# ShanningLiu/xsDeepFwFM_deprecated

Measured on AMD Instinct MI355X. Metric: CTR samples/sec (forward, batch 4096, Criteo-39) at 1/2/4/8 MI355X; AUC match, higher is better.
Workload: dtype f32

## Files before the change

xsdeepfwfm_deprecated_amd/DeepFMs.py:

```python
from __future__ import annotations

import contextlib
import logging
import math
import os
import random
from time import time, time_ns

import numpy as np
import torch
import torch.nn as nn
import torch.nn.functional as F

from . import metrics
from .QREmbeddingBag import QREmbeddingBag
from .engine import CpuEngine, ForwardEngine
from ._lib import DfwfmError, FLAG_INDEX_OUT_OF_RANGE

_log = logging.getLogger("xsDeepFwFM")


class DeepFMs(nn.Module):
    def __init__(self, field_size, feature_sizes, embedding_size=10, is_shallow_dropout=True,
                 dropout_shallow=[0.0, 0.0], h_depth=3, deep_nodes=400, is_deep_dropout=True,
                 dropout_deep=[0.5, 0.5, 0.5, 0.5], eval_metric=metrics.roc_auc_score, n_epochs=64,
                 batch_size=2048, learning_rate=0.001, momentum=0.9, optimizer_type="adam",
                 is_batch_norm=False, verbose=False, random_seed=0, weight_decay=0.0, use_fm=True,
                 use_fwlw=False, use_lw=False, use_ffm=False, use_fwfm=False, use_deep=True,
                 loss_type="logloss", use_cuda=True, n_class=1, greater_is_better=True, sparse=0.9,
                 warm=10, num_deeps=1, numerical=13, use_logit=0, embedding_bag=False,
                 quantization_aware=False, dynamic_quantization=False, static_quantization=False,
                 static_calibrate=False, qr_flag=0, qr_operation="mult", qr_collisions=1,
                 qr_threshold=200, md_flag=0, md_threshold=200, logger=None):
        super().__init__()
        self.logger = logger if logger is not None else _log
        self.field_size = int(field_size)
        self.feature_sizes = [int(s) for s in feature_sizes]
        self.embedding_size = int(embedding_size)
        self.is_shallow_dropout = is_shallow_dropout
        self.dropout_shallow = dropout_shallow
        self.h_depth = int(h_depth)
        self.num_deeps = int(num_deeps)
        self.deep_layers = [int(deep_nodes)] * self.h_depth
        self.is_deep_dropout = is_deep_dropout
        self.dropout_deep = [0.5] * (self.h_depth + 1)
        self.n_epochs = n_epochs
        self.batch_size = batch_size
        self.learning_rate = learning_rate
        self.momentum = momentum
        self.optimizer_type = optimizer_type
        self.is_batch_norm = is_batch_norm
        self.verbose = verbose
        self.weight_decay = weight_decay
        self.random_seed = random_seed
        self.use_fm, self.use_ffm, self.use_fwfm = use_fm, use_ffm, use_fwfm
        self.use_fwlw, self.use_lw, self.use_logit, self.use_deep = use_fwlw, use_lw, use_logit, use_deep
        self.loss_type = loss_type
        self.eval_metric = eval_metric
        self.use_cuda = use_cuda
        self.n_class = n_class
        self.greater_is_better = greater_is_better
        self.target_sparse = sparse
        self.warm = warm
        self.num = int(numerical)
        self.embedding_bag = embedding_bag if not qr_flag else qr_flag
        self.quantization_aware = quantization_aware
        self.static_quantization = static_quantization
        self.static_calibrate = static_calibrate
        self.dynamic_quantization = dynamic_quantization
        self.qr_flag = qr_flag
        self.qr_operation = qr_operation
        self.qr_collisions = qr_collisions
        self.qr_threshold = qr_threshold
        self.md_flag = md_flag
        self.md_threshold = md_threshold
        self.strict_index_check = True
        self.eval_batch_sets = True
        self.sparse_mlp_max_density = 0.0
        self.fwfm_pair_max = 0
        self.pack_tables = True
        self.small_batch_rows = 0
        self.mlp_dtype = "f32"
        self.deterministic = True
        self._defer_index_check = 0
        self._engine = None

        np.random.seed(self.random_seed)
        random.seed(self.random_seed)
        torch.manual_seed(self.random_seed)

        if quantization_aware or dynamic_quantization or static_quantization:
            raise NotImplementedError("quantization is not part of the MI355X engine (SURVEY.md section 2 #10)")
        if use_ffm:
            raise NotImplementedError("FFM is not part of the MI355X engine (SURVEY.md section 2 #12)")
        if self.num_deeps != 1:
            raise NotImplementedError("num_deeps > 1 is not supported")
        if is_batch_norm:
            raise NotImplementedError("batch norm in the deep tower is not supported")
        if self.use_cuda and not torch.cuda.is_available():
            self.use_cuda = False
            self.logger.info("Cuda is not available, automatically changed into cpu model")

        n_shallow = int(bool(use_fm)) + int(bool(use_ffm)) + int(bool(use_fwfm)) + int(bool(use_logit))
        if n_shallow > 1:
            self.logger.info("only support one type only, please make sure to choose only LR, FM, FFM or FwFM part")
            raise SystemExit(1)
        if n_shallow == 0 and not use_deep:
            self.logger.info("You have to choose more than one of (fm, ffm, fwfm, deep) models to use")
            raise SystemExit(1)
        self.logger.info(self._describe())

        D, Fs = self.embedding_size, self.field_size
        if use_logit or use_fm or use_fwfm:
            self.bias = nn.Parameter(torch.tensor([0.01]))
            if not use_fwlw:
                self.fm_1st_embeddings = self._tables(1)
            if self.dropout_shallow:
                self.fm_first_order_dropout = nn.Dropout(self.dropout_shallow[0])
            if use_fm or use_fwfm:
                self.fm_2nd_embeddings = self._tables(D)
                if self.dropout_shallow:
                    self.fm_second_order_dropout = nn.Dropout(self.dropout_shallow[1])
                if use_lw:
                    self.fm_1st = nn.Linear(Fs, 1, bias=False)
                if use_fwlw:
                    self.fwfm_linear = nn.Linear(D, Fs, bias=False)
                if use_fwfm:
                    self.field_cov = nn.Linear(Fs, Fs, bias=False)
        if use_deep:
            if not use_fm and not use_fwfm:
                self.fm_2nd_embeddings = self._tables(D)
            widths = [Fs * D] + self.deep_layers
            if self.is_deep_dropout:
                self.net_1_linear_0_dropout = nn.Dropout(self.dropout_deep[0])
            for i in range(1, self.h_depth + 1):
                setattr(self, f"net_1_linear_{i}", nn.Linear(widths[i - 1], widths[i]))
                setattr(self, f"net_1_linear_{i}_relu", nn.ReLU())
                if self.is_deep_dropout:
                    setattr(self, f"net_1_linear_{i}_dropout", nn.Dropout(self.dropout_deep[i]))
            self.net_1_fc = nn.Linear(self.deep_layers[-1], 1, bias=False)

    def _describe(self):
        if self.use_logit:
            return "The model is logistic regression."
        kind = "fm" if self.use_fm else ("fwfm" if self.use_fwfm else None)
        if kind and self.use_deep:
            return f"The model is deep{kind}({kind}+deep layers)"
        if kind:
            return f"The model is {kind} only"
        return "The model is deep layers only"

    def _tables(self, dim):
        if not self.embedding_bag:
            return nn.ModuleList([nn.Embedding(n, dim) for n in self.feature_sizes])
        tables = nn.ModuleList()
        for n in self.feature_sizes:
            if self.qr_flag and n > self.qr_threshold:
                tables.append(QREmbeddingBag(n, dim, self.qr_collisions, operation=self.qr_operation,
                                             mode="sum", sparse=False))
            else:
                bag = nn.EmbeddingBag(n, dim, mode="sum", sparse=False)
                w = np.random.uniform(low=-np.sqrt(1 / n), high=np.sqrt(1 / n), size=(n, dim)).astype(np.float32)
                bag.weight.data = torch.tensor(w)
                tables.append(bag)
        return tables

    def engine_config(self):
        return dict(field_size=self.field_size, numerical=self.num, embedding_size=self.embedding_size,
                    use_fwfm=int(bool(self.use_fwfm)), use_fm=int(bool(self.use_fm)),
                    use_logit=int(bool(self.use_logit)), use_deep=int(bool(self.use_deep)),
                    use_lw=int(bool(self.use_lw)), use_fwlw=int(bool(self.use_fwlw)),
                    h_depth=self.h_depth, deep_nodes=self.deep_layers[0])

    @staticmethod
    def _field_desc(mod_2nd, mod_1st):
        def parts(mod):
            if mod is None:
                return None, None
            if isinstance(mod, QREmbeddingBag):
                if mod.operation not in ("mult", "add"):
                    raise NotImplementedError("QR 'concat' changes the field width; unsupported")
                return mod.weight_q.detach(), mod.weight_r.detach()
            return mod.weight.detach(), None
        ref = mod_2nd if mod_2nd is not None else mod_1st
        if isinstance(ref, QREmbeddingBag):
            n, c, op = ref.num_categories, ref.num_collisions, 0 if ref.operation == "mult" else 1
        else:
            n, c, op = ref.weight.shape[0], 0, 0
        e2, e2r = parts(mod_2nd)
        e1, e1r = parts(mod_1st)
        return dict(emb2=e2, emb2_r=e2r, emb1=e1, emb1_r=e1r, n=n, c=c, op=op)

    def _sync_engine(self, device):
        if device.type == "cpu":
            return self._sync_cpu_engine()
        if device.type != "cuda":
            raise DfwfmError(f"DeepFMs forward runs on a HIP device or the CPU, not on {device}")
        if self._engine is None or self._engine.device != device:
            if self._engine is not None:
                self._engine.close()
            self._engine = ForwardEngine(self.engine_config(), device)
        eng = self._engine
        first = getattr(self, "fm_1st_embeddings", None)
        second = getattr(self, "fm_2nd_embeddings", None)
        fields = [self._field_desc(None if second is None else second[f], None if first is None else first[f])
                  for f in range(self.field_size)]
        eng.sync_tables(fields)

        def w(name, attr="weight"):
            m = getattr(self, name, None)
            return None if m is None else getattr(m, attr).detach()

        lin_w = [w(f"net_1_linear_{i}") for i in range(1, self.h_depth + 1)] if self.use_deep else []
        lin_b = [w(f"net_1_linear_{i}", "bias") for i in range(1, self.h_depth + 1)] if self.use_deep else []
        eng.sync_dense(w("field_cov"), w("fwfm_linear"), w("fm_1st") if self.use_lw else None,
                       self.bias.detach(), lin_w, lin_b, w("net_1_fc") if self.use_deep else None)
        return eng

    def _sync_inference(self, device):
        eng = self._sync_engine(device)
        if device.type == "cuda":
            first = getattr(self, "fm_1st_embeddings", None)
            second = getattr(self, "fm_2nd_embeddings", None)
            tabs = []
            for f in range(self.num, self.field_size):
                d = self._field_desc(None if second is None else second[f], None if first is None else first[f])
                tabs.append((d["emb2"], d["emb1"]))
            eng.sync_packed(tabs, self.pack_tables)
            eng.small_rows = max(int(getattr(self, "small_batch_rows", 0)), 0) if self.use_deep else 0
            eng.bf16 = eng.sync_bf16(self._mlp_bf16()) if self.use_deep else False
        return eng

    def _mlp_bf16(self) -> bool:
        dt = getattr(self, "mlp_dtype", "f32")
        if dt not in ("f32", "bf16"):
            raise ValueError(f"mlp_dtype must be 'f32' or 'bf16', got {dt!r}")
        if not self.use_deep or dt == "f32":
            return False
        if self.sparse_mlp_max_density > 0:
            raise ValueError("mlp_dtype='bf16' and sparse_mlp_max_density > 0 are two deep towers: choose one")
        return True

    def _sync_cpu_engine(self):
        if not isinstance(self._engine, CpuEngine):
            if self._engine is not None:
                self._engine.close()
            self._engine = CpuEngine(self.engine_config())
        first = getattr(self, "fm_1st_embeddings", None)
        second = getattr(self, "fm_2nd_embeddings", None)
        fields = [self._field_desc(None if second is None else second[f], None if first is None else first[f])
                  for f in range(self.field_size)]

        def w(name, attr="weight"):
            m = getattr(self, name, None)
            return None if m is None else getattr(m, attr).detach()
        lin_w = [w(f"net_1_linear_{i}") for i in range(1, self.h_depth + 1)] if self.use_deep else []
        lin_b = [w(f"net_1_linear_{i}", "bias") for i in range(1, self.h_depth + 1)] if self.use_deep else []
        self._engine.sync(fields, w("field_cov"), w("fwfm_linear"), w("fm_1st") if self.use_lw else None,
                          self.bias.detach(), lin_w, lin_b, w("net_1_fc") if self.use_deep else None)
        return self._engine

    def _param_layout(self):
        def parts(mod):
            if mod is None:
                return None, None
            if isinstance(mod, QREmbeddingBag):
                return mod.weight_q, mod.weight_r
            return mod.weight, None
        first = getattr(self, "fm_1st_embeddings", None)
        second = getattr(self, "fm_2nd_embeddings", None)
        fields = []
        for f in range(self.field_size):
            e2, e2r = parts(None if second is None else second[f])
            e1, e1r = parts(None if first is None else first[f])
            fields.append((e2, e2r, e1, e1r))

        def w(name, attr="weight"):
            m = getattr(self, name, None)
            return None if m is None else getattr(m, attr)
        H = self.h_depth if self.use_deep else 0
        dense = dict(field_cov=w("field_cov"), fwfm_lin=w("fwfm_linear"),
                     fm_1st=w("fm_1st") if self.use_lw else None, bias=getattr(self, "bias", None),
                     lin_w=[w(f"net_1_linear_{i}") for i in range(1, H + 1)],
                     lin_b=[w(f"net_1_linear_{i}", "bias") for i in range(1, H + 1)],
                     fc_w=w("net_1_fc") if self.use_deep else None)
        return fields, dense

    def _prep_inputs(self, Xi, Xv, device):
        ncat = self.field_size - self.num
        Xi = torch.as_tensor(Xi)
        Xv = torch.as_tensor(Xv)
        if Xi.dim() == 3:
            Xi = Xi.reshape(Xi.shape[0], Xi.shape[1])
        if Xi.dim() != 2 or Xi.shape[1] != ncat:
            raise RuntimeError(f"Xi must be [B, {ncat}, 1] or [B, {ncat}], got {tuple(Xi.shape)}")
        if Xv.dim() != 2 or Xv.shape[0] != Xi.shape[0] or Xv.shape[1] < self.num:
            raise RuntimeError(f"Xv must be [B, >= {self.num}], got {tuple(Xv.shape)}")
        Xi = Xi.to(device=device, dtype=torch.int64)
        Xv = Xv.to(device=device, dtype=torch.float32)
        if Xi.stride(1) != 1:
            Xi = Xi.contiguous()
        if Xv.stride(1) != 1:
            Xv = Xv.contiguous()
        return Xi, Xv

    def forward(self, Xi, Xv):
        device = self._device()
        eng = self._sync_engine(device)
        xi, xv = self._prep_inputs(Xi, Xv, device)
        needs_grad = torch.is_grad_enabled() and any(p.requires_grad for p in self.parameters())
        if needs_grad:
# ... 306 lines not shown
```

xsdeepfwfm_deprecated_amd/_lib.py:

```python
from __future__ import annotations

import ctypes
import os
import subprocess
import threading

import torch

PKG_DIR = os.path.dirname(os.path.abspath(__file__))
REPO_DIR = os.path.dirname(PKG_DIR)
CSRC = os.path.join(PKG_DIR, "csrc")
LIB_PATH = os.path.join(PKG_DIR, "libdfwfm.so")
LOAD_PATH = os.path.join(PKG_DIR, os.environ["DFWFM_LIB"]) if os.environ.get("DFWFM_LIB") else LIB_PATH
SOURCES = ["dfwfm_kernels.hip", "dfwfm_fwd32.hip", "dfwfm_ftrain.hip", "dfwfm_train.hip", "dfwfm_prune.hip", "dfwfm_metrics.hip", "dfwfm_sparse.hip",
           "dfwfm_spmlp.hip", "dfwfm_serve.hip", "dfwfm_bf16.hip", "dfwfm_capi.hip"]
EMB_SIZES = (4, 8, 10, 16, 32)
PER_D_SOURCES = ["dfwfm_kernels.hip", "dfwfm_train.hip"]


def _units():
    u = [(s, os.path.splitext(s)[0] + ".o", []) for s in SOURCES]
    for s in PER_D_SOURCES:
        u += [(s, f"{os.path.splitext(s)[0]}_d{d}.o", [f"-DDFWFM_KD={d}"]) for d in EMB_SIZES]
    return u
HEADERS = ["dfwfm_internal.h", "dfwfm_device.h", os.path.join("..", "..", "include", "dfwfm.h"),
           os.path.join("..", "..", "include", "dfwfm_serve.h"), os.path.join("..", "..", "include", "dfwfm_bf16.h")]
ARCH = os.environ.get("DFWFM_OFFLOAD_ARCH", "gfx950")
CPU_PATH = os.path.join(PKG_DIR, "libdfwfm_cpu.so")
CPU_SOURCES = ["dfwfm_cpu.cpp"]
CPU_HEADERS = [os.path.join("..", "..", "include", "dfwfm_cpu.h"), os.path.join("..", "..", "include", "dfwfm.h")]
INGEST_PATH = os.path.join(PKG_DIR, "libdfwfm_ingest.so")
INGEST_SOURCES = ["dfwfm_ingest.cpp"]
INGEST_HEADERS = [os.path.join("..", "..", "include", "dfwfm_ingest.h")]

DFWFM_OK = 0
STATUS = {0: "ok", -1: "invalid argument", -2: "unsupported", -3: "HIP error", -4: "bad state"}
FLAG_INDEX_OUT_OF_RANGE = 1
BWD_TABLES, BWD_MLP_WEIGHTS, BWD_TILES, BWD_SPREAD, BWD_REDUCE, BWD_SCATTER = 1, 2, 4, 8, 16, 32
FAMILY_SECOND, FAMILY_FIRST = 0, 1
ADAM_STATE_BYTES = 48


class DfwfmError(RuntimeError):
    pass


class dfwfm_config(ctypes.Structure):
    _fields_ = [(n, ctypes.c_int32) for n in (
        "field_size", "numerical", "embedding_size", "use_fwfm", "use_fm", "use_logit",
        "use_deep", "use_lw", "use_fwlw", "h_depth", "deep_nodes")]


class dfwfm_field_tables(ctypes.Structure):
    _fields_ = [
        ("emb2", ctypes.c_void_p), ("emb2_r", ctypes.c_void_p),
        ("emb1", ctypes.c_void_p), ("emb1_r", ctypes.c_void_p),
        ("num_categories", ctypes.c_int64), ("qr_collisions", ctypes.c_int64),
        ("qr_operation", ctypes.c_int32), ("reserved", ctypes.c_int32),
    ]


class dfwfm_field_grads(ctypes.Structure):
    _fields_ = [(n, ctypes.c_void_p) for n in ("emb2", "emb2_r", "emb1", "emb1_r")]


class dfwfm_grads(ctypes.Structure):
    _fields_ = [
        ("fields", ctypes.POINTER(dfwfm_field_grads)),
        ("field_cov", ctypes.c_void_p), ("fwfm_lin", ctypes.c_void_p), ("fm_1st", ctypes.c_void_p),
        ("bias", ctypes.c_void_p), ("lin_w", ctypes.POINTER(ctypes.c_void_p)),
        ("lin_b", ctypes.POINTER(ctypes.c_void_p)), ("fc_w", ctypes.c_void_p),
    ]


class dfwfm_adam_tensor(ctypes.Structure):
    _fields_ = [("param", ctypes.c_void_p), ("grad", ctypes.c_void_p), ("exp_avg", ctypes.c_void_p),
                ("exp_avg_sq", ctypes.c_void_p), ("numel", ctypes.c_int64)]


class dfwfm_sparse_dest(ctypes.Structure):
    _fields_ = [("q", ctypes.c_int64), ("r", ctypes.c_int64)]


class dfwfm_prune_source(ctypes.Structure):
    _fields_ = [("values", ctypes.c_void_p), ("numel", ctypes.c_int64), ("sym_f", ctypes.c_int32),
                ("reserved", ctypes.c_int32)]


_P = ctypes.c_void_p
SIGNATURES = {
    "dfwfm_model_create": (ctypes.c_int, [ctypes.POINTER(dfwfm_config), ctypes.POINTER(_P)]),
    "dfwfm_model_destroy": (None, [_P]),
    "dfwfm_model_set_tables": (ctypes.c_int, [_P, ctypes.POINTER(dfwfm_field_tables), ctypes.c_int32, _P]),
    "dfwfm_model_set_dense": (ctypes.c_int, [_P, _P, _P, _P, _P, ctypes.POINTER(_P), ctypes.POINTER(_P), _P, _P]),
    "dfwfm_model_set_dense_zero": (ctypes.c_int, [_P, _P, _P, _P, _P, ctypes.POINTER(_P), ctypes.POINTER(_P), _P, _P,
                                                  ctypes.c_int64, _P]),
    "dfwfm_forward": (ctypes.c_int, [_P, _P, ctypes.c_int64, _P, ctypes.c_int64, ctypes.c_int64, _P, _P]),
    "dfwfm_forward_batches": (ctypes.c_int, [_P, ctypes.c_int32, _P, ctypes.c_int64, _P, ctypes.c_int64,
                                             ctypes.c_int64, _P, _P]),
    "dfwfm_forward_workspace_bytes": (ctypes.c_int, [_P, ctypes.c_int64, ctypes.POINTER(ctypes.c_size_t)]),
    "dfwfm_forward_ws": (ctypes.c_int, [_P, _P, ctypes.c_int64, _P, ctypes.c_int64, ctypes.c_int64, _P, _P,
                                        ctypes.c_size_t, _P]),
    "dfwfm_model_build_sparse_mlp": (ctypes.c_int, [_P, ctypes.c_double, ctypes.POINTER(ctypes.c_int32), _P]),
    "dfwfm_model_build_fwfm_pairs": (ctypes.c_int, [_P, ctypes.c_int32, ctypes.POINTER(ctypes.c_int32), _P]),
    "dfwfm_model_pack_tables": (ctypes.c_int, [_P, ctypes.c_int32, ctypes.POINTER(ctypes.c_int32), _P]),
    "dfwfm_forward_gather": (ctypes.c_int, [_P, _P, ctypes.c_int64, _P, ctypes.c_int64, ctypes.c_int64, _P,
                                            ctypes.c_int64, _P, _P]),
    "dfwfm_train_forward": (ctypes.c_int, [_P, _P, ctypes.c_int64, _P, ctypes.c_int64, ctypes.c_int64, _P,
                                           ctypes.c_float, ctypes.c_uint32, _P]),
    "dfwfm_backward": (ctypes.c_int, [_P, _P, ctypes.POINTER(dfwfm_grads), _P]),
    "dfwfm_backward_phases": (ctypes.c_int, [_P, _P, ctypes.POINTER(dfwfm_grads), ctypes.c_int32, _P]),
    "dfwfm_adam_step": (ctypes.c_int, [ctypes.POINTER(dfwfm_adam_tensor), ctypes.c_int32, ctypes.c_double,
                                       ctypes.c_double, ctypes.c_double, ctypes.c_double, ctypes.c_double,
                                       ctypes.c_int64, _P]),
    "dfwfm_set_step_source": (ctypes.c_int, [_P, _P]),
    "dfwfm_workspace_generation": (ctypes.c_int, [_P, ctypes.POINTER(ctypes.c_int64)]),
    "dfwfm_adam_step_dev": (ctypes.c_int, [ctypes.POINTER(dfwfm_adam_tensor), ctypes.c_int32, ctypes.c_double,
                                           ctypes.c_double, ctypes.c_double, ctypes.c_double, ctypes.c_double,
                                           _P, _P]),
    "dfwfm_bce_grad": (ctypes.c_int, [_P, _P, ctypes.c_int64, ctypes.c_double, _P, _P, _P]),
    "dfwfm_backward_phases_bce": (ctypes.c_int, [_P, _P, _P, ctypes.c_double, _P, _P, ctypes.POINTER(dfwfm_grads),
                                                 ctypes.c_int32, _P]),
    "dfwfm_sparse_grads_size": (ctypes.c_int, [_P, ctypes.c_int32, ctypes.c_int64, ctypes.POINTER(ctypes.c_int64),
                                               ctypes.POINTER(ctypes.c_int32), ctypes.POINTER(ctypes.c_int64)]),
    "dfwfm_sparse_grads_apply": (ctypes.c_int, [_P, ctypes.c_int32, _P, _P, _P, ctypes.c_int64, _P]),
    "dfwfm_sparse_grads_local": (ctypes.c_int, [_P, ctypes.c_int32, ctypes.POINTER(dfwfm_sparse_dest), ctypes.c_int64,
                                                _P, _P, ctypes.c_int64, _P, _P, _P, _P]),
    "dfwfm_prune_workspace_bytes": (ctypes.c_int64, [ctypes.c_int64]),
    "dfwfm_prune_threshold": (ctypes.c_int, [ctypes.POINTER(dfwfm_prune_source), ctypes.c_int32, ctypes.c_double,
                                             _P, _P, ctypes.c_int64, _P]),
    "dfwfm_prune_apply": (ctypes.c_int, [_P, ctypes.c_int64, ctypes.c_int32, _P, _P]),
    "dfwfm_metrics_workspace_bytes": (ctypes.c_int64, [ctypes.c_int64]),
    "dfwfm_eval_metrics": (ctypes.c_int, [_P, _P, ctypes.c_int64, _P, _P, ctypes.c_int64, _P]),
    "dfwfm_read_error_flag": (ctypes.c_int, [_P, ctypes.POINTER(ctypes.c_int32), _P]),
    "dfwfm_last_error": (ctypes.c_char_p, []),
    "dfwfm_diag_stamps": (ctypes.c_int, [_P, ctypes.POINTER(ctypes.c_uint64), ctypes.c_int64, _P]),
    "dfwfm_abi_version": (ctypes.c_int, []),
    "dfwfm_set_deterministic": (ctypes.c_int, [_P, ctypes.c_int32]),
}

SERVE_SIGNATURES = {
    "dfwfm_serve_abi_version": (ctypes.c_int, []),
    "dfwfm_serve_workspace_bytes": (ctypes.c_int, [_P, ctypes.c_int64, ctypes.POINTER(ctypes.c_size_t)]),
    "dfwfm_serve_forward": (ctypes.c_int, [_P, _P, ctypes.c_int64, _P, ctypes.c_int64, ctypes.c_int64, _P, _P,
                                           ctypes.c_size_t, _P]),
}

BF16_SIGNATURES = {
    "dfwfm_bf16_abi_version": (ctypes.c_int, []),
    "dfwfm_model_pack_bf16": (ctypes.c_int, [_P, ctypes.c_int, _P]),
    "dfwfm_bf16_workspace_bytes": (ctypes.c_int, [_P, ctypes.c_int64, ctypes.POINTER(ctypes.c_size_t)]),
    "dfwfm_bf16_forward": (ctypes.c_int, [_P, _P, ctypes.c_int64, _P, ctypes.c_int64, ctypes.c_int64, _P, _P,
                                          ctypes.c_size_t, _P]),
}

_lib = None
_lock = threading.Lock()


def _stale() -> bool:
    if not os.path.exists(LIB_PATH):
        return True
    t = os.path.getmtime(LIB_PATH)
    deps = [os.path.join(CSRC, s) for s in SOURCES + HEADERS]
    return any(os.path.getmtime(d) > t for d in deps if os.path.exists(d))


def _stale_ingest() -> bool:
    if not os.path.exists(INGEST_PATH):
        return True
    t = os.path.getmtime(INGEST_PATH)
    deps = [os.path.join(CSRC, s) for s in INGEST_SOURCES + INGEST_HEADERS]
    return any(os.path.getmtime(d) > t for d in deps if os.path.exists(d))


def build_ingest(force: bool = False, verbose: bool = False) -> str:
    if not force and not _stale_ingest():
        return INGEST_PATH
    cxx = os.environ.get("CXX", "g++")
    tmp = INGEST_PATH + ".tmp"
    cmd = [cxx, "-O3", "-std=c++17", "-fPIC", "-shared", "-pthread", "-o", tmp] + \
        [os.path.join(CSRC, s) for s in INGEST_SOURCES]
    if verbose:
        print(" ".join(cmd))
    subprocess.run(cmd, check=True, cwd=CSRC)
    os.replace(tmp, INGEST_PATH)
    return INGEST_PATH


def _stale_cpu() -> bool:
    if not os.path.exists(CPU_PATH):
        return True
    t = os.path.getmtime(CPU_PATH)
    deps = [os.path.join(CSRC, s) for s in CPU_SOURCES + CPU_HEADERS]
    return any(os.path.getmtime(d) > t for d in deps if os.path.exists(d))


def build_cpu(force: bool = False, verbose: bool = False) -> str:
    if not force and not _stale_cpu():
        return CPU_PATH
    cxx = os.environ.get("CXX", "g++")
    tmp = CPU_PATH + ".tmp"
    cmd = [cxx, "-O3", "-std=c++17", "-fPIC", "-shared", "-pthread", "-mavx2", "-mfma", "-o", tmp] + \
        [os.path.join(CSRC, s) for s in CPU_SOURCES]
    if verbose:
        print(" ".join(cmd))
    subprocess.run(cmd, check=True, cwd=CSRC)
    os.replace(tmp, CPU_PATH)
    return CPU_PATH


def build(force: bool = False, verbose: bool = False) -> str:
    build_ingest(force, verbose)
    build_cpu(force, verbose)
    hipcc = os.environ.get("HIPCC", "/opt/rocm/bin/hipcc")
    flags = [f"--offload-arch={ARCH}", "-O3", "-std=c++17", "-fPIC"] + os.environ.get("DFWFM_HIPCC_FLAGS", "").split()
    stamp = os.path.join(CSRC, ".build_flags")
    if not os.path.exists(stamp) or open(stamp).read() != " ".join(flags):
        force = True
    if not force and not _stale():
        return LIB_PATH
    from concurrent.futures import ThreadPoolExecutor
    units = _units()
    objs = [os.path.join(CSRC, o) for _, o, _ in units]
    hdr_m = max(os.path.getmtime(os.path.join(CSRC, h)) for h in HEADERS)

    def compile_one(i):
        src, _, extra = units[i]
        src = os.path.join(CSRC, src)
        if not force and os.path.exists(objs[i]) and \
                os.path.getmtime(objs[i]) >= max(os.path.getmtime(src), hdr_m):
            return
        cmd = [hipcc] + flags + extra + ["-c", "-o", objs[i], src]
        if verbose:
            print(" ".join(cmd))
        subprocess.run(cmd, check=True, cwd=CSRC)

    jobs = int(os.environ.get("MAX_JOBS", "0")) or min(len(units), max(1, len(os.sched_getaffinity(0))))
# ... 31 lines not shown
    "dfwfm_cpu_saved_floats": (ctypes.c_int64, [ctypes.POINTER(dfwfm_config)]),
    "dfwfm_cpu_forward": (ctypes.c_int, [ctypes.POINTER(dfwfm_cpu_model), _P, ctypes.c_int64, _P, ctypes.c_int64,
                                         ctypes.c_int64, _P, _P, ctypes.c_float, ctypes.c_uint32,
                                         ctypes.POINTER(ctypes.c_int32), ctypes.c_int32]),
    "dfwfm_cpu_backward": (ctypes.c_int, [ctypes.POINTER(dfwfm_cpu_model), _P, ctypes.c_int64, _P, ctypes.c_int64,
                                          ctypes.c_int64, _P, _P, ctypes.c_float, ctypes.c_uint32,
                                          ctypes.POINTER(dfwfm_grads), ctypes.c_int32]),
    "dfwfm_cpu_last_error": (ctypes.c_char_p, []),
    "dfwfm_cpu_abi_version": (ctypes.c_int, []),
}


def cpu_lib():
    global _cpu
    if _cpu is not None:
        return _cpu
    with _lock:
        if _cpu is None:
            if not os.path.exists(CPU_PATH):
                raise DfwfmError(f"{CPU_PATH} is missing: run xsdeepfwfm_deprecated_amd.build()")
            L = ctypes.CDLL(CPU_PATH)
            for name, (res, args) in CPU_SIGNATURES.items():
                fn = getattr(L, name)
                fn.restype = res
                fn.argtypes = args
            if L.dfwfm_cpu_abi_version() != 1:
                raise DfwfmError("libdfwfm_cpu ABI mismatch")
            _cpu = L
    return _cpu


def check_cpu(rc: int, what: str) -> None:
    if rc != DFWFM_OK:
        msg = cpu_lib().dfwfm_cpu_last_error().decode(errors="replace")
        raise DfwfmError(f"{what} failed ({STATUS.get(rc, rc)}): {msg}")


def ingest_lib():
    global _ingest
    if _ingest is not None:
        return _ingest
    with _lock:
        if _ingest is None:
            if not os.path.exists(INGEST_PATH):
                raise DfwfmError(f"{INGEST_PATH} is missing: run xsdeepfwfm_deprecated_amd.build()")
            L = ctypes.CDLL(INGEST_PATH)
            for name, (res, args) in INGEST_SIGNATURES.items():
                fn = getattr(L, name)
                fn.restype = res
                fn.argtypes = args
            _ingest = L
    return _ingest


def lib():
    global _lib
    if _lib is not None:
        return _lib
    with _lock:
        if _lib is not None:
            return _lib
        if not os.path.exists(LOAD_PATH):
            raise DfwfmError(f"{LOAD_PATH} is missing: run xsdeepfwfm_deprecated_amd.build() "
                             "(hipcc --offload-arch=gfx950); there is no CPU fallback")
        L = ctypes.CDLL(LOAD_PATH)
        for name, (res, args) in SIGNATURES.items():
            fn = getattr(L, name)
            fn.restype = res
            fn.argtypes = args
        if L.dfwfm_abi_version() != 4:
            raise DfwfmError("libdfwfm ABI mismatch")
        for name, (res, args) in SERVE_SIGNATURES.items():
            fn = getattr(L, name)
            fn.restype = res
            fn.argtypes = args
        if L.dfwfm_serve_abi_version() != 1:
            raise DfwfmError("libdfwfm serve ABI mismatch")
        for name, (res, args) in BF16_SIGNATURES.items():
            fn = getattr(L, name)
            fn.restype = res
            fn.argtypes = args
        if L.dfwfm_bf16_abi_version() != 1:
            raise DfwfmError("libdfwfm bf16 ABI mismatch")
        _lib = L
    return _lib


def check(rc: int, what: str) -> None:
    if rc != DFWFM_OK:
        msg = lib().dfwfm_last_error().decode(errors="replace")
        raise DfwfmError(f"{what} failed ({STATUS.get(rc, rc)}): {msg}")
```

xsdeepfwfm_deprecated_amd/csrc/dfwfm_capi.hip:

```cpp
#include <hip/hip_runtime.h>
#include <mutex>
#include <stdint.h>
#include <stdarg.h>
#include <stdio.h>
#include <stdlib.h>
#include <string.h>

#include <cmath>
#include <string>
#include <vector>

#include "dfwfm_internal.h"
#include "../../include/dfwfm_serve.h"
#include "../../include/dfwfm_bf16.h"

using namespace dfwfm;

struct dfwfm_model {
  dfwfm_config cfg;
  int device;
  int F, D, num, H, N;
  int NT, NC0, SX, SY, TPW, MT, S, W0, KS;
  int TPWF, tail;
  int flags;
  size_t lds_bytes;
  size_t lds_gather;
  int NG, TPWI, tailI;
  int r32;
  size_t lds_r32;
  size_t lds_ftrain;
  void* cu_stream[8];
  int cu_count[8], cu_n, cu_next;
  int dev_cus;
  size_t lds_inf;
  int sp;
  const float* lin_w[kMaxH];
  int2* d_ell;
  int32_t* d_cnt;
  int32_t* d_spstat;
  int spW[kMaxH];
  int64_t spoff[kMaxH];
  double sp_density;
  uint8_t fw_list4[kMaxPieces], fw_off4[5];
  uint8_t fw_list8[kMaxPieces], fw_off8[9];
  FieldDev* d_fields;
  float* d_upack;
  int2* d_pairs;
  float* d_pkrows;
  size_t pkrows_floats;
  const float** d_pk;
  int pkw;
  int32_t npairs;
  int32_t* d_err;
  float4* d_wpack;
  size_t wpack_elems;
  float* d_mlp_b;
  float* d_fc;
  float* d_fwlw;
  float* d_lw;
  float* d_bias;
  uint16_t* d_wbf16;
  bool bf16_on;
  uint64_t* d_stamps;
  size_t stamps_cap;
  size_t stamps_ring;
  size_t stamps_next;
  float4* d_wtpack;
  size_t wtpack_elems;
  int wt_off[kMaxH + 1];
  float* d_rsk;
  float* d_ws;
  int64_t ws_batch;
  int64_t ws_gen;
  float* sv_e;
  float* sv_fo;
  float* sv_x[kMaxH + 1];
  float* sv_g[kMaxH + 1];
  float* sv_de;
  int32_t* sv_keys;
  int64_t keys_stride;
  bool t_keys;
  float* sv_x0;
  float* red_part;
  float* dw_part;
  float* dw_bpart;
  int64_t dw_slices;
  FieldDev h_fields[64];
  const int64_t* t_xi;
  int64_t t_xs;
  const float* t_xv;
  int64_t t_vs;
  int64_t t_batch;
  float t_drop;
  uint32_t t_seed;
  const int64_t* step_src;
  bool trained;
  bool bwd_tables;
  bool bwd_fused_red;
  float* bwd_loss_sum;
  bool deterministic;
  bool tables_set;
  bool dense_set;
};

namespace {

thread_local std::string g_last_error;

int fail(int code, const char* fmt, ...) __attribute__((format(printf, 2, 3)));
int fail(int code, const char* fmt, ...) {
  char buf[512];
  va_list ap;
  va_start(ap, fmt);
  vsnprintf(buf, sizeof buf, fmt, ap);
  va_end(ap);
  g_last_error = buf;
  return code;
}

int hip_fail(hipError_t e, const char* what) {
  return fail(DFWFM_ERR_HIP, "%s: %s", what, hipGetErrorString(e));
}

#define HIP_TRY(expr)                                  \
  do {                                                 \
    hipError_t e_ = (expr);                            \
    if (e_ != hipSuccess) return hip_fail(e_, #expr);  \
  } while (0)

template <typename T>
int dev_alloc(T** p, size_t count) {
  *p = nullptr;
  if (count == 0) count = 1;
  HIP_TRY(hipMalloc(reinterpret_cast<void**>(p), count * sizeof(T)));
  return DFWFM_OK;
}

void free_model(dfwfm_model* m) {
  if (!m) return;
  void* ptrs[] = {m->d_fields, m->d_upack, m->d_err,     m->d_wpack, m->d_mlp_b,   m->d_fc,  m->d_fwlw,
                  m->d_lw,     m->d_bias,  m->d_stamps,  m->d_wtpack, m->d_rsk,   m->d_ws,
                  m->d_ell,    m->d_cnt,   m->d_spstat, m->d_pairs, m->d_pkrows, m->d_pk,
                  m->d_wbf16};
  for (void* p : ptrs)
    if (p) (void)hipFree(p);
// ... 51 lines not shown
    return fail(DFWFM_ERR_INVALID_ARG, "use_logit with use_fwlw has no first-order tables");
  const int F = c.field_size, D = c.embedding_size;
  int H = 0, N = 0, NT = 0, TPW = 0;
  if (c.use_deep) {
    H = c.h_depth;
    N = c.deep_nodes;
    if (H < 1 || H > 16) return fail(DFWFM_ERR_UNSUPPORTED, "h_depth %d outside [1, 16]", H);
    NT = (N + 15) / 16;
    TPW = (NT + 3) / 4;
    if (N < 1 || TPW > kMaxTPW)
      return fail(DFWFM_ERR_UNSUPPORTED, "deep_nodes %d outside [1, %d]", N, 64 * kMaxTPW);
  }

  dfwfm_model* m = new dfwfm_model();
  memset(m, 0, sizeof *m);
  m->cfg = c;
  m->deterministic = true;
  hipError_t e = hipGetDevice(&m->device);
  if (e != hipSuccess) {
    delete m;
    return hip_fail(e, "hipGetDevice");
  }
  m->F = F;
  m->D = D;
  m->num = c.numerical;
  m->H = H;
  m->N = N;
  m->NT = NT;
  m->TPW = TPW;
  m->NC0 = (F * D + 15) / 16;
  m->MT = (F + 15) / 16;
  m->S = (F + 3) / 4;
  fw_schedule(m->MT, D, m->S, 4, m->fw_list4, m->fw_off4);
  fw_schedule(m->MT, D, m->S, 8, m->fw_list8, m->fw_off8);
  m->W0 = m->NC0 * 16 > 4 * m->S * D ? m->NC0 * 16 : 4 * m->S * D;
  const int kx = m->W0 > NT * 16 ? m->W0 : NT * 16;
  m->SX = r4(kx) + 4;
  m->SY = c.use_deep ? NT * 16 + 4 : 0;
  m->KS = 1;
  m->TPWF = TPW;
  m->tail = 0;
  if (c.use_deep && m->KS == 1 && NT % 4 == 1 && NT >= 5 && m->NC0 >= 4 && m->NC0 <= 4 * kTailC &&
      NT <= 4 * kTailC) {
    m->TPWF = NT / 4;
    m->tail = 1;
  }
  const bool second = c.use_fwfm || c.use_fm;
  m->flags = (second ? kHasSecond : 0) | (c.use_deep ? kHasDeep : 0) |
             (c.use_fwlw ? kFoFwlw : kFoTables) | ((second && c.use_lw) ? kFoLw : 0) |
             ((second || c.use_deep) ? kNeedE : 0);
  const LdsLayout L = lds_layout(F, D, m->MT, m->S, m->SX, m->SY, m->TPWF > 0 ? m->TPWF : 1, m->KS,
                                 c.use_deep != 0, m->tail != 0);
  m->lds_bytes = sizeof(float) * (size_t)L.total;
  m->lds_gather = sizeof(float) * (size_t)lds_layout(F, D, m->MT, m->S, m->SX, m->SY, m->TPWF > 0 ? m->TPWF : 1,
                                                     1, false, false).total;
  m->NG = 4;
  m->TPWI = m->TPWF;
  m->tailI = m->tail;
  m->lds_inf = m->lds_bytes;
  if (!c.use_deep)
    m->lds_inf = sizeof(float) * (size_t)lds_layout(F, D, m->MT, m->S, m->SX, m->SY, 1, 1, false, false, 8).total;
  if (c.use_deep && m->KS == 1 && NT <= 32 && m->NC0 <= 32) {
    if (diag_opt("ng", 8) == 8) {
      m->NG = 8;
      m->tailI = (NT % 8 == 1 && NT >= 9 && m->NC0 >= 8) ? 1 : 0;
      m->TPWI = m->tailI ? NT / 8 : (NT + 7) / 8;
      m->lds_inf = sizeof(float) * (size_t)lds_layout(F, D, m->MT, m->S, m->SX, m->SY, m->TPWI, 1, true,
                                                      m->tailI != 0, 8).total;
    }
  }
  {
    const int r32 = diag_opt("r32", -1);
    const int mode = r32 < 0 ? 1 : (r32 != 0 ? 2 : 0);
    m->r32 = (c.use_deep && fwd32_supported(F, D, H, NT, m->NC0, m->tailI, m->NG)) ? mode : 0;
    m->lds_r32 = m->r32 ? fwd32_lds_bytes(F, D, m->MT, m->S, m->SX) : 0;
    m->lds_ftrain = (c.use_deep && ftrain_supported(F, D, H, NT, m->NC0, m->tailI, m->NG))
                        ? ftrain_lds_bytes(F, D, m->MT, m->S, m->SX, m->SY) : 0;
    if (m->lds_ftrain > 160 * 1024) m->lds_ftrain = 0;
  }
  if (m->lds_bytes > 160 * 1024 || m->lds_inf > 160 * 1024) {
    free_model(m);
    return fail(DFWFM_ERR_UNSUPPORTED, "LDS tile of %zu bytes exceeds 160 KiB", m->lds_bytes);
  }

  int rc = DFWFM_OK;
  if ((rc = dev_alloc(&m->d_fields, F)) || (rc = dev_alloc(&m->d_upack, (size_t)m->MT * m->S * 64)) ||
      (rc = dev_alloc(&m->d_err, 1)) ||
      (rc = dev_alloc(&m->d_fwlw, (size_t)F * D)) || (rc = dev_alloc(&m->d_lw, F)) ||
      (rc = dev_alloc(&m->d_bias, 1))) {
    free_model(m);
    return rc;
  }
  if ((rc = dev_alloc(&m->d_rsk, (size_t)m->MT * m->S * 64))) {
    free_model(m);
    return rc;
  }
  if (c.use_deep) {
    m->wpack_elems = (size_t)NT * m->NC0 * 64 + (size_t)(H - 1) * NT * NT * 64;
    if (m->wpack_elems * sizeof(float4) >= (size_t)1 << 31) {
      free_model(m);
      return fail(DFWFM_ERR_UNSUPPORTED, "packed MLP weights exceed the 2 GiB buffer-descriptor range");
    }
    m->wtpack_elems = m->wpack_elems;
    m->wt_off[1] = 0;
    for (int l = 2; l <= H; ++l) m->wt_off[l] = m->wt_off[l - 1] + (l == 2 ? m->NC0 : NT) * NT * 64;
    if ((rc = dev_alloc(&m->d_wtpack, m->wtpack_elems)) || (rc = dev_alloc(&m->d_wpack, m->wpack_elems)) ||
        (rc = dev_alloc(&m->d_mlp_b, (size_t)H * NT * 16)) || (rc = dev_alloc(&m->d_fc, (size_t)NT * 16))) {
      free_model(m);
      return rc;
    }
  }
  e = hipMemset(m->d_err, 0, sizeof(int32_t));
  if (e == hipSuccess) e = hipMemset(m->d_upack, 0, sizeof(float) * (size_t)m->MT * m->S * 64);
  if (e != hipSuccess) {
    free_model(m);
    return hip_fail(e, "hipMemset");
  }
  *out = m;
  return DFWFM_OK;
}

void dfwfm_model_destroy(dfwfm_model* m) { free_model(m); }

int dfwfm_model_set_tables(dfwfm_model* m, const dfwfm_field_tables* t, int32_t n, void* stream) {
  if (!m || !t) return fail(DFWFM_ERR_INVALID_ARG, "null argument");
  if (n != m->F) return fail(DFWFM_ERR_INVALID_ARG, "%d tables for %d fields", n, m->F);
  const bool need_fo = (m->flags & kFoTables) != 0;
  const bool need_e = (m->flags & kNeedE) != 0;
  for (int f = 0; f < n; ++f) {
    const dfwfm_field_tables& x = t[f];
    if (need_e && !x.emb2) return fail(DFWFM_ERR_INVALID_ARG, "field %d: emb2 is null", f);
    if (need_fo && !x.emb1) return fail(DFWFM_ERR_INVALID_ARG, "field %d: emb1 is null", f);
    if (x.num_categories < 1) return fail(DFWFM_ERR_INVALID_ARG, "field %d: num_categories < 1", f);
    if (x.qr_collisions < 0) return fail(DFWFM_ERR_INVALID_ARG, "field %d: qr_collisions < 0", f);
    if (x.qr_collisions > 0) {
      if (f < m->num) return fail(DFWFM_ERR_INVALID_ARG, "field %d: numerical field cannot be QR", f);
      if ((need_e && !x.emb2_r) || (need_fo && !x.emb1_r))
        return fail(DFWFM_ERR_INVALID_ARG, "field %d: QR remainder table is null", f);
      if (x.qr_operation != 0 && x.qr_operation != 1)
        return fail(DFWFM_ERR_UNSUPPORTED, "field %d: QR operation %d (only mult=0, add=1)", f,
                    x.qr_operation);
    }
    const uintptr_t align = (m->D % 4 == 0) ? 16 : (m->D % 2 == 0 ? 8 : 4);
    if (((uintptr_t)x.emb2 % align) || (x.emb2_r && ((uintptr_t)x.emb2_r % align)))
      return fail(DFWFM_ERR_UNSUPPORTED, "field %d: table base not %zu-byte aligned", f, (size_t)align);
  }
  FieldDev host[64];
  memcpy(host, t, sizeof(dfwfm_field_tables) * n);
  for (int f = 0; f < n; ++f)
    if (host[f].c > 0) host[f].n = (host[f].n + host[f].c - 1) / host[f].c * host[f].c;
  memcpy(m->h_fields, host, sizeof(FieldDev) * n);
  m->pkw = 0;
  m->flags &= ~kHasQR;
  for (int f = 0; f < n; ++f)
    if (host[f].c > 0) m->flags |= kHasQR;
  HIP_TRY(hipMemcpyAsync(m->d_fields, host, sizeof(FieldDev) * n, hipMemcpyHostToDevice, (hipStream_t)stream));
  HIP_TRY(hipStreamSynchronize((hipStream_t)stream));
  m->tables_set = true;
  return DFWFM_OK;
}

static int set_dense_impl(dfwfm_model* m, const float* field_cov, const float* fwfm_lin, const float* fm_1st,
                          const float* bias, const float* const* lin_w, const float* const* lin_b,
                          const float* fc_w, float* zero, int64_t nzero, void* stream) {
  if (!m) return fail(DFWFM_ERR_INVALID_ARG, "null model");
  if (nzero < 0 || (nzero > 0 && (!zero || (nzero & 3) || (reinterpret_cast<uintptr_t>(zero) & 15))))
    return fail(DFWFM_ERR_INVALID_ARG, "zero range: 16-byte aligned, a multiple of 4 floats");
  hipStream_t s = (hipStream_t)stream;
  const dfwfm_config& c = m->cfg;
  if (c.use_fwfm && !field_cov) return fail(DFWFM_ERR_INVALID_ARG, "use_fwfm needs field_cov");
  if ((m->flags & kFoFwlw) && !fwfm_lin) return fail(DFWFM_ERR_INVALID_ARG, "use_fwlw needs fwfm_linear");
  if ((m->flags & kFoLw) && !fm_1st) return fail(DFWFM_ERR_INVALID_ARG, "use_lw needs fm_1st");
  if (!bias) return fail(DFWFM_ERR_INVALID_ARG, "bias is required");
  PackList L;
  memset(&L, 0, sizeof L);
  int blocks = 0;
  auto job = [&](int type, const float* src, void* dst, int64_t total, int a, int b, int d) {
    PackJob& j = L.j[L.n++];
    j.src = src;
    j.dst = reinterpret_cast<float*>(dst);
    j.total = total;
    j.type = type;
    j.a = a;
    j.b = b;
    j.d = d;
    j.block0 = blocks;
    blocks += (int)((total + 255) / 256);
  };
  if (nzero > 0) {
    const int64_t n4 = nzero / 4;
    if ((n4 + 256 * kPackZeroPT - 1) / (256 * kPackZeroPT) > 0x3fffffff) return fail(DFWFM_ERR_UNSUPPORTED, "zero range");
    PackJob& j = L.j[L.n++];
    j.src = nullptr;
    j.dst = zero;
    j.total = n4;
    j.type = kPackZero;
    j.a = j.b = j.d = 0;
    j.block0 = blocks;
    blocks += (int)((n4 + 256 * kPackZeroPT - 1) / (256 * kPackZeroPT));
  }
  if (c.use_fwfm || c.use_fm) {
    const int64_t tot = (int64_t)m->MT * m->S * 64;
    job(kPackFwfm, field_cov, m->d_upack, tot, m->F, c.use_fm ? 1 : 0, m->S);
    job(kPackFwfmSym, field_cov, m->d_rsk, tot, m->F, c.use_fm ? 1 : 0, m->S);
  }
  if (m->flags & kFoFwlw) job(kPackPad, fwfm_lin, m->d_fwlw, m->F * m->D, m->F * m->D, 0, 0);
  if (m->flags & kFoLw) job(kPackPad, fm_1st, m->d_lw, m->F, m->F, 0, 0);
  job(kPackPad, bias, m->d_bias, 1, 1, 0, 0);
  if (c.use_deep) {
    if (!lin_w || !lin_b || !fc_w) return fail(DFWFM_ERR_INVALID_ARG, "use_deep needs MLP weights");
    size_t off = 0;
    for (int h = 0; h < m->H; ++h) {
      if (!lin_w[h] || !lin_b[h]) return fail(DFWFM_ERR_INVALID_ARG, "layer %d weight/bias is null", h);
      const int K = h == 0 ? m->F * m->D : m->N;
      const int NC = h == 0 ? m->NC0 : m->NT;
      const int64_t tot = (int64_t)m->NT * NC * 64;
      job(kPackLinear, lin_w[h], m->d_wpack + off, tot, m->N, K, NC);
      job(kPackLinearT, lin_w[h], m->d_wtpack + m->wt_off[h + 1], tot, m->N, K, m->NT);
      job(kPackPad, lin_b[h], m->d_mlp_b + (size_t)h * m->NT * 16, m->NT * 16, m->N, 0, 0);
      off += (size_t)tot;
    }
    job(kPackPad, fc_w, m->d_fc, m->NT * 16, m->N, 0, 0);
  }
  hipError_t e = launch_pack_list(L, blocks, s);
  if (e != hipSuccess) return hip_fail(e, "pack launch");
  m->dense_set = true;
  m->sp = 0;
  m->bf16_on = false;
  m->flags &= ~kPairs;
  for (int h = 0; h < m->H; ++h) m->lin_w[h] = lin_w ? lin_w[h] : nullptr;
  return DFWFM_OK;
}

int dfwfm_model_set_dense(dfwfm_model* m, const float* field_cov, const float* fwfm_lin, const float* fm_1st,
                          const float* bias, const float* const* lin_w, const float* const* lin_b,
                          const float* fc_w, void* stream) {
  return set_dense_impl(m, field_cov, fwfm_lin, fm_1st, bias, lin_w, lin_b, fc_w, nullptr, 0, stream);
}

int dfwfm_model_set_dense_zero(dfwfm_model* m, const float* field_cov, const float* fwfm_lin, const float* fm_1st,
                               const float* bias, const float* const* lin_w, const float* const* lin_b,
                               const float* fc_w, float* zero, int64_t nzero, void* stream) {
  return set_dense_impl(m, field_cov, fwfm_lin, fm_1st, bias, lin_w, lin_b, fc_w, zero, nzero, stream);
}

}

namespace {

int check_inputs(dfwfm_model* m, const int64_t* xi, int64_t xi_stride, const float* xv, int64_t xv_stride,
                 int64_t batch, const void* out) {
  if (batch < 0) return fail(DFWFM_ERR_INVALID_ARG, "negative batch");
  if (!m->tables_set || !m->dense_set)
    return fail(DFWFM_ERR_STATE, "set_tables and set_dense must precede forward");
  if (batch == 0) return DFWFM_OK;
  const int ncat = m->F - m->num;
  if (!out || (ncat > 0 && !xi) || (m->num > 0 && !xv))
    return fail(DFWFM_ERR_INVALID_ARG, "null input/output pointer");
  if (ncat > 0 && xi_stride < ncat) return fail(DFWFM_ERR_INVALID_ARG, "xi_stride < F - numerical");
  if (m->num > 0 && xv_stride < m->num) return fail(DFWFM_ERR_INVALID_ARG, "xv_stride < numerical");
  if ((batch + kBM - 1) / kBM > 0x7fffffff) return fail(DFWFM_ERR_UNSUPPORTED, "batch too large");
  return DFWFM_OK;
}

void fill_forward_args(const dfwfm_model* m, FwdArgs& a, const int64_t* xi, int64_t xi_stride, const float* xv,
                       int64_t xv_stride, int64_t batch, float* out) {
  memset(&a, 0, sizeof a);
  a.fields = m->d_fields;
  a.xi = xi;
  a.xi_stride = xi_stride;
  a.xv = xv;
  a.xv_stride = xv_stride;
  a.batch = batch;
  a.out = out;
  a.err = m->d_err;
  a.upack = m->d_upack;
  a.pk = m->pkw ? m->d_pk : nullptr;
  a.pkw = m->pkw;
  a.pairs = m->d_pairs;
  a.npairs = m->npairs;
  a.fwlw = m->d_fwlw;
  a.lw = m->d_lw;
  a.bias = m->d_bias;
  a.wpack = m->d_wpack;
  a.wpack_bytes = (int32_t)(m->wpack_elems * sizeof(float4));
  a.mlp_b = m->d_mlp_b;
  a.fc = m->d_fc;
  a.F = m->F;
  a.num = m->num;
  a.H = m->H;
  a.N = m->N;
  a.NT = m->NT;
  a.NC0 = m->NC0;
  a.MT = m->MT;
  a.S = m->S;
  a.W0 = m->W0;
  a.tail = m->tail;
  a.SX = m->SX;
  a.SY = m->SY;
  a.flags = m->flags;
  if (!m->cfg.use_deep && m->MT <= 3) a.flags |= kP3Pieces;
  a.ns = (m->NC0 == 25 && m->NT == 25) ? 25 : 0;
  memcpy(a.fw_list4, m->fw_list4, sizeof a.fw_list4);
  memcpy(a.fw_list8, m->fw_list8, sizeof a.fw_list8);
  memcpy(a.fw_off4, m->fw_off4, sizeof a.fw_off4);
  memcpy(a.fw_off8, m->fw_off8, sizeof a.fw_off8);
}

int dw_plan(const dfwfm_model* m, int64_t batch, int* per_split, int64_t* splits, int64_t* rows,
            int64_t* cap = nullptr) {
  const int edge = kDwEdge, quantum = kDwRows;
  const int nnb = (m->N + edge - 1) / edge;
  int ps = 0;
  for (int l = 1; l <= m->H; ++l) ps += nnb * (((l == 1 ? m->F * m->D : m->N) + edge - 1) / edge);
  *per_split = ps;
  *splits = *rows = 0;
  if (cap) *cap = 0;
  if (ps == 0 || batch <= 0) return DFWFM_OK;
  int64_t sp = 256 / ps;
  const int64_t max_splits = (batch + 127) / 128;
  if (sp > max_splits) sp = max_splits;
  if (sp < 1) sp = 1;
  const int64_t wmax = r4(m->F * m->D) > m->N ? r4(m->F * m->D) : m->N;
  const int64_t rows_cap = ((0x7fffffffLL / (wmax * 4)) * 4 - 4 * quantum) / quantum * quantum;
  if (rows_cap < quantum) return fail(DFWFM_ERR_UNSUPPORTED, "MLP rows of %lld floats", (long long)wmax);
  if ((batch + sp - 1) / sp > rows_cap) sp = (batch + rows_cap - 1) / rows_cap;
  if (cap) *cap = sp;
  int64_t r = (batch + sp - 1) / sp;
  r = (r + quantum - 1) / quantum * quantum;
  *splits = (batch + r - 1) / r;
  *rows = r;
  return DFWFM_OK;
}

int ensure_workspace(dfwfm_model* m, int64_t batch) {
  if (batch <= m->ws_batch) return DFWFM_OK;
  const int64_t FD = (int64_t)m->F * m->D;
  const int64_t SE = r4((int)FD);
  const int64_t per_row = SE + FD + m->F + (m->H > 0 ? SE + 2 * (int64_t)m->H * m->N : 0);
  const int64_t keys_stride = (batch + 3) & ~(int64_t)3;
  const int64_t keys_words = (int64_t)(m->F - m->num) * keys_stride;
  const int64_t red_blocks = (batch + kBM - 1) / kBM;
  const int64_t red_floats = red_blocks * red_outputs(m->F, m->D, m->N, m->num);
  int per_split = 0;
  int64_t splits = 0, rows = 0, cap = 0;
  int rc = dw_plan(m, batch, &per_split, &splits, &rows, &cap);
  if (rc != DFWFM_OK) return rc;
  const int64_t slices = cap > 1 ? (int64_t)per_split * cap : 0;
  const int64_t dw_floats = slices * (kDwEdge * kDwEdge + kDwEdge);
  if (m->d_ws) (void)hipFree(m->d_ws);
  m->d_ws = nullptr;
  m->ws_batch = 0;
  const size_t total = (size_t)(per_row * batch + red_floats + dw_floats + keys_words + 64);
  HIP_TRY(hipMalloc(reinterpret_cast<void**>(&m->d_ws), sizeof(float) * total));
  auto al = [](int64_t x) { return (x + 3) & ~(int64_t)3; };
  float* p = m->d_ws;
  m->dw_part = p;   p += slices * kDwEdge * kDwEdge;
  m->dw_bpart = p;  p += al(slices * kDwEdge);
  m->dw_slices = slices;
  m->sv_e = p;   p += al(SE * batch);
  m->sv_de = p;  p += al(FD * batch);
  m->red_part = p;  p += al(red_floats);
  m->sv_fo = p;  p += al((int64_t)m->F * batch);
  m->sv_keys = reinterpret_cast<int32_t*>(p);  p += keys_words;
  m->keys_stride = keys_stride;
  for (int h = 0; h <= kMaxH; ++h) m->sv_x[h] = m->sv_g[h] = nullptr;
  if (m->H > 0) {
    m->sv_x0 = p;  p += SE * batch;
    for (int h = 1; h <= m->H; ++h) {
      m->sv_x[h] = p;  p += (int64_t)m->N * batch;
      m->sv_g[h] = p;  p += (int64_t)m->N * batch;
    }
  }
  m->ws_batch = batch;
  m->ws_gen++;
  return DFWFM_OK;
}

size_t split_e_floats(const dfwfm_model* m, int64_t batch) { return (size_t)batch * m->NC0 * 16; }
size_t split_ws_bytes(const dfwfm_model* m, int64_t batch) {
  return sizeof(float) * (split_e_floats(m, batch) + (size_t)batch);
}

int diag_stamps_buffer(dfwfm_model* m, int64_t batch, int which, uint64_t** out) {
  *out = nullptr;
  if (diag_opt("stamps", 0) != which) return DFWFM_OK;
  const size_t grid = (size_t)((batch + kBM - 1) / kBM);
  const size_t ring = diag_opt("ring", 1) > 1 ? (size_t)diag_opt("ring", 1) : 1;
  if (grid > m->stamps_cap || ring != m->stamps_ring) {
    if (m->d_stamps) (void)hipFree(m->d_stamps);
    m->d_stamps = nullptr;
    m->stamps_cap = 0;
    HIP_TRY(hipMalloc(reinterpret_cast<void**>(&m->d_stamps), ring * grid * kStampSlots * sizeof(uint64_t)));
    m->stamps_cap = grid;
    m->stamps_ring = ring;
    m->stamps_next = 0;
  }
  *out = m->d_stamps + (m->stamps_next % ring) * m->stamps_cap * kStampSlots;
  m->stamps_next++;
  return DFWFM_OK;
}

std::mutex g_cu_mu;

int stream_cu_count(dfwfm_model* m, void* stream) {
  std::lock_guard<std::mutex> lock(g_cu_mu);
  if (m->dev_cus == 0) {
    hipDeviceProp_t prop;
    m->dev_cus = hipGetDeviceProperties(&prop, m->device) == hipSuccess ? prop.multiProcessorCount : 256;
  }
  const int cached = m->cu_n < 8 ? m->cu_n : 8;
  for (int i = 0; i < cached; ++i)
    if (m->cu_stream[i] == stream) return m->cu_count[i];
  int n = 0;
  uint32_t mask[64] = {0};
  if (hipExtStreamGetCUMask((hipStream_t)stream, 64, mask) == hipSuccess) {
    for (int i = 0; i < 64; ++i) n += __builtin_popcount(mask[i]);
  } else {
    (void)hipGetLastError();
    hipDeviceProp_t prop;
    n = hipGetDeviceProperties(&prop, m->device) == hipSuccess ? prop.multiProcessorCount : 256;
  }
  const int slot = m->cu_n < 8 ? m->cu_n++ : (m->cu_next++ & 7);
  m->cu_stream[slot] = stream;
  m->cu_count[slot] = n > 0 ? n : 256;
  return m->cu_count[slot];
}

bool use_fwd32(dfwfm_model* m, int64_t batch, void* stream) {
  if (m->r32 == 0) return false;
  if (m->r32 == 2) return true;
  const int cus = stream_cu_count(m, stream);
  const bool masked = cus < m->dev_cus;
  return (batch + 31) / 32 >= (masked ? 1 : 2) * (int64_t)cus;
}

}

extern "C" {

int dfwfm_forward(dfwfm_model* m, const int64_t* xi, int64_t xi_stride, const float* xv, int64_t xv_stride,
                  int64_t batch, float* out, void* stream) {
  if (!m) return fail(DFWFM_ERR_INVALID_ARG, "null model");
  int rc = check_inputs(m, xi, xi_stride, xv, xv_stride, batch, out);
  if (rc != DFWFM_OK || batch == 0) return rc;
  FwdArgs a;
  fill_forward_args(m, a, xi, xi_stride, xv, xv_stride, batch, out);
  a.flags &= ~diag_opt("drop_flags", 0);
  a.flags |= kPrio | kPrioEpi | kDeferTail;
  if ((rc = diag_stamps_buffer(m, batch, 1, &a.stamps)) != DFWFM_OK) return rc;
  a.tail = m->tailI;
  const bool r32 = (a.flags & kHasDeep) && use_fwd32(m, batch, stream);
  hipError_t e = r32 ? launch_fwd32(a, m->D, m->lds_r32, (hipStream_t)stream)
                     : launch_forward(a, m->D, m->TPWI > 0 ? m->TPWI : 1, m->KS, m->NG, m->lds_inf, (hipStream_t)stream);
  if (e != hipSuccess) return hip_fail(e, "forward launch");
  return DFWFM_OK;
}

int dfwfm_forward_batches(dfwfm_model* m, int32_t nb, const int64_t* const* xi, int64_t xi_stride,
                          const float* const* xv, int64_t xv_stride, int64_t batch, float* const* out, void* stream) {
  if (!m) return fail(DFWFM_ERR_INVALID_ARG, "null model");
  if (nb < 0) return fail(DFWFM_ERR_INVALID_ARG, "negative batch count");
  if (nb == 0) return DFWFM_OK;
  if (!xi || !xv || !out) return fail(DFWFM_ERR_INVALID_ARG, "null pointer array");
  for (int32_t i = 0; i < nb; ++i) {
    const int rc = check_inputs(m, xi[i], xi_stride, xv[i], xv_stride, batch, out[i]);
    if (rc != DFWFM_OK) return rc;
  }
  if (batch == 0) return DFWFM_OK;
  if (nb == 1) {
    for (int32_t i = 0; i < nb; ++i) {
      const int rc = dfwfm_forward(m, xi[i], xi_stride, xv[i], xv_stride, batch, out[i], stream);
      if (rc != DFWFM_OK) return rc;
    }
    return DFWFM_OK;
  }
  if ((int64_t)nb * ((batch + kBM - 1) / kBM) > 0x7fffffff) return fail(DFWFM_ERR_UNSUPPORTED, "batch set too large");
  const int64_t set_rows = (int64_t)(nb < kMaxSet ? nb : kMaxSet) * batch;
  const bool r32 = m->cfg.use_deep && use_fwd32(m, set_rows, stream);
  const int rows = r32 ? 32 : kBM;
  for (int32_t i0 = 0; i0 < nb; i0 += kMaxSet) {
    const int32_t n = nb - i0 < kMaxSet ? nb - i0 : kMaxSet;
    FwdArgs a;
    fill_forward_args(m, a, xi[i0], xi_stride, xv[i0], xv_stride, batch, out[i0]);
    a.flags |= kPrio | kPrioEpi | kDeferTail;
    a.tail = m->tailI;
    if (n > 1) {
      a.nb = n;
      a.tiles = (int32_t)((batch + rows - 1) / rows);
      for (int32_t j = 0; j < n; ++j) {
        a.set_xi[j] = xi[i0 + j];
        a.set_xv[j] = xv[i0 + j];
        a.set_out[j] = out[i0 + j];
      }
    }
    int rc = diag_stamps_buffer(m, (int64_t)n * a.tiles * rows, 1, &a.stamps);
    if (rc != DFWFM_OK) return rc;
    const hipError_t e = r32 ? launch_fwd32(a, m->D, m->lds_r32, (hipStream_t)stream)
                             : launch_forward(a, m->D, m->TPWI > 0 ? m->TPWI : 1, m->KS, m->NG, m->lds_inf,
                                              (hipStream_t)stream);
    if (e != hipSuccess) return hip_fail(e, "batch-set forward launch");
  }
  return DFWFM_OK;
}

int dfwfm_forward_workspace_bytes(dfwfm_model* m, int64_t batch, size_t* bytes) {
  if (!m || !bytes || batch < 0) return fail(DFWFM_ERR_INVALID_ARG, "null argument");
  *bytes = m->sp ? split_ws_bytes(m, batch) : 0;
  return DFWFM_OK;
}

int dfwfm_forward_ws(dfwfm_model* m, const int64_t* xi, int64_t xi_stride, const float* xv, int64_t xv_stride,
                     int64_t batch, float* out, void* workspace, size_t ws_bytes, void* stream) {
  if (!m) return fail(DFWFM_ERR_INVALID_ARG, "null model");
  if (!m->sp || !workspace) return dfwfm_forward(m, xi, xi_stride, xv, xv_stride, batch, out, stream);
  int rc = check_inputs(m, xi, xi_stride, xv, xv_stride, batch, out);
  if (rc != DFWFM_OK || batch == 0) return rc;
  if (ws_bytes < split_ws_bytes(m, batch))
    return fail(DFWFM_ERR_INVALID_ARG, "workspace of %zu bytes < %zu (dfwfm_forward_workspace_bytes)", ws_bytes,
                split_ws_bytes(m, batch));
  if (reinterpret_cast<uintptr_t>(workspace) % 16) return fail(DFWFM_ERR_INVALID_ARG, "workspace not 16-byte aligned");
  FwdArgs a;
  fill_forward_args(m, a, xi, xi_stride, xv, xv_stride, batch, out);
  a.part_stride = m->NC0 * 16;
  a.part_e = static_cast<float*>(workspace);
  a.part_fs = a.part_e + split_e_floats(m, batch);
  if ((rc = diag_stamps_buffer(m, batch, 1, &a.stamps)) != DFWFM_OK) return rc;
  a.tail = m->tailI;
  {
    hipError_t e = launch_forward_gather(a, m->D, m->lds_gather, (hipStream_t)stream);
    if (e != hipSuccess) return hip_fail(e, "gather launch");
    SpMlpArgs sa;
    memset(&sa, 0, sizeof sa);
    sa.part_e = a.part_e;
    sa.part_fs = a.part_fs;
    sa.part_stride = a.part_stride;
    sa.K0p = a.part_stride;
    sa.ell = m->d_ell;
    sa.gcnt = m->d_cnt + m->H * m->N;
    for (int h = 0; h < m->H; ++h) {
      sa.W[h] = m->spW[h];
      sa.off[h] = m->spoff[h];
    }
    sa.mlp_b = m->d_mlp_b;
    sa.fc = m->d_fc;
    sa.bias = m->d_bias;
    sa.out = out;
    sa.batch = batch;
    sa.H = m->H;
    sa.N = m->N;
    sa.NT = m->NT;
    e = launch_sparse_mlp(sa, (hipStream_t)stream);
    if (e != hipSuccess) return hip_fail(e, "sparse MLP launch");
    return DFWFM_OK;
  }
}

int dfwfm_forward_gather(dfwfm_model* m, const int64_t* xi, int64_t xi_stride, const float* xv, int64_t xv_stride,
                         int64_t batch, float* deep_emb, int64_t deep_emb_stride, float* first_second, void* stream) {
  if (!m) return fail(DFWFM_ERR_INVALID_ARG, "null model");
  if (!m->cfg.use_deep) return fail(DFWFM_ERR_UNSUPPORTED, "forward_gather: the model has no deep tower");
  int rc = check_inputs(m, xi, xi_stride, xv, xv_stride, batch, first_second);
  if (rc != DFWFM_OK || batch == 0) return rc;
  if (!deep_emb || deep_emb_stride != (int64_t)m->NC0 * 16)
    return fail(DFWFM_ERR_INVALID_ARG, "deep_emb stride %lld, need %d", (long long)deep_emb_stride, m->NC0 * 16);
  if (reinterpret_cast<uintptr_t>(deep_emb) % 16) return fail(DFWFM_ERR_INVALID_ARG, "deep_emb not 16-byte aligned");
  FwdArgs a;
  fill_forward_args(m, a, xi, xi_stride, xv, xv_stride, batch, nullptr);
  a.flags &= ~kHasDeep;
  if (m->MT <= 3) a.flags |= kP3Pieces;
  a.part_stride = m->NC0 * 16;
  a.part_e = deep_emb;
  a.part_fs = first_second;
  hipError_t e = launch_forward(a, m->D, 1, 1, 8, m->lds_inf, (hipStream_t)stream);
  if (e != hipSuccess) return hip_fail(e, "gather launch");
  return DFWFM_OK;
}

int dfwfm_serve_abi_version(void) { return DFWFM_SERVE_ABI_VERSION; }

int dfwfm_serve_workspace_bytes(dfwfm_model* m, int64_t batch, size_t* bytes) {
  if (!m || !bytes) return fail(DFWFM_ERR_INVALID_ARG, "null argument");
  if (batch < 0) return fail(DFWFM_ERR_INVALID_ARG, "negative batch");
// ... 52 lines not shown
  sa.NC0 = m->NC0;
  e = launch_serve_mlp(sa, (hipStream_t)stream);
  if (e != hipSuccess) return hip_fail(e, "serve MLP launch");
  return DFWFM_OK;
}

int dfwfm_bf16_abi_version(void) { return DFWFM_BF16_ABI_VERSION; }

int dfwfm_model_pack_bf16(dfwfm_model* m, int enable, void* stream) {
  if (!m) return fail(DFWFM_ERR_INVALID_ARG, "null model");
  m->bf16_on = false;
  if (!enable) return DFWFM_OK;
  if (!m->cfg.use_deep) return fail(DFWFM_ERR_UNSUPPORTED, "bf16 pack: the model has no deep tower");
  if (!m->dense_set) return fail(DFWFM_ERR_STATE, "set_dense must precede pack_bf16");
  if (!m->d_wbf16) {
    int rc = dev_alloc(&m->d_wbf16, bf16_pack_elems(m->H, m->NT, m->NC0));
    if (rc != DFWFM_OK) return rc;
  }
  hipError_t e = launch_bf16_pack(m->lin_w, m->d_wbf16, m->H, m->N, m->F * m->D, m->NT, m->NC0, (hipStream_t)stream);
  if (e != hipSuccess) return hip_fail(e, "bf16 pack launch");
  m->bf16_on = true;
  return DFWFM_OK;
}

int dfwfm_bf16_workspace_bytes(dfwfm_model* m, int64_t batch, size_t* bytes) {
  if (!m || !bytes) return fail(DFWFM_ERR_INVALID_ARG, "null argument");
  if (batch < 0) return fail(DFWFM_ERR_INVALID_ARG, "negative batch");
  if (!m->cfg.use_deep) return fail(DFWFM_ERR_UNSUPPORTED, "bf16 forward: the model has no deep tower");
  *bytes = bf16_workspace_bytes(m->NT, m->NC0, batch);
  return DFWFM_OK;
}

int dfwfm_bf16_forward(dfwfm_model* m, const int64_t* xi, int64_t xi_stride, const float* xv, int64_t xv_stride,
                       int64_t batch, float* out, void* workspace, size_t ws_bytes, void* stream) {
  if (!m) return fail(DFWFM_ERR_INVALID_ARG, "null model");
  if (!m->cfg.use_deep) return fail(DFWFM_ERR_UNSUPPORTED, "bf16 forward: the model has no deep tower");
  int rc = check_inputs(m, xi, xi_stride, xv, xv_stride, batch, out);
  if (rc != DFWFM_OK) return rc;
  if (!m->bf16_on)
    return fail(DFWFM_ERR_STATE, "bf16 forward: the bf16 weight copy is absent or stale (dfwfm_model_pack_bf16)");
  if (batch == 0) return DFWFM_OK;
  if (!workspace) return fail(DFWFM_ERR_INVALID_ARG, "null workspace");
  const size_t need = bf16_workspace_bytes(m->NT, m->NC0, batch);
  if (ws_bytes < need)
    return fail(DFWFM_ERR_INVALID_ARG, "workspace of %zu bytes < %zu (dfwfm_bf16_workspace_bytes)", ws_bytes, need);
  if (reinterpret_cast<uintptr_t>(workspace) % 16) return fail(DFWFM_ERR_INVALID_ARG, "workspace not 16-byte aligned");
  const int64_t tiles = (batch + kBM - 1) / kBM;
  if (tiles * m->NT > 0x7fffffff) return fail(DFWFM_ERR_UNSUPPORTED, "batch too large for the bf16 forward");
  const size_t rows16 = (size_t)tiles * kBM;
  Bf16Args ba;
  memset(&ba, 0, sizeof ba);
  float* w = static_cast<float*>(workspace);
  float* deep_emb = w;
  w += rows16 * m->NC0 * 16;
  float* fs = w;
  w += rows16;
  ba.partial = w;
  w += rows16 * m->NT;
  ba.act[0] = reinterpret_cast<uint16_t*>(w);
  ba.act[1] = ba.act[0] + rows16 * m->NT * 16;
  FwdArgs a;
  fill_forward_args(m, a, xi, xi_stride, xv, xv_stride, batch, nullptr);
  a.flags &= ~kHasDeep;
  if (m->MT <= 3) a.flags |= kP3Pieces;
  a.part_stride = m->NC0 * 16;
  a.part_e = deep_emb;
  a.part_fs = fs;
  hipError_t e = launch_forward(a, m->D, 1, 1, 8, m->lds_inf, (hipStream_t)stream);
  if (e != hipSuccess) return hip_fail(e, "bf16 gather launch");
  ba.deep_emb = deep_emb;
  ba.fs = fs;
  ba.wb = m->d_wbf16;
  ba.mlp_b = m->d_mlp_b;
  ba.fc = m->d_fc;
  ba.bias = m->d_bias;
  ba.out = out;
  ba.batch = batch;
  ba.H = m->H;
  ba.N = m->N;
  ba.NT = m->NT;
  ba.NC0 = m->NC0;
  e = launch_bf16_mlp(ba, (hipStream_t)stream);
  if (e != hipSuccess) return hip_fail(e, "bf16 MLP launch");
  return DFWFM_OK;
}

int dfwfm_model_pack_tables(dfwfm_model* m, int32_t enable, int32_t* enabled, void* stream) {
  if (!m || !enabled) return fail(DFWFM_ERR_INVALID_ARG, "null argument");
  *enabled = 0;
  m->pkw = 0;
  if (!enable) return DFWFM_OK;
  if (!m->tables_set) return fail(DFWFM_ERR_STATE, "set_tables must precede pack_tables");
  const int need = kHasSecond | kNeedE | kFoTables;
  if ((m->flags & need) != need || (m->flags & kHasQR) || m->F - m->num < 1) return DFWFM_OK;
  const int D = m->D;
  const int pkw = D + 1 <= 16 ? 16 : (D + 4) & ~3;
  PackTabList L;
  memset(&L, 0, sizeof L);
  L.D = D;
  L.pkw = pkw;
  size_t rows = 0;
  for (int f = m->num; f < m->F; ++f) rows += (size_t)m->h_fields[f].n;
  if (rows * pkw > m->pkrows_floats) {
    if (m->d_pkrows) (void)hipFree(m->d_pkrows);
    m->d_pkrows = nullptr;
    m->pkrows_floats = 0;
    HIP_TRY(hipMalloc(reinterpret_cast<void**>(&m->d_pkrows), rows * pkw * sizeof(float)));
    m->pkrows_floats = rows * pkw;
  }
  if (!m->d_pk) HIP_TRY(hipMalloc(reinterpret_cast<void**>(&m->d_pk), 64 * sizeof(float*)));
  const float* bases[64] = {};
  size_t off = 0;
  for (int f = m->num; f < m->F; ++f) {
    const int j = f - m->num;
    const int64_t n = m->h_fields[f].n;
    bases[f] = m->d_pkrows + off;
    L.emb2[j] = m->h_fields[f].emb2;
    L.emb1[j] = m->h_fields[f].emb1;
    L.dst[j] = m->d_pkrows + off;
    L.n[j] = n;
    const int64_t nb = (n + 255) / 256;
    if ((int64_t)L.blk0[j] + nb > 0x7fffffff) return fail(DFWFM_ERR_UNSUPPORTED, "tables too large to pack");
    L.blk0[j + 1] = L.blk0[j] + (int32_t)nb;
    off += (size_t)n * pkw;
  }
  L.nf = m->F - m->num;
  hipStream_t s = (hipStream_t)stream;
  HIP_TRY(hipMemcpyAsync(m->d_pk, bases, sizeof bases, hipMemcpyHostToDevice, s));
  HIP_TRY(hipStreamSynchronize(s));
  hipError_t e = launch_pack_tables(L, s);
  if (e != hipSuccess) return hip_fail(e, "pack tables launch");
  m->pkw = pkw;
  *enabled = 1;
  return DFWFM_OK;
}

int dfwfm_model_build_fwfm_pairs(dfwfm_model* m, int32_t max_pairs, int32_t* enabled, void* stream) {
  if (!m || !enabled) return fail(DFWFM_ERR_INVALID_ARG, "null argument");
  *enabled = 0;
  m->flags &= ~kPairs;
  if (!m->dense_set) return fail(DFWFM_ERR_STATE, "set_dense must precede build_fwfm_pairs");
  if (!(m->flags & kHasSecond) || max_pairs <= 0) return DFWFM_OK;
  hipStream_t s = (hipStream_t)stream;
  std::vector<float> pk((size_t)m->MT * m->S * 64);
  hipError_t e = hipMemcpyAsync(pk.data(), m->d_upack, pk.size() * sizeof(float), hipMemcpyDeviceToHost, s);
  if (e == hipSuccess) e = hipStreamSynchronize(s);
  if (e != hipSuccess) return hip_fail(e, "read FwFM pack");
  std::vector<int2> list;
  for (int k = 0; k < m->F; ++k)
    for (int l = k + 1; l < m->F; ++l) {
      const float w = pk[((size_t)(k >> 4) * m->S + (l >> 2)) * 64 + (k & 15) + 16 * (l & 3)];
      if (w != 0.f) {
        if ((int)list.size() >= max_pairs) return DFWFM_OK;
        int2 q;
        q.x = k | (l << 16);
        memcpy(&q.y, &w, sizeof w);
        list.push_back(q);
      }
    }
  if (!m->d_pairs) {
    const size_t cap = (size_t)m->F * (m->F - 1) / 2 + 1;
    e = hipMalloc(&m->d_pairs, cap * sizeof(int2));
    if (e != hipSuccess) return hip_fail(e, "pair list alloc");
  }
  if (!list.empty()) {
    e = hipMemcpyAsync(m->d_pairs, list.data(), list.size() * sizeof(int2), hipMemcpyHostToDevice, s);
// ... 747 lines not shown
```

xsdeepfwfm_deprecated_amd/csrc/dfwfm_fwd32.hip:

```cpp
#include <hip/hip_runtime.h>
#include <stdint.h>

#include "dfwfm_device.h"
#include "dfwfm_internal.h"

namespace dfwfm {

namespace {

constexpr int kRT = 2;
constexpr int kRows = 16 * kRT;
constexpr int kNG = 8;
constexpr int kTPW = 3;
constexpr int kNS = 25;
constexpr int kNTH = 64 * kNG;

struct Lds32 {
  int buf, fs, dsum, desc, lw, fwlw, upk, fo, part2, tailr, taild, total;
};

__host__ __device__ inline Lds32 lds32_layout(int F, int D, int MT, int S, int SX) {
  Lds32 L;
  int o = 0;
  L.buf = o;   o += kRows * SX;
  L.fs = o;    o += kRows;
  L.dsum = o;  o += kNG * kRows;
  int s = o;
  L.desc = s;  s += r4(14 * F);
  L.lw = s;    s += r4(F);
  L.fwlw = s;  s += r4(F * D);
  L.upk = s;   s += MT * S * 64;
  L.fo = s;    s += kRows * r4(F);
  L.part2 = s; s += kRT * MT * D * 16;
  int t = o;
  L.tailr = t; t += kNG * kRT * 64 * 4;
  L.taild = t; t += 4 * kRows;
  L.total = r4(s > t ? s : t);
  return L;
}

template <int TPW, int RT>
__device__ __forceinline__ void mfma_chunk_rt(f32x4 (&acc)[RT][TPW], const float4 (&a)[RT], const f32x4 (&w)[TPW]) {
#pragma unroll
  for (int s = 0; s < 4; ++s)
#pragma unroll
    for (int rt = 0; rt < RT; ++rt)
#pragma unroll
      for (int j = 0; j < TPW; ++j) {
        const float av = s == 0 ? a[rt].x : (s == 1 ? a[rt].y : (s == 2 ? a[rt].z : a[rt].w));
        acc[rt][j] = __builtin_amdgcn_mfma_f32_16x16x4f32(w[j][s], av, acc[rt][j], 0, 0, 0);
      }
}

template <int TPW, int RT, int NG, int NS>
__device__ __forceinline__ void k_loop_rt(f32x4 (&acc)[RT][TPW], const float* __restrict__ act, int SA,
                                          const LayerStream<TPW, 1, NG>& ls, f32x4 (&b0)[TPW], f32x4 (&b1)[TPW],
                                          f32x4 (&b2)[TPW], int lane, const TailStream<NG>& ts, f32x4 (&tp)[RT],
                                          bool mid_barrier) {
  const int voff = lane * 16;
  const float* arow = act + (lane & 15) * SA + 4 * (lane >> 4);
  float4 a0[RT], a1[RT], a2[RT];
#pragma unroll
  for (int rt = 0; rt < RT; ++rt) {
    a0[rt] = *reinterpret_cast<const float4*>(arow + rt * 16 * SA);
    a1[rt] = *reinterpret_cast<const float4*>(arow + rt * 16 * SA + 16);
  }
#pragma unroll
  for (int i = 0; i < NS; ++i) {
    f32x4 (&X)[TPW] = (i % 3 == 0) ? b0 : ((i % 3 == 1) ? b1 : b2);
    f32x4 (&Z)[TPW] = (i % 3 == 0) ? b2 : ((i % 3 == 1) ? b0 : b1);
    float4 (&AX)[RT] = (i % 3 == 0) ? a0 : ((i % 3 == 1) ? a1 : a2);
    float4 (&AZ)[RT] = (i % 3 == 0) ? a2 : ((i % 3 == 1) ? a0 : a1);
    if (i + 3 == NS && mid_barrier) __syncthreads();
    if (i + 2 < NS) {
#pragma unroll
      for (int rt = 0; rt < RT; ++rt) AZ[rt] = *reinterpret_cast<const float4*>(arow + rt * 16 * SA + 16 * (i + 2));
      ls.load(Z, ls.c0 + i + 2, voff);
    } else {
      ts.template load_set<TPW>(ls.rsrc, Z, i + 2 == NS ? 0 : TPW, voff);
    }
    mfma_chunk_rt<TPW, RT>(acc, AX, X);
    __builtin_amdgcn_sched_group_barrier(0x100, RT, 0);
    for (int q = 0; q < TPW; ++q) {
      __builtin_amdgcn_sched_group_barrier(0x008, 2 * RT, 0);
      __builtin_amdgcn_sched_group_barrier(0x020, 1, 0);
    }
    __builtin_amdgcn_sched_group_barrier(0x008, 2 * RT * TPW, 0);
    __builtin_amdgcn_sched_barrier(0);
  }
  f32x4 c0[RT], c1[RT];
#pragma unroll
  for (int rt = 0; rt < RT; ++rt) c0[rt] = c1[rt] = f32x4{0.f, 0.f, 0.f, 0.f};
#pragma unroll
  for (int half = 0; half < 2; ++half) {
    const f32x4 (&B)[TPW] = ((NS + half) % 3 == 0) ? b0 : (((NS + half) % 3 == 1) ? b1 : b2);
#pragma unroll
    for (int j = 0; j < TPW; ++j) {
      const int u = half * TPW + j;
      if (u < ts.cnt) {
#pragma unroll
        for (int rt = 0; rt < RT; ++rt) {
          const float4 a = *reinterpret_cast<const float4*>(arow + rt * 16 * SA + 16 * (ts.c_lo + u));
          f32x4& c = (u & 1) ? c1[rt] : c0[rt];
          c = __builtin_amdgcn_mfma_f32_16x16x4f32(B[j].x, a.x, c, 0, 0, 0);
          c = __builtin_amdgcn_mfma_f32_16x16x4f32(B[j].y, a.y, c, 0, 0, 0);
          c = __builtin_amdgcn_mfma_f32_16x16x4f32(B[j].z, a.z, c, 0, 0, 0);
          c = __builtin_amdgcn_mfma_f32_16x16x4f32(B[j].w, a.w, c, 0, 0, 0);
        }
      }
    }
  }
#pragma unroll
  for (int rt = 0; rt < RT; ++rt) tp[rt] = c0[rt] + c1[rt];
}

}

template <int D, bool QR>
__global__ void __launch_bounds__(kNTH) __attribute__((amdgpu_waves_per_eu(4)))
fwd32_kernel(FwdArgs p) {
  constexpr int RPT = (kRows * 48 + kNTH - 1) / kNTH;
  extern __shared__ __attribute__((aligned(16))) float smem[];
  const int tid = threadIdx.x;
  const int lane = tid & 63;
  const int wave = __builtin_amdgcn_readfirstlane(tid >> 6);
  const int F = p.F;
  const int num = p.num;
  const int SX = p.SX;
  const int flags = p.flags;
  const int Fp = r4(F);
  const Lds32 L = lds32_layout(F, D, p.MT, p.S, SX);
  float* buf = smem + L.buf;
  float* fs = smem + L.fs;
  float* dsum = smem + L.dsum;
  FieldDev* desc = reinterpret_cast<FieldDev*>(smem + L.desc);
  float* lw_s = smem + L.lw;
  float* fwlw_s = smem + L.fwlw;
  float* upk = smem + L.upk;
  float* fo = smem + L.fo;
  float* part2 = smem + L.part2;
  float* tailr = smem + L.tailr;
  float* taild = smem + L.taild;
  const TileRef tr = tile_ref<kRows>(p);
  const int64_t b0 = tr.b0;
  stamp(p.stamps, 0, tid);
  stamp_start_rt(p.stamps, tid);
  if (flags & kPrio) __builtin_amdgcn_s_setprio(1);
  const int g = wave;

  LayerStream<kTPW, 1, kNG> ls;
  f32x4 wb0[kTPW], wb1[kTPW], wb2[kTPW];
  const __amdgpu_buffer_rsrc_t wrsrc = __builtin_amdgcn_make_buffer_rsrc(
      const_cast<float4*>(p.wpack), (short)0, p.wpack_bytes, 0x00020000);
  const __amdgpu_buffer_rsrc_t brsrc = __builtin_amdgcn_make_buffer_rsrc(
      const_cast<float*>(p.mlp_b), (short)0, p.H * p.NT * 16 * 4, 0x00020000);
  const __amdgpu_buffer_rsrc_t frsrc = __builtin_amdgcn_make_buffer_rsrc(
      const_cast<float*>(p.fc), (short)0, p.NT * 16 * 4, 0x00020000);
  TailStream<kNG> ts;
  constexpr int TT = kNG * kTPW;

  typedef uint32_t u32x2 __attribute__((ext_vector_type(2)));
  constexpr int kDescPT = (7 * 64 + kNTH - 1) / kNTH;
  constexpr int kUpkPT = (kMaxMT * 16 * 16 + kNTH - 1) / kNTH;
  constexpr int kFwlwPT = (64 * 32 + kNTH - 1) / kNTH;
  u32x2 dw[QR ? kDescPT : 1];
  const float* rd_emb2[QR ? 1 : RPT];
  const float* rd_emb1[QR ? 1 : RPT];
  int64_t rd_n[QR ? 1 : RPT];
  bool pkrow[QR ? 1 : RPT];
  if constexpr (!QR) {
#pragma unroll
    for (int k = 0; k < RPT; ++k) {
      const int f = (tid + k * kNTH) >> 5;
      rd_emb2[k] = rd_emb1[k] = nullptr;
      rd_n[k] = 0;
      pkrow[k] = p.pkw != 0 && f >= num && f < F;
      if (f < F) {
        rd_emb2[k] = pkrow[k] ? p.pk[f] : p.fields[f].emb2;
        rd_emb1[k] = p.fields[f].emb1;
        rd_n[k] = p.fields[f].n;
      }
    }
  } else {
#pragma unroll
    for (int k = 0; k < kDescPT; ++k) {
      const int i = tid + k * kNTH;
      if (i < 7 * F) dw[k] = reinterpret_cast<const u32x2*>(p.fields)[i];
    }
  }
  int64_t key[RPT];
#pragma unroll
  for (int k = 0; k < RPT; ++k) {
    const int r = tid + k * kNTH;
    const int f = r >> 5;
    const int64_t gb = b0 + (r & 31);
    key[k] = 0;
    if (f < F && gb < p.batch) {
      if (f < num)
        key[k] = __float_as_int(tr.xv[gb * p.xv_stride + f]);
      else
        key[k] = tr.xi[gb * p.xi_stride + (f - num)];
    }
  }
  f32x4 uw[kUpkPT];
  const int n_upk = (flags & kHasSecond) ? p.MT * p.S * 16 : 0;
#pragma unroll
  for (int k = 0; k < kUpkPT; ++k) {
    const int i = tid + k * kNTH;
    if (i < n_upk) uw[k] = reinterpret_cast<const f32x4*>(p.upack)[i];
  }
  float fw[kFwlwPT];
  const int n_fwlw = (flags & kFoFwlw) ? F * D : 0;
#pragma unroll
  for (int k = 0; k < kFwlwPT; ++k) {
    const int i = tid + k * kNTH;
// ... 24 lines not shown
#pragma unroll
    for (int k = 0; k < RPT; ++k) {
      const int r = tid + k * kNTH;
      const int f = r >> 5;
      live[k] = f < F && (b0 + (r & 31)) < p.batch;
      pa[k] = qa[k] = nullptr;
      if constexpr (QR) pb[k] = qb[k] = nullptr;
      scale[k] = 1.f;
      mode[k] = 0;
      if (!live[k]) continue;
      if constexpr (!QR) {
        if (f < num) {
          scale[k] = __int_as_float((int)key[k]);
          pa[k] = rd_emb2[k];
          qa[k] = rd_emb1[k];
        } else {
          int64_t idx = key[k];
          if (idx < 0 || idx >= rd_n[k]) {
            atomicOr(p.err, DFWFM_FLAG_INDEX_OUT_OF_RANGE);
            idx = 0;
          }
          if (pkrow[k]) {
            pa[k] = rd_emb2[k] + idx * p.pkw;
          } else {
            pa[k] = rd_emb2[k] + idx * D;
            if (fo_tab) qa[k] = rd_emb1[k] + idx;
          }
        }
      } else {
        const FieldDev fd = desc[f];
        if (f < num) {
          scale[k] = __int_as_float((int)key[k]);
          pa[k] = fd.emb2;
          qa[k] = fd.emb1;
        } else {
          int64_t idx = key[k];
          if (idx < 0 || idx >= fd.n) {
            atomicOr(p.err, DFWFM_FLAG_INDEX_OUT_OF_RANGE);
            idx = 0;
          }
          if (fd.c == 0) {
            pa[k] = fd.emb2 + idx * D;
            if (fo_tab) qa[k] = fd.emb1 + idx;
          } else {
            const int64_t q = idx / fd.c;
            const int64_t rr = idx - q * fd.c;
            mode[k] = fd.op == 0 ? 1 : 2;
            pa[k] = fd.emb2 + q * D;
            pb[k] = fd.emb2_r + rr * D;
            if (fo_tab) {
              qa[k] = fd.emb1 + q;
              qb[k] = fd.emb1_r + rr;
            }
          }
        }
      }
    }
    float va[RPT][D], vb[RQ][D], fa[RPT], fb[RQ];
#pragma unroll
    for (int k = 0; k < RPT; ++k) {
      fa[k] = 0.f;
#pragma unroll
      for (int d = 0; d < D; ++d) va[k][d] = 0.f;
      if constexpr (QR) {
        fb[k] = 0.f;
#pragma unroll
        for (int d = 0; d < D; ++d) vb[k][d] = 0.f;
      }
      if (!QR && live[k] && pkrow[QR ? 0 : k]) {
        load_row_fo<D>(va[k], fa[k], pa[k]);
      } else {
        if (live[k] && needE) {
          load_row<D>(va[k], pa[k]);
          if constexpr (QR)
            if (mode[k] != 0) load_row<D>(vb[k], pb[k]);
        }
        if (live[k] && fo_tab) {
          fa[k] = *qa[k];
          if constexpr (QR)
            if (mode[k] != 0) fb[k] = *qb[k];
        }
      }
    }
    ls.init(wrsrc, 0, p.NC0, p.NT, g, 0);
    ls.preload(wb0, wb1, lane * 16);
#pragma unroll
    for (int k = 0; k < kUpkPT; ++k) {
      const int i = tid + k * kNTH;
      if (i < n_upk) reinterpret_cast<f32x4*>(upk)[i] = uw[k];
    }
#pragma unroll
    for (int k = 0; k < kFwlwPT; ++k) {
      const int i = tid + k * kNTH;
      if (i < n_fwlw) fwlw_s[i] = fw[k];
    }
    if ((flags & kFoLw) && tid < F) lw_s[tid] = lwv;
    const int w = p.W0 - F * D;
    for (int i = tid; i < kRows * w; i += kNTH) {
      const int b = i / w;
      buf[b * SX + F * D + (i - b * w)] = 0.f;
    }
#pragma unroll
    for (int k = 0; k < RPT; ++k) {
      const int r = tid + k * kNTH;
      const int f = r >> 5;
      const int b = r & 31;
      if (f < F) {
        if (needE) {
          float e[D];
#pragma unroll
          for (int d = 0; d < D; ++d) e[d] = live[k] ? combine(mode[k], va[k][d], QR ? vb[k][d] : 0.f, scale[k]) : 0.f;
          store_row<D>(buf + b * SX + f * D, e);
        }
        fo[b * Fp + f] = live[k] ? combine(mode[k], fa[k], QR ? fb[k] : 0.f, scale[k]) : 0.f;
      }
    }
  }
  __syncthreads();
  stamp(p.stamps, 2, tid);

  if (flags & kFoFwlw) {
    for (int r = tid; r < kRows * F; r += kNTH) {
      const int f = r >> 5;
      const int b = r & 31;
      const float* e = buf + b * SX + f * D;
      const float* w = fwlw_s + f * D;
      float s = 0.f;
#pragma unroll
      for (int d = 0; d < D; ++d) s += e[d] * w[d];
      fo[b * Fp + f] = s;
    }
  }
  stamp(p.stamps, 9, tid);
  if (flags & kHasSecond) {
    const int S = p.S;
    const int MTD = p.MT * D;
    const int p_lo = p.fw_off8[wave], p_hi = p.fw_off8[wave + 1];
    for (int pi = p_lo; pi < p_hi; ++pi) {
      const int pc = p.fw_list8[pi];
      const int m = pc / D;
      const int nt = pc - m * D;
      const int n = nt * 16 + (lane & 15);
      const int b = n / D;
      const float* ecol0 = buf + b * SX + (n - b * D);
      const float* ecol1 = ecol0 + 16 * SX;
      const float* ua = upk + m * S * 64 + lane;
      f32x4 acc0 = f32x4{0.f, 0.f, 0.f, 0.f}, acc1 = acc0;
      auto group = [&](int s0, auto U_) {
        constexpr int U = decltype(U_)::value;
        float av[U], bv0[U], bv1[U];
#pragma unroll
        for (int u = 0; u < U; ++u) {
          const int l = (4 * (s0 + u) + (lane >> 4)) * D;
          av[u] = ua[(s0 + u) * 64];
          bv0[u] = ecol0[l];
          bv1[u] = ecol1[l];
        }
        __builtin_amdgcn_sched_barrier(0);
#pragma unroll
        for (int u = 0; u < U; ++u) {
          acc0 = __builtin_amdgcn_mfma_f32_16x16x4f32(av[u], bv0[u], acc0, 0, 0, 0);
          acc1 = __builtin_amdgcn_mfma_f32_16x16x4f32(av[u], bv1[u], acc1, 0, 0, 0);
        }
      };
      int s0 = 4 * m;
      for (; s0 + 4 <= S; s0 += 4) group(s0, std::integral_constant<int, 4>{});
      const int rem = S - s0;
      if (rem == 3) group(s0, std::integral_constant<int, 3>{});
      else if (rem == 2) group(s0, std::integral_constant<int, 2>{});
      else if (rem == 1) group(s0, std::integral_constant<int, 1>{});
      float v0 = 0.f, v1 = 0.f;
#pragma unroll
      for (int r = 0; r < 4; ++r) {
        const int k = 16 * m + 4 * (lane >> 4) + r;
        const int kk = (k < F ? k : 0) * D;
        v0 = fmaf(k < F ? ecol0[kk] : 0.f, acc0[r], v0);
        v1 = fmaf(k < F ? ecol1[kk] : 0.f, acc1[r], v1);
      }
      v0 += __shfl_xor(v0, 16);
      v1 += __shfl_xor(v1, 16);
      v0 += __shfl_xor(v0, 32);
      v1 += __shfl_xor(v1, 32);
      if (lane < 16) {
        part2[pc * 16 + lane] = v0;
        part2[(MTD + pc) * 16 + lane] = v1;
      }
    }
  }
  stamp(p.stamps, 10, tid);
  __syncthreads();
  stamp(p.stamps, 11, tid);
  {
    const int b = wave * 4 + (lane >> 4);
    const int h = b >> 4;
    const int bl = b & 15;
    const int q = lane & 15;
    float first = 0.f, second = 0.f;
    for (int f0 = 0; f0 < F; f0 += 64) {
      float x[4], l[4];
#pragma unroll
      for (int k = 0; k < 4; ++k) {
        const int f = min(f0 + 16 * k + q, F - 1);
        x[k] = fo[b * Fp + f];
        l[k] = (flags & kFoLw) ? lw_s[f] : 1.f;
      }
#pragma unroll
      for (int k = 0; k < 4; ++k) first = f0 + 16 * k + q < F ? fmaf(x[k], l[k], first) : first;
    }
    if (flags & kHasSecond) {
      const int MT = p.MT;
      for (int d = q; d < D; d += 16) {
        const int n = bl * D + d;
        const float* pp = part2 + (h * MT * D + (n >> 4)) * 16 + (n & 15);
        float v[4];
#pragma unroll
        for (int m = 0; m < 4; ++m) v[m] = pp[min(m, MT - 1) * D * 16];
#pragma unroll
        for (int m = 0; m < 4; ++m) second += m < MT ? v[m] : 0.f;
        for (int m = 4; m < MT; ++m) second += pp[m * D * 16];
      }
    }
    first = sum16(first);
    second = sum16(second);
    if (q == 0) fs[b] = first + second;
  }
  stamp(p.stamps, 3, tid);
  if (flags & kPrio) __builtin_amdgcn_s_setprio(0);

  auto load_bias = [&](f32x4 (&bq)[kTPW], int h, int nq) {
#pragma unroll
    for (int j = 0; j < kTPW; ++j) {
      int t = g + kNG * j;
      t = t < p.NT ? t : p.NT - 1;
      bq[j] = __builtin_bit_cast(f32x4, __builtin_amdgcn_raw_buffer_load_b128(
                                            brsrc, nq * 4, __builtin_amdgcn_readfirstlane((h * p.NT + t) * 64), 0));
    }
  };
  f32x4 bq[kTPW];
  load_bias(bq, 0, 4 * (lane >> 4));
  int layer_off = 0;
  for (int h = 0; h < p.H; ++h) {
    int lv = lane;
    asm volatile("" : "+v"(lv));
    const int rowl = lv & 15;
    const int nq = 4 * (lv >> 4);
    const int NC = h == 0 ? p.NC0 : p.NT;
    const bool last = h == p.H - 1;
    const int boff = __builtin_amdgcn_readfirstlane((h * p.NT + TT) * 64 + (g & 3) * 4);
    const int ntail = TT * 16 + nq + (g & 3);
    const float bn_t = __builtin_bit_cast(float, __builtin_amdgcn_raw_buffer_load_b32(brsrc, nq * 4, boff, 0));

    f32x4 acc[kRT][kTPW];
#pragma unroll
    for (int rt = 0; rt < kRT; ++rt)
#pragma unroll
      for (int j = 0; j < kTPW; ++j) acc[rt][j] = bq[j];
    ts.init(layer_off, NC, TT, g);
    f32x4 tp[kRT];
    k_loop_rt<kTPW, kRT, kNG, kNS>(acc, buf, SX, ls, wb0, wb1, wb2, lane, ts, tp, h > 0 && (flags & kDeferTail));
    if (flags & kPrioEpi) __builtin_amdgcn_s_setprio(1);
    if (h == 0) stamp(p.stamps, 12, tid);
    __syncthreads();
#pragma unroll
    for (int rt = 0; rt < kRT; ++rt) reinterpret_cast<f32x4*>(tailr)[(g * kRT + rt) * 64 + lane] = tp[rt];
    float dpart[kRT] = {0.f, 0.f};
#pragma unroll
    for (int rt = 0; rt < kRT; ++rt) {
      float* orow = buf + (rt * 16 + rowl) * SX + nq;
#pragma unroll
      for (int j = 0; j < kTPW; ++j) {
        const int t = g + kNG * j;
        float v[4];
#pragma unroll
        for (int r = 0; r < 4; ++r) v[r] = relu_keep_nan(acc[rt][j][r]);
        if (!last) {
          *reinterpret_cast<f32x4*>(orow + t * 16) = f32x4{v[0], v[1], v[2], v[3]};
        } else {
          const f32x4 wf = __builtin_bit_cast(f32x4, __builtin_amdgcn_raw_buffer_load_b128(frsrc, nq * 4, t * 64, 0));
          dpart[rt] = fmaf(v[0], wf[0], dpart[rt]);
          dpart[rt] = fmaf(v[1], wf[1], dpart[rt]);
          dpart[rt] = fmaf(v[2], wf[2], dpart[rt]);
          dpart[rt] = fmaf(v[3], wf[3], dpart[rt]);
        }
      }
    }
    if (last) {
#pragma unroll
      for (int rt = 0; rt < kRT; ++rt) {
        float d = dpart[rt];
        d += __shfl_xor(d, 16);
        d += __shfl_xor(d, 32);
        if (lane < 16) dsum[g * kRows + rt * 16 + rowl] = d;
      }
    }
    layer_off += p.NT * NC * 64;
    if (!last) {
      ls.init(wrsrc, layer_off, p.NT, p.NT, g, 0);
      ls.preload(wb0, wb1, lane * 16);
      load_bias(bq, h + 1, nq);
    }
    if (h == 0) stamp(p.stamps, 13, tid);
    __syncthreads();
    if (g < 4) {
      const bool valid = ntail < p.N;
      float wf_t = 0.f;
      if (last)
        wf_t = __builtin_bit_cast(float, __builtin_amdgcn_raw_buffer_load_b32(
                                             frsrc, nq * 4, __builtin_amdgcn_readfirstlane(TT * 64 + g * 4), 0));
#pragma unroll
      for (int rt = 0; rt < kRT; ++rt) {
        const float* tpp = tailr + (rt * 64 + lane) * 4 + g;
        float sum = tpp[0];
#pragma unroll
        for (int w = 1; w < kNG; ++w) sum += tpp[w * kRT * 256];
        const float v = valid ? relu_keep_nan(sum + bn_t) : 0.f;
        if (!last) {
          buf[(rt * 16 + rowl) * SX + TT * 16 + nq + g] = v;
        } else {
          float c = v * wf_t;
          c += __shfl_xor(c, 16);
          c += __shfl_xor(c, 32);
          if (lane < 16) taild[g * kRows + rt * 16 + rowl] = c;
        }
      }
    }
    if (last || !(flags & kDeferTail)) __syncthreads();
    if (flags & kPrioEpi) __builtin_amdgcn_s_setprio(0);
    stamp(p.stamps, 4 + (h < 3 ? h : 3), tid);
  }

  if (tid < kRows && b0 + tid < p.batch) {
    float deepv = dsum[tid];
#pragma unroll
    for (int w = 1; w < kNG; ++w) deepv += dsum[w * kRows + tid];
    deepv += ((taild[tid] + taild[kRows + tid]) + taild[2 * kRows + tid]) + taild[3 * kRows + tid];
    tr.out[b0 + tid] = (fs[tid] + deepv) + p.bias[0];
  }
  stamp(p.stamps, 8, tid);
  stamp_end_rt(p.stamps, tid);
}

size_t fwd32_lds_bytes(int F, int D, int MT, int S, int SX) {
  return sizeof(float) * (size_t)lds32_layout(F, D, MT, S, SX).total;
}

bool fwd32_supported(int F, int D, int H, int NT, int NC0, int tailI, int NG) {
  return D == 10 && F <= 48 && H >= 1 && NT == kNS && NC0 == kNS && tailI == 1 && NG == kNG;
}

hipError_t launch_fwd32(const FwdArgs& a, int D, size_t lds, hipStream_t s) {
  if (D != 10) return hipErrorInvalidValue;
  auto k = (a.flags & kHasQR) ? fwd32_kernel<10, true> : fwd32_kernel<10, false>;
  hipError_t e = ensure_lds_limit(reinterpret_cast<const void*>(k), lds);
  if (e != hipSuccess) return e;
  const unsigned grid = fwd_grid(a, kRows);
  hipLaunchKernelGGL(k, dim3(grid), dim3(kNTH), lds, s, a);
  return hipGetLastError();
}

}
```

xsdeepfwfm_deprecated_amd/csrc/dfwfm_internal.h:

```cpp
#pragma once
#include <hip/hip_runtime.h>
#include <stdint.h>
#include <stdlib.h>
#include <string.h>

#include <mutex>
#include <unordered_map>

#include "../../include/dfwfm.h"

namespace dfwfm {

constexpr int kBM = 16;
constexpr int kMaxTPW = 8;
constexpr int kMaxMT = 4;
constexpr int kStampSlots = 16;
constexpr int kTailC = 8;
constexpr int kMaxPieces = kMaxMT * 32;

constexpr int kHasSecond = 1;
constexpr int kHasDeep = 2;
constexpr int kFoTables = 4;
constexpr int kFoFwlw = 8;
constexpr int kFoLw = 16;
constexpr int kNeedE = 32;
constexpr int kTrain = 64;
constexpr int kDrop = 128;
constexpr int kPrio = 256;
constexpr int kHasQR = 512;
constexpr int kPrioEpi = 2048;
constexpr int kDeferTail = 4096;
constexpr int kPairs = 1024;
constexpr int kP3Pieces = 8192;
constexpr int kBwdNoGStore = 1 << 20, kBwdNoMask = 1 << 21, kBwdGeneric = 1 << 22;
constexpr int kFtDiagHwId = 1 << 23, kFtDiagNoMlp = 1 << 24;
constexpr int kMaxH = 16;
constexpr int kMaxSet = 32;

struct FieldDev {
  const float* emb2;
  const float* emb2_r;
  const float* emb1;
  const float* emb1_r;
  int64_t n;
  int64_t c;
  int32_t op;
  int32_t reserved;
};
static_assert(sizeof(FieldDev) == sizeof(dfwfm_field_tables), "descriptor layout");
static_assert(sizeof(FieldDev) == 56, "descriptor is 7 x 8 bytes in LDS");

struct FwdArgs {
  const FieldDev* fields;
  const int64_t* xi;
  int64_t xi_stride;
  const float* xv;
  int64_t xv_stride;
  int64_t batch;
  float* out;
  int32_t* err;
  const float* const* pk;
  int32_t pkw;
  const float* upack;
  const int2* pairs;
  int32_t npairs;
  const float* fwlw;
  const float* lw;
  const float* bias;
  const float4* wpack;
  int32_t wpack_bytes;
  const float* mlp_b;
  const float* fc;
  int32_t F, num, H, N;
  int32_t NT, NC0;
  int32_t MT, S;
  int32_t SX, SY;
  int32_t W0;
  int32_t tail;
  int32_t ns;
  int32_t flags;
  uint64_t* stamps;
  float* sv_e;
  float* sv_fo;
  float* sv_x[kMaxH + 1];
  float drop_p;
  float drop_scale;
  uint32_t seed;
  const int64_t* seed_src;
  int32_t* sv_keys;
  int64_t keys_stride;
  float* part_e;
  float* part_fs;
  int32_t part_stride;
  uint8_t fw_list4[kMaxPieces];
  uint8_t fw_list8[kMaxPieces];
  uint8_t fw_off4[5];
  uint8_t fw_off8[9];
  int32_t nb;
  int32_t tiles;
  const int64_t* set_xi[kMaxSet];
  const float* set_xv[kMaxSet];
  float* set_out[kMaxSet];
};

inline unsigned fwd_grid(const FwdArgs& a, int rows) {
  const unsigned tiles = (unsigned)((a.batch + rows - 1) / rows);
  return a.nb > 1 ? (unsigned)a.nb * tiles : tiles;
}

inline int diag_opt(const char* key, int dflt) {
  const char* s = getenv("DFWFM_DIAG");
  const size_t kl = strlen(key);
  while (s && *s) {
    if (!strncmp(s, key, kl) && s[kl] == '=') return atoi(s + kl + 1);
    s = strchr(s, ',');
    if (s) ++s;
  }
  return dflt;
}

struct LdsLayout {
  int desc, lw, fwlw, upk, bufX, bufY, red, tailr, fo, part2, dsum, fs, total;
};

__host__ __device__ inline int r4(int x) { return (x + 3) & ~3; }

__host__ __device__ inline LdsLayout lds_layout(int F, int D, int MT, int S, int SX, int SY, int TPW, int KS,
                                                bool deep, bool tail, int NG = 4, bool p3 = false, bool fwlw = true) {
  LdsLayout L;
  int o = 0;
  L.desc = o;  o += r4(14 * F);
  L.lw = o;    o += r4(F);
  L.fwlw = o;  o += (p3 && !fwlw) ? 0 : r4(F * D);
  L.upk = o;   o += p3 ? 0 : MT * S * 64;
  L.bufX = o;  o += kBM * SX;
  L.bufY = o;  o += deep ? kBM * SY : 0;
  L.red = o;   o += (deep && KS == 2) ? 4 * TPW * 64 * 4 : 0;
  L.tailr = o; o += (deep && tail) ? NG * 64 * 4 + 4 * kBM : 0;
  L.fo = o;    o += kBM * r4(F);
  L.part2 = o; o += p3 ? kBM * D : MT * D * 16;
  L.dsum = o;  o += p3 ? 0 : NG * kBM;
  L.fs = o;    o += kBM;
  L.total = r4(o);
  return L;
}

struct BwdArgs {
  int64_t batch;
  const float* dlogit;
  const float* bce_z;
  const float* bce_y;
  float* bce_dl;
  float* loss_sum;
  float bce_denom;
  const float* sv_e;
  const float* sv_x[kMaxH + 1];
  float* sv_g[kMaxH + 1];
  float* sv_de;
  const float* rsk;
  const float* fwlw;
  const float* lw;
  const float* fc;
  const float4* wtpack;
// ... 219 lines not shown
};

struct AdamTensor {
  float* p;
  const float* g;
  float* m;
  float* v;
  int64_t n;
};
constexpr int kAdamBlock = 4096;
constexpr int kAdamList = 91;
struct AdamList {
  AdamTensor t[kAdamList];
  int32_t block0[kAdamList];
  int32_t n;
};
static_assert(sizeof(AdamList) + 64 <= 4096, "Adam launch arguments over 4 KiB");

inline hipError_t ensure_lds_limit(const void* fn, size_t lds) {
  if (lds <= 65536) return hipSuccess;
  static std::mutex mu;
  static std::unordered_map<const void*, size_t> granted;
  std::lock_guard<std::mutex> g(mu);
  size_t& cur = granted[fn];
  if (lds <= cur) return hipSuccess;
  hipError_t e = hipFuncSetAttribute(fn, hipFuncAttributeMaxDynamicSharedMemorySize, (int)lds);
  if (e == hipSuccess) cur = lds;
  return e;
}

enum PackType : int32_t { kPackPad = 0, kPackLinear = 1, kPackLinearT = 2, kPackFwfm = 3, kPackFwfmSym = 4, kPackZero = 5 };
constexpr int kPackZeroPT = 16;
struct PackJob {
  const float* src;
  float* dst;
  int64_t total;
  int32_t type;
  int32_t a, b, d;
  int32_t block0;
  int32_t pad_;
};
constexpr int kPackList = 56;
struct PackList {
  PackJob j[kPackList];
  int32_t n;
};

struct PruneSrc {
  const float* p;
  int64_t numel;
  int64_t offset;
  int32_t sym_f;
  int32_t pad_;
};
constexpr int kMaxPruneSrc = 96;
struct PruneList {
  PruneSrc s[kMaxPruneSrc];
  int32_t n;
};
size_t prune_workspace_bytes(int64_t n);
hipError_t launch_prune_threshold(const PruneList& L, double target, double* d_thr, void* ws, size_t ws_bytes,
                                  hipStream_t s);
hipError_t launch_prune_apply(float* p, int64_t numel, int sym_f, const double* d_thr, hipStream_t s);

size_t metrics_workspace_bytes(int64_t n);
hipError_t launch_metrics(const float* z, const float* y, int64_t n, double* out, void* ws, size_t ws_bytes,
                          hipStream_t s);

bool supported_embedding_size(int D);
hipError_t launch_forward(const FwdArgs& a, int D, int tpw, int ks, int ng, size_t lds, hipStream_t s);

constexpr int kPackTabList = 64;
struct PackTabList {
  const float* emb2[kPackTabList];
  const float* emb1[kPackTabList];
  float* dst[kPackTabList];
  int64_t n[kPackTabList];
  int32_t blk0[kPackTabList + 1];
  int32_t nf, D, pkw;
};
hipError_t launch_pack_tables(const PackTabList& L, hipStream_t s);
hipError_t launch_forward_gather(const FwdArgs& a, int D, size_t lds1, hipStream_t s);
hipError_t launch_pack_list(const PackList& L, int total_blocks, hipStream_t s);
bool fwd32_supported(int F, int D, int H, int NT, int NC0, int tailI, int NG);
size_t fwd32_lds_bytes(int F, int D, int MT, int S, int SX);
hipError_t launch_fwd32(const FwdArgs& a, int D, size_t lds, hipStream_t s);
bool ftrain_supported(int F, int D, int H, int NT, int NC0, int tailI, int NG);
size_t ftrain_lds_bytes(int F, int D, int MT, int S, int SX, int SY);
hipError_t launch_ftrain(const FwdArgs& a, int D, size_t lds, hipStream_t s);
#define DFWFM_PER_D_CAT2(a, b) a##b
#define DFWFM_PER_D_CAT(a, b) DFWFM_PER_D_CAT2(a, b)
#define DFWFM_PER_D(name) DFWFM_PER_D_CAT(name, DFWFM_KD)
#define DFWFM_DECL_PER_D(D)                                                                                   \
  hipError_t launch_forward_d##D(const FwdArgs& a, int tpw, int ks, int ng, size_t lds, hipStream_t s);        \
  hipError_t launch_forward_gather_d##D(const FwdArgs& a, size_t lds1, hipStream_t s);                      \
  hipError_t launch_backward_d##D(const BwdArgs& a, int tpw, int ng, size_t lds, hipStream_t s);
DFWFM_DECL_PER_D(4)
DFWFM_DECL_PER_D(8)
DFWFM_DECL_PER_D(10)
DFWFM_DECL_PER_D(16)
DFWFM_DECL_PER_D(32)
hipError_t launch_backward(const BwdArgs& a, int D, int tpw, int ng, size_t lds, hipStream_t s);
size_t backward_lds_bytes(int F, int D, int MT, int S, int SX, int SY);
hipError_t launch_dw(const DwArgs& a, int total_blocks, hipStream_t s);
hipError_t launch_dw_reduce(const DwArgs& a, int total_blocks, const RedArgs& r, hipStream_t s);
constexpr int kDwEdge = 80;
constexpr int kDwRows = 64;
hipError_t launch_reduce(const RedArgs& a, hipStream_t s);
hipError_t launch_reduce_final(const RedArgs& a, hipStream_t s);
hipError_t launch_scatter(const ScatterArgs& a, int total_blocks, hipStream_t s);
hipError_t launch_sort_scatter(const SortScatterArgs& a, int total_blocks, hipStream_t s);
hipError_t launch_adam(const AdamList& list, int total_blocks, float step_size, float omb1, float b2, float omb2,
                       float eps, float wd, float bc2_sqrt, hipStream_t s);
struct AdamDevState {
  int64_t step;
  float step_size, omb1, b2, omb2, eps, wd, bc2_sqrt;
  int32_t ticket;
  int32_t pad[2];
};
constexpr int kAdamGrid = 2048;
struct AdamHyper {
  double lr, b1, b2, eps, wd;
};
hipError_t launch_adam_dev(const AdamList& list, int total_blocks, AdamDevState* st, const AdamHyper& h, bool bump,
                           hipStream_t s);
hipError_t launch_bce_grad(const float* z, const float* y, int64_t n, float denom, float* dz, float* loss_sum,
                           hipStream_t s);

}
```

xsdeepfwfm_deprecated_amd/csrc/dfwfm_kernels.hip:

```cpp
#include <hip/hip_runtime.h>
#include <stdint.h>
#include <stdlib.h>

#include <type_traits>

#include "dfwfm_device.h"
#include "dfwfm_internal.h"

namespace dfwfm {

#ifndef DFWFM_FWD_WPE
#define DFWFM_FWD_WPE 2
#endif
#ifndef DFWFM_P3_WPE
#define DFWFM_P3_WPE 6
#endif
#ifndef DFWFM_P3_DIRECT_DESC
#define DFWFM_P3_DIRECT_DESC 1
#endif
#ifndef DFWFM_DIRECT_DESC_DEEP
#define DFWFM_DIRECT_DESC_DEEP 1
#endif
#ifndef DFWFM_P3_WPE4
#define DFWFM_P3_WPE4 5
#endif
template <int D, int TPW, int KS, bool TRAIN, int PART, int NG, int NS, bool QR = true>
__global__ void __launch_bounds__(64 * NG * KS)
__attribute__((amdgpu_waves_per_eu(PART == 1 ? 3 : (PART == 3 ? (NG == 4 ? DFWFM_P3_WPE4 : DFWFM_P3_WPE)
                                                               : (NG == 8 ? (TRAIN ? 2 : 4) : DFWFM_FWD_WPE)))))
fwd_kernel(FwdArgs p) {
  static_assert(NG == 4 || (NG == 8 && KS == 1), "8 tile groups: no K split");
  constexpr int NTH = 64 * NG * KS;
  constexpr int NW = NG * KS;
  constexpr int RPT = (kBM * 64 + NTH - 1) / NTH;
  extern __shared__ __attribute__((aligned(16))) float smem[];
  const int tid = threadIdx.x;
  const int lane = tid & 63;
  const int wave = __builtin_amdgcn_readfirstlane(tid >> 6);
  const int F = p.F;
  const int num = p.num;
  const int SX = p.SX;
  const int SY = p.SY;
  const int flags = p.flags;
  const bool deep = PART != 1 && PART != 3 && (flags & kHasDeep) != 0;
  const int Fp = r4(F);
  const bool tail = KS == 1 && p.tail != 0;
  const LdsLayout L = lds_layout(F, D, p.MT, p.S, SX, SY, TPW, KS, deep, tail, NG, PART == 3,
                                 (flags & kFoFwlw) != 0);
  FieldDev* desc = reinterpret_cast<FieldDev*>(smem + L.desc);
  float* lw_s = smem + L.lw;
  float* fwlw_s = smem + L.fwlw;
  float* upk = smem + L.upk;
  float* bufX = smem + L.bufX;
  float* bufY = smem + L.bufY;
  f32x4* red = reinterpret_cast<f32x4*>(smem + L.red);
  float* tailr = smem + L.tailr;
  float* fo = smem + L.fo;
  float* part2 = smem + L.part2;
  float* dsum = smem + L.dsum;
  float* fs = smem + L.fs;

  const TileRef tr = tile_ref<kBM>(p);
  const int64_t b0 = tr.b0;
  stamp(p.stamps, 0, tid);
  stamp_start_rt(p.stamps, tid);
  if (flags & kPrio) __builtin_amdgcn_s_setprio(1);
  const int g = wave & (NG - 1);
  const int kh = wave / NG;

  LayerStream<TPW, KS, NG> ls;
  f32x4 wb0[TPW], wb1[TPW], wb2[TPW];
#define DFWFM_PRELOAD(LS) (LS).preload(wb0, wb1, lane * 16)
#define DFWFM_KLOOP(ACC, IN, SA, LS) mlp_k_loop<TPW, KS, NG>(ACC, IN, SA, LS, wb0, wb1, wb2, lane)
  const __amdgpu_buffer_rsrc_t wrsrc = __builtin_amdgcn_make_buffer_rsrc(
      const_cast<float4*>(p.wpack), (short)0, p.wpack_bytes, 0x00020000);
  const __amdgpu_buffer_rsrc_t brsrc = __builtin_amdgcn_make_buffer_rsrc(
      const_cast<float*>(p.mlp_b), (short)0, p.H * p.NT * 16 * 4, 0x00020000);
  const __amdgpu_buffer_rsrc_t frsrc = __builtin_amdgcn_make_buffer_rsrc(
      const_cast<float*>(p.fc), (short)0, p.NT * 16 * 4, 0x00020000);
  TailStream<NG> ts;
  constexpr int NSK = PART == 3 ? 0 : NS;
  f32x4 tw[NSK ? 1 : TailStream<NG>::C];
  constexpr int TT = NG * TPW;

  constexpr bool train = TRAIN;
  const int FD = F * D;
  const int SE = r4(FD);
  const int nrows = (int)((p.batch - b0) < kBM ? (p.batch - b0) : kBM);
  const bool drop0 = train && deep && (flags & kDrop) != 0;
  {
  constexpr int kDescPT = (7 * 64 + NTH - 1) / NTH;
  constexpr int kUpkPT = (kMaxMT * 16 * 16 + NTH - 1) / NTH;
  constexpr int kFwlwPT = (64 * 32 + NTH - 1) / NTH;
  typedef uint32_t u32x2 __attribute__((ext_vector_type(2)));
  constexpr bool kDirectDesc = !QR && ((DFWFM_P3_DIRECT_DESC && PART == 3) || (DFWFM_DIRECT_DESC_DEEP && PART == 0));
  u32x2 dw[kDirectDesc ? 1 : kDescPT];
  const float* rd_emb2[kDirectDesc ? RPT : 1];
  const float* rd_emb1[kDirectDesc ? RPT : 1];
  int64_t rd_n[kDirectDesc ? RPT : 1];
  constexpr bool kPackable = (PART == 3 || (PART == 0 && !TRAIN)) && !QR && kDirectDesc;
  bool pkrow[kPackable ? RPT : 1];
  if constexpr (kDirectDesc) {
#pragma unroll
    for (int k = 0; k < RPT; ++k) {
      const int f = (tid + k * NTH) >> 4;
      rd_emb2[k] = rd_emb1[k] = nullptr;
      rd_n[k] = 0;
      if constexpr (kPackable) pkrow[k] = p.pkw != 0 && f >= num && f < F;
      if (f < F) {
        rd_emb2[k] = (kPackable && pkrow[kPackable ? k : 0]) ? p.pk[f] : p.fields[f].emb2;
        rd_emb1[k] = p.fields[f].emb1;
        rd_n[k] = p.fields[f].n;
      }
    }
  } else {
#pragma unroll
    for (int k = 0; k < kDescPT; ++k) {
      const int i = tid + k * NTH;
      if (i < 7 * F) dw[k] = reinterpret_cast<const u32x2*>(p.fields)[i];
    }
  }
  int64_t key[RPT];
#pragma unroll
  for (int k = 0; k < RPT; ++k) {
    const int r = tid + k * NTH;
    const int f = r >> 4;
    const int64_t gb = b0 + (r & 15);
    key[k] = 0;
    if (f < F && gb < p.batch) {
      if (f < num)
        key[k] = __float_as_int(tr.xv[gb * p.xv_stride + f]);
      else
        key[k] = tr.xi[gb * p.xi_stride + (f - num)];
    }
  }
  f32x4 uw[kUpkPT];
  const int n_upk = (PART != 3 && (flags & kHasSecond)) ? p.MT * p.S * 16 : 0;
#pragma unroll
  for (int k = 0; k < kUpkPT; ++k) {
    const int i = tid + k * NTH;
    if (i < n_upk) uw[k] = reinterpret_cast<const f32x4*>(p.upack)[i];
  }
  float fw[kFwlwPT];
// ... 51 lines not shown
#pragma unroll
    for (int k = 0; k < RPT; ++k) {
      const int r = tid + k * NTH;
      const int f = r >> 4;
      live[k] = f < F && (b0 + (r & 15)) < p.batch;
      pa[k] = qa[k] = nullptr;
      if constexpr (QR) pb[k] = qb[k] = nullptr;
      scale[k] = 1.f;
      mode[k] = 0;
      if (kDirectDesc && live[k]) {
        if (f < num) {
          scale[k] = __int_as_float((int)key[k]);
          pa[k] = rd_emb2[kDirectDesc ? k : 0];
          qa[k] = rd_emb1[kDirectDesc ? k : 0];
        } else {
          int64_t idx = key[k];
          if (idx < 0 || idx >= rd_n[kDirectDesc ? k : 0]) {
            atomicOr(p.err, DFWFM_FLAG_INDEX_OUT_OF_RANGE);
            idx = 0;
          }
          if (kPackable && pkrow[kPackable ? k : 0]) {
            pa[k] = rd_emb2[kDirectDesc ? k : 0] + idx * p.pkw;
          } else {
            pa[k] = rd_emb2[kDirectDesc ? k : 0] + idx * D;
            if (fo_tab) qa[k] = rd_emb1[kDirectDesc ? k : 0] + idx;
          }
        }
      } else if (live[k]) {
        const FieldDev fd = desc[f];
        if (f < num) {
          scale[k] = __int_as_float((int)key[k]);
          pa[k] = fd.emb2;
          qa[k] = fd.emb1;
        } else {
          int64_t idx = key[k];
          if (idx < 0 || idx >= fd.n) {
            atomicOr(p.err, DFWFM_FLAG_INDEX_OUT_OF_RANGE);
            idx = 0;
          }
          if (!QR || fd.c == 0) {
            pa[k] = fd.emb2 + idx * D;
            if (fo_tab) qa[k] = fd.emb1 + idx;
          } else if constexpr (QR) {
            const int64_t q = idx / fd.c;
            const int64_t rr = idx - q * fd.c;
            mode[k] = fd.op == 0 ? 1 : 2;
            pa[k] = fd.emb2 + q * D;
            pb[k] = fd.emb2_r + rr * D;
            if (fo_tab) {
              qa[k] = fd.emb1 + q;
              qb[k] = fd.emb1_r + rr;
            }
          }
        }
      }
    }
    float va[RPT][D], vb[RQ][D], fa[RPT], fb[RQ];
#pragma unroll
    for (int k = 0; k < RPT; ++k) {
      fa[k] = 0.f;
#pragma unroll
      for (int d = 0; d < D; ++d) va[k][d] = 0.f;
      if constexpr (QR) {
        fb[k] = 0.f;
#pragma unroll
        for (int d = 0; d < D; ++d) vb[k][d] = 0.f;
      }
      if (kPackable && live[k] && pkrow[kPackable ? k : 0]) {
        load_row_fo<D>(va[k], fa[k], pa[k]);
      } else {
        if (live[k] && needE) {
          load_row<D>(va[k], pa[k]);
          if constexpr (QR)
            if (mode[k] != 0) load_row<D>(vb[k], pb[k]);
        }
        if (live[k] && fo_tab) {
          fa[k] = *qa[k];
          if constexpr (QR)
            if (mode[k] != 0) fb[k] = *qb[k];
        }
      }
    }
    if (deep) {
      ls.init(wrsrc, 0, p.NC0, p.NT, g, kh);
      DFWFM_PRELOAD(ls);
    }
    if constexpr (!QR)
      if (!(flags & kPairs) && !(kPieces && (flags & kP3Pieces))) load_uu();
#pragma unroll
    for (int k = 0; k < kUpkPT; ++k) {
      const int i = tid + k * NTH;
      if (i < n_upk) reinterpret_cast<f32x4*>(upk)[i] = uw[k];
    }
#pragma unroll
    for (int k = 0; k < kFwlwPT; ++k) {
      const int i = tid + k * NTH;
      if (i < n_fwlw) fwlw_s[i] = fw[k];
    }
    if ((flags & kFoLw) && tid < F) lw_s[tid] = lwv;
    const int w = p.W0 - F * D;
    for (int i = tid; i < kBM * w; i += NTH) {
      const int b = i / w;
      bufX[b * SX + F * D + (i - b * w)] = 0.f;
    }
#pragma unroll
    for (int k = 0; k < RPT; ++k) {
      const int r = tid + k * NTH;
      const int f = r >> 4;
      const int b = r & 15;
      if (f < F) {
        if (needE) {
          float e[D];
#pragma unroll
          for (int d = 0; d < D; ++d) e[d] = live[k] ? combine(mode[k], va[k][d], QR ? vb[k][d] : 0.f, scale[k]) : 0.f;
          store_row<D>(bufX + b * SX + f * D, e);
        }
        fo[b * Fp + f] = live[k] ? combine(mode[k], fa[k], QR ? fb[k] : 0.f, scale[k]) : 0.f;
      }
    }
  }
  __syncthreads();
  stamp(p.stamps, 2, tid);
  if constexpr (PART == 1 || PART == 3) {
    if (PART == 1 || p.part_e)
      store_tile(p.part_e + b0 * p.part_stride, p.part_stride, bufX, SX, nrows, p.part_stride >> 2, tid, NTH);
  }
  if constexpr (train) {
    if (drop0 || !deep) store_tile(p.sv_e + b0 * SE, SE, bufX, SX, nrows, SE / 4, tid, NTH);
  }

  if (flags & kFoFwlw) {
    for (int r = tid; r < kBM * F; r += NTH) {
      const int f = r >> 4;
      const int b = r & 15;
      const float* e = bufX + b * SX + f * D;
      const float* w = fwlw_s + f * D;
      float s = 0.f;
#pragma unroll
      for (int d = 0; d < D; ++d) s += e[d] * w[d];
      fo[b * Fp + f] = s;
    }
  }
  stamp(p.stamps, 9, tid);
  if constexpr (PART == 3) {
    if ((flags & kHasSecond) && (flags & kPairs)) {
      constexpr int LPS = NTH / kBM;
      const int b = tid / LPS, j = tid % LPS;
      const float* eb = bufX + b * SX;
      float part = 0.f;
      for (int q = j; q < p.npairs; q += LPS) {
        const int2 pr = p.pairs[q];
        const float* ek = eb + (pr.x & 0xffff) * D;
        const float* el = eb + (pr.x >> 16) * D;
        float dot = 0.f;
#pragma unroll
        for (int d = 0; d < D; ++d) dot = fmaf(ek[d], el[d], dot);
        part = fmaf(__int_as_float(pr.y), dot, part);
      }
#pragma unroll
      for (int o = LPS / 2; o >= 1; o >>= 1) part += __shfl_xor(part, o);
      if (j == 0) part2[b] = part;
    } else if ((flags & kHasSecond) && kPieces && (flags & kP3Pieces)) {
      constexpr int MTC = P3_MTC;
      constexpr int SMAX = 4 * MTC;
      const int MT = p.MT, S = p.S;
      float uf[MTC][SMAX];
      {
        const float* up = p.upack;
#pragma unroll
        for (int m = 0; m < MTC; ++m)
#pragma unroll
          for (int s = 0; s < SMAX; ++s)
            uf[m][s] = (m < MT && s >= 4 * m && s < S) ? up[(m * S + s) * 64 + lane] : 0.f;
      }
      for (int nt = wave; nt < D; nt += NW) {
        const int n = nt * 16 + (lane & 15);
        const int b = n / D;
        const int d = n - b * D;
        const float* ecol = bufX + b * SX + d;
        f32x4 acc[MTC];
#pragma unroll
        for (int m = 0; m < MTC; ++m) acc[m] = f32x4{0.f, 0.f, 0.f, 0.f};
#pragma unroll
        for (int s0 = 0; s0 < SMAX; s0 += 4) {
          float bv[4];
#pragma unroll
          for (int u = 0; u < 4; ++u) {
            const int s = s0 + u;
            bv[u] = s < S ? ecol[(4 * s + (lane >> 4)) * D] : 0.f;
          }
#pragma unroll
          for (int u = 0; u < 4; ++u)
#pragma unroll
            for (int m = 0; m < MTC; ++m)
              if (4 * m <= s0 + u && s0 + u < S && m < MT)
                acc[m] = __builtin_amdgcn_mfma_f32_16x16x4f32(uf[m][s0 + u], bv[u], acc[m], 0, 0, 0);
        }
        float colv = 0.f;
#pragma unroll
        for (int m = 0; m < MTC; ++m) {
#pragma unroll
          for (int r = 0; r < 4; ++r) {
            const int k = 16 * m + 4 * (lane >> 4) + r;
            colv = fmaf(k < F ? ecol[(k < F ? k : 0) * D] : 0.f, acc[m][r], colv);
          }
        }
        colv += __shfl_xor(colv, 16);
        colv += __shfl_xor(colv, 32);
        if (lane < 16) part2[n] = colv;
      }
    } else if (flags & kHasSecond) {
      constexpr int SD = (D + 3) / 4;
      constexpr int MTC = P3_MTC;
      constexpr int NTL = P3_NTL;
      const int MT = p.MT;
      if constexpr (QR) load_uu();
      for (int b = wave; b < kBM; b += NW) {
        float ev[MTC][SD];
#pragma unroll
        for (int m = 0; m < MTC; ++m)
#pragma unroll
          for (int s = 0; s < SD; ++s) {
            const int k = 16 * m + (lane & 15);
            const int d = 4 * s + (lane >> 4);
            ev[m][s] = (m < MT && k < F && d < D) ? bufX[b * SX + k * D + d] : 0.f;
          }
        f32x4 acc[NTL];
#pragma unroll
        for (int t = 0; t < NTL; ++t) acc[t] = f32x4{0.f, 0.f, 0.f, 0.f};
#pragma unroll
        for (int s = 0; s < SD; ++s)
#pragma unroll
          for (int m = 0, t = 0; m < MTC; ++m)
#pragma unroll
            for (int n = m; n < MTC; ++n, ++t)
              if (n < MT) acc[t] = __builtin_amdgcn_mfma_f32_16x16x4f32(ev[m][s], ev[n][s], acc[t], 0, 0, 0);
        float part = 0.f;
#pragma unroll
        for (int t = 0; t < NTL; ++t)
#pragma unroll
          for (int r = 0; r < 4; ++r) part = fmaf(uu[t][r], acc[t][r], part);
#pragma unroll
        for (int o = 32; o >= 1; o >>= 1) part += __shfl_xor(part, o);
        if (lane == 0) part2[b] = part;
      }
    }
  } else if (flags & kHasSecond) {
    const int S = p.S;
    const uint8_t* plist = NW == 8 ? p.fw_list8 : p.fw_list4;
    const int p_lo = NW == 8 ? p.fw_off8[wave] : p.fw_off4[wave];
    const int p_hi = NW == 8 ? p.fw_off8[wave + 1] : p.fw_off4[wave + 1];
    for (int pi = p_lo; pi < p_hi; ++pi) {
      const int pc = plist[pi];
      const int m = pc / D;
      const int nt = pc - m * D;
      const int n = nt * 16 + (lane & 15);
      const int b = n / D;
      const float* ecol = bufX + b * SX + (n - b * D);
      const float* ua = upk + m * S * 64 + lane;
      f32x4 acc = f32x4{0.f, 0.f, 0.f, 0.f};
      auto group = [&](int s0, auto U_) {
        constexpr int U = decltype(U_)::value;
        float av[U], bv[U];
#pragma unroll
        for (int u = 0; u < U; ++u) {
          av[u] = ua[(s0 + u) * 64];
          bv[u] = ecol[(4 * (s0 + u) + (lane >> 4)) * D];
        }
        __builtin_amdgcn_sched_barrier(0);
#pragma unroll
        for (int u = 0; u < U; ++u) acc = __builtin_amdgcn_mfma_f32_16x16x4f32(av[u], bv[u], acc, 0, 0, 0);
      };
      int s0 = 4 * m;
      for (; s0 + 4 <= S; s0 += 4) group(s0, std::integral_constant<int, 4>{});
      const int rem = S - s0;
      if (rem == 3) group(s0, std::integral_constant<int, 3>{});
      else if (rem == 2) group(s0, std::integral_constant<int, 2>{});
      else if (rem == 1) group(s0, std::integral_constant<int, 1>{});
      float v = 0.f;
#pragma unroll
      for (int r = 0; r < 4; ++r) {
        const int k = 16 * m + 4 * (lane >> 4) + r;
        const float e = ecol[(k < F ? k : 0) * D];
        v = fmaf(k < F ? e : 0.f, acc[r], v);
      }
      v += __shfl_xor(v, 16);
      v += __shfl_xor(v, 32);
      if (lane < 16) part2[pc * 16 + lane] = v;
    }
  }
  if constexpr (NSK == 0) {
    if (deep && tail) {
      ts.init(0, p.NC0, TT, g);
      ts.load(wrsrc, tw, lane * 16);
    }
  }
  stamp(p.stamps, 10, tid);
  __syncthreads();
  stamp(p.stamps, 11, tid);
  if constexpr (train) {
    for (int i = tid; i < kBM * F; i += NTH) {
      const int b = i / F;
      if (b0 + b < p.batch) p.sv_fo[(b0 + b) * F + (i - b * F)] = fo[b * Fp + (i - b * F)];
    }
    if (drop0) {
      const uint32_t dseed = step_seed(p.seed, p.seed_src);
      for (int i = tid; i < kBM * FD; i += NTH) {
        const int b = i / FD;
        const int c = i - b * FD;
        const float v = bufX[b * SX + c];
        bufX[b * SX + c] = dropout_keep(dseed, 0, b0 + b, c, p.drop_p) ? v * p.drop_scale : 0.f;
      }
    }
  }
  if (wave < 4) {
    const int b = wave * 4 + (lane >> 4);
    const int q = lane & 15;
    float first = 0.f, second = 0.f;
    for (int f0 = 0; f0 < F; f0 += 64) {
      float x[4], l[4];
#pragma unroll
      for (int k = 0; k < 4; ++k) {
        const int f = min(f0 + 16 * k + q, F - 1);
        x[k] = fo[b * Fp + f];
        l[k] = (flags & kFoLw) ? lw_s[f] : 1.f;
      }
#pragma unroll
      for (int k = 0; k < 4; ++k) first = f0 + 16 * k + q < F ? fmaf(x[k], l[k], first) : first;
    }
    if (flags & kHasSecond) {
      if constexpr (PART == 3) {
        if (kPieces && (flags & kP3Pieces) && !(flags & kPairs)) {
          for (int d = q; d < D; d += 16) second += part2[b * D + d];
        } else {
          second = q == 0 ? part2[b] : 0.f;
        }
      } else {
        const int MT = p.MT;
        for (int d = q; d < D; d += 16) {
          const int n = b * D + d;
          const float* pp = part2 + (n >> 4) * 16 + (n & 15);
          float v[4];
#pragma unroll
          for (int m = 0; m < 4; ++m) v[m] = pp[min(m, MT - 1) * D * 16];
#pragma unroll
          for (int m = 0; m < 4; ++m) second += m < MT ? v[m] : 0.f;
          for (int m = 4; m < MT; ++m) second += pp[m * D * 16];
        }
      }
    }
    first = sum16(first);
    second = sum16(second);
    if (q == 0) fs[b] = first + second;
  }
  if (p.H < 4) stamp(p.stamps, 7, tid);

  if (!deep) {
    __syncthreads();
    if (PART == 1 || (PART == 3 && p.part_fs)) {
      if (tid < kBM && b0 + tid < p.batch) p.part_fs[b0 + tid] = fs[tid];
    } else {
      if (tid < kBM && b0 + tid < p.batch) tr.out[b0 + tid] = fs[tid] + p.bias[0];
    }
    stamp(p.stamps, 8, tid);
    stamp_end_rt(p.stamps, tid);
    return;
  }
  }

  stamp(p.stamps, 3, tid);
  if (flags & kPrio) __builtin_amdgcn_s_setprio(0);
  if constexpr (train) __syncthreads();
  const bool drop = train && (flags & kDrop) != 0;
  const uint32_t hseed = drop ? step_seed(p.seed, p.seed_src) : 0u;
  auto load_bias = [&](f32x4 (&bq)[TPW], int h, int nq) {
#pragma unroll
    for (int j = 0; j < TPW; ++j) {
      int t = g + NG * j;
      t = t < p.NT ? t : p.NT - 1;
      bq[j] = kh == 0 ? __builtin_bit_cast(f32x4, __builtin_amdgcn_raw_buffer_load_b128(
                            brsrc, nq * 4, __builtin_amdgcn_readfirstlane((h * p.NT + t) * 64), 0))
                      : f32x4{0.f, 0.f, 0.f, 0.f};
    }
  };
  f32x4 bq[TPW];
  load_bias(bq, 0, 4 * (lane >> 4));
  int layer_off = 0;
  for (int h = 0; h < p.H; ++h) {
    int lv = lane;
    asm volatile("" : "+v"(lv));
    const int rowl = lv & 15;
    const int nq = 4 * (lv >> 4);
    const bool even = (h & 1) == 0;
    const float* in = even ? bufX : bufY;
    const int SA = even ? SX : SY;
    float* outa = even ? bufY : bufX;
    const int SO = even ? SY : SX;
    const int NC = h == 0 ? p.NC0 : p.NT;
    const bool last = h == p.H - 1;
    const int boff = __builtin_amdgcn_readfirstlane((h * p.NT + TT) * 64 + (g & 3) * 4);
    const int ntail = TT * 16 + nq + (g & 3);
    const float bn_t = tail ? __builtin_bit_cast(float, __builtin_amdgcn_raw_buffer_load_b32(brsrc, nq * 4, boff, 0))
                            : 0.f;

    f32x4 acc[TPW];
#pragma unroll
    for (int j = 0; j < TPW; ++j) acc[j] = bq[j];
    if constexpr (NSK > 0) {
      if (tail) ts.init(layer_off, NC, TT, g);
      else ts.cnt = 0;
      f32x4 tp;
      mlp_k_loop_s<TPW, NG, NSK, true>(acc, in, SA, ls, wb0, wb1, wb2, lane, ts, tp);
      if (tail) reinterpret_cast<f32x4*>(tailr)[g * 64 + lane] = tp;
    } else {
      if (tail) reinterpret_cast<f32x4*>(tailr)[g * 64 + lane] = ts.template mma<true>(in, SA, tw, lane);
      mlp_k_loop<TPW, KS, NG, true, true>(acc, in, SA, ls, wb0, wb1, wb2, lane);
    }
    if (h == 0) stamp(p.stamps, 12, tid);
    if constexpr (KS == 2) {
      if (kh == 1) {
#pragma unroll
        for (int j = 0; j < TPW; ++j) red[(g * TPW + j) * 64 + lane] = acc[j];
      }
      __syncthreads();
      if (kh == 0) {
#pragma unroll
        for (int j = 0; j < TPW; ++j) acc[j] += red[(g * TPW + j) * 64 + lane];
      }
    }
    float dpart = 0.f;
    if (kh == 0) {
      float* orow = outa + rowl * SO + nq;
#pragma unroll
      for (int j = 0; j < TPW; ++j) {
        const int t = g + NG * j;
        if (t < p.NT) {
          float v[4];
          if (t * 16 + 16 <= p.N) {
#pragma unroll
            for (int r = 0; r < 4; ++r) v[r] = relu_keep_nan(acc[j][r]);
          } else {
#pragma unroll
            for (int r = 0; r < 4; ++r) v[r] = nq + r < p.N - t * 16 ? relu_keep_nan(acc[j][r]) : 0.f;
          }
          if constexpr (train) {
            if (drop) {
#pragma unroll
              for (int r = 0; r < 4; ++r)
                v[r] = dropout_keep(hseed, h + 1, b0 + rowl, t * 16 + nq + r, p.drop_p) ? v[r] * p.drop_scale : 0.f;
            }
          }
          if (!last || train) *reinterpret_cast<f32x4*>(orow + t * 16) = f32x4{v[0], v[1], v[2], v[3]};
          if (last) {
            const f32x4 wf =
                __builtin_bit_cast(f32x4, __builtin_amdgcn_raw_buffer_load_b128(frsrc, nq * 4, t * 64, 0));
            dpart = fmaf(v[0], wf[0], dpart);
            dpart = fmaf(v[1], wf[1], dpart);
            dpart = fmaf(v[2], wf[2], dpart);
            dpart = fmaf(v[3], wf[3], dpart);
          }
        }
      }
    }
    if (last && kh == 0) {
      dpart += __shfl_xor(dpart, 16);
      dpart += __shfl_xor(dpart, 32);
      if (lane < 16) dsum[g * kBM + rowl] = dpart;
    }
    layer_off += p.NT * NC * 64;
    if (!last) {
      ls.init(wrsrc, layer_off, p.NT, p.NT, g, kh);
      DFWFM_PRELOAD(ls);
      if constexpr (NSK == 0) {
        if (tail) {
          ts.init(layer_off, p.NT, TT, g);
          ts.load(wrsrc, tw, lane * 16);
        }
      }
      load_bias(bq, h + 1, nq);
    }
    if constexpr (train) {
      if (h == 0)
        store_tile(p.sv_x[0] + b0 * SE, SE, in, SA, nrows, SE / 4, tid, NTH);
      else
        store_tile(p.sv_x[h] + b0 * p.N, p.N, in, SA, nrows, p.N / 4, tid, NTH);
    }
    if (h == 0) stamp(p.stamps, 13, tid);
    __syncthreads();
    if (tail) {
      if (g < 4) {
        float* orow_t = outa + rowl * SO + nq;
        const bool valid = ntail < p.N;
        const float* tp = tailr + lane * 4 + g;
        float sum = tp[0];
#pragma unroll
        for (int w = 1; w < NG; ++w) sum += tp[w * 256];
        float v = valid ? relu_keep_nan(sum + bn_t) : 0.f;
        if constexpr (train) {
          if (drop) v = dropout_keep(hseed, h + 1, b0 + rowl, ntail, p.drop_p) ? v * p.drop_scale : 0.f;
          if (last) orow_t[TT * 16 + g] = v;
        }
        if (!last) {
          orow_t[TT * 16 + g] = v;
        } else {
          const float wf_t = __builtin_bit_cast(float, __builtin_amdgcn_raw_buffer_load_b32(
                                 frsrc, nq * 4, __builtin_amdgcn_readfirstlane(TT * 64 + g * 4), 0));
          float c = v * wf_t;
          c += __shfl_xor(c, 16);
          c += __shfl_xor(c, 32);
          if (lane < 16) tailr[NG * 64 * 4 + g * kBM + rowl] = c;
        }
      }
      if (!last) __syncthreads();
    }
    stamp(p.stamps, 4 + (h < 3 ? h : 3), tid);
  }

  if constexpr (train) {
    if (tail) __syncthreads();
    float* last_out = ((p.H - 1) & 1) == 0 ? bufY : bufX;
    const int SL = ((p.H - 1) & 1) == 0 ? SY : SX;
    store_tile(p.sv_x[p.H] + b0 * p.N, p.N, last_out, SL, nrows, p.N / 4, tid, NTH);
  }

  __syncthreads();
  if (tid < kBM && b0 + tid < p.batch) {
    float deepv = dsum[tid];
#pragma unroll
    for (int w = 1; w < NG; ++w) deepv += dsum[w * kBM + tid];
    if (tail) deepv += ((tailr[NG * 64 * 4 + tid] + tailr[NG * 64 * 4 + kBM + tid]) +
                        tailr[NG * 64 * 4 + 2 * kBM + tid]) + tailr[NG * 64 * 4 + 3 * kBM + tid];
    tr.out[b0 + tid] = (fs[tid] + deepv) + p.bias[0];
  }
  stamp(p.stamps, 8, tid);
  stamp_end_rt(p.stamps, tid);
}

#ifndef DFWFM_KD

__device__ __forceinline__ void pack_elem(const PackJob& j, int64_t i) {
  switch (j.type) {
    case kPackPad:
      j.dst[i] = (j.src && i < j.a) ? j.src[i] : 0.f;
      break;
    case kPackLinear:
    case kPackLinearT: {
      const int N = j.a, K = j.b, NC = j.d;
      const int lane = (int)(i & 63);
      const int64_t tc = i >> 6;
      const int c = (int)(tc % NC);
      const int t = (int)(tc / NC);
      const bool tr = j.type == kPackLinearT;
// ... 105 lines not shown
           : a.MT == 2 ? fwd_kernel<D, 1, 1, false, 3, NG, 2, Q>
           : a.MT == 3 ? fwd_kernel<D, 1, 1, false, 3, NG, 3, Q> : fwd_kernel<D, 1, 1, false, 3, NG, 4, Q>;
    };
    using I4 = std::integral_constant<int, 4>;
    using I8 = std::integral_constant<int, 8>;
    using T = std::true_type;
    using Fl = std::false_type;
    auto k = qr ? pick(I8{}, T{}) : (w8 ? pick(I8{}, Fl{}) : pick(I4{}, Fl{}));
    const int ng = w8 ? 8 : 4;
    const size_t lds3 = sizeof(float) * (size_t)lds_layout(a.F, D, a.MT, a.S, a.SX, a.SY, 1, 1, false, false, ng,
                                                            true, (a.flags & kFoFwlw) != 0).total;
    hipError_t e = ensure_lds_limit(reinterpret_cast<const void*>(k), lds3);
    if (e != hipSuccess) return e;
    hipLaunchKernelGGL(k, dim3(fwd_grid(a, kBM)), dim3(64 * ng), lds3, s, a);
    return hipGetLastError();
  }
  if (a.flags & kTrain) return ng == 8 ? launch_fwd_8<D, 0, true>(a, tpw, lds, s) : launch_fwd_k<D, 1, true>(a, tpw, lds, s);
  if (ng == 8) return launch_fwd_8<D, 0>(a, tpw, lds, s);
  return launch_fwd_k<D, 1, false>(a, tpw, lds, s);
}

#ifdef DFWFM_KD
hipError_t DFWFM_PER_D(launch_forward_d)(const FwdArgs& a, int tpw, int ks, int ng, size_t lds, hipStream_t s) {
  return launch_fwd_d<DFWFM_KD>(a, tpw, ks, ng, lds, s);
}
hipError_t DFWFM_PER_D(launch_forward_gather_d)(const FwdArgs& a, size_t lds1, hipStream_t s) {
  return launch_fwd_t<DFWFM_KD, 1, 1, false, 1, 4>(a, lds1, s);
}
#else
hipError_t launch_forward_gather(const FwdArgs& a, int D, size_t lds1, hipStream_t s) {
  switch (D) {
    case 4: return launch_forward_gather_d4(a, lds1, s);
    case 8: return launch_forward_gather_d8(a, lds1, s);
    case 10: return launch_forward_gather_d10(a, lds1, s);
    case 16: return launch_forward_gather_d16(a, lds1, s);
    case 32: return launch_forward_gather_d32(a, lds1, s);
    default: return hipErrorInvalidValue;
  }
}

bool supported_embedding_size(int D) { return D == 4 || D == 8 || D == 10 || D == 16 || D == 32; }

hipError_t launch_forward(const FwdArgs& a, int D, int tpw, int ks, int ng, size_t lds, hipStream_t s) {
  switch (D) {
    case 4: return launch_forward_d4(a, tpw, ks, ng, lds, s);
    case 8: return launch_forward_d8(a, tpw, ks, ng, lds, s);
    case 10: return launch_forward_d10(a, tpw, ks, ng, lds, s);
    case 16: return launch_forward_d16(a, tpw, ks, ng, lds, s);
    case 32: return launch_forward_d32(a, tpw, ks, ng, lds, s);
    default: return hipErrorInvalidValue;
  }
}

__global__ void __launch_bounds__(256) pack_tables_kernel(const PackTabList L) {
  int j = 0;
  while (j + 1 < L.nf && (int)blockIdx.x >= L.blk0[j + 1]) ++j;
  const int64_t r = (int64_t)((int)blockIdx.x - L.blk0[j]) * 256 + threadIdx.x;
  if (r >= L.n[j]) return;
  const float* e2 = L.emb2[j] + r * L.D;
  const float e1 = L.emb1[j][r];
  f32x4* dst = reinterpret_cast<f32x4*>(L.dst[j] + r * L.pkw);
  for (int q = 0; q < L.pkw / 4; ++q) {
    f32x4 v;
#pragma unroll
    for (int i = 0; i < 4; ++i) {
      const int e = 4 * q + i;
      v[i] = e < L.D ? e2[e] : (e == L.D ? e1 : 0.f);
    }
    dst[q] = v;
  }
}

hipError_t launch_pack_tables(const PackTabList& L, hipStream_t s) {
  if (L.nf <= 0 || L.blk0[L.nf] <= 0) return hipSuccess;
  hipLaunchKernelGGL(pack_tables_kernel, dim3(L.blk0[L.nf]), dim3(256), 0, s, L);
  return hipGetLastError();
}

hipError_t launch_pack_list(const PackList& L, int total_blocks, hipStream_t s) {
  if (total_blocks <= 0 || L.n <= 0) return hipSuccess;
  hipLaunchKernelGGL(pack_dense_kernel, dim3(total_blocks), dim3(256), 0, s, L);
  return hipGetLastError();
}
#endif

}
```

xsdeepfwfm_deprecated_amd/engine.py:

```python
from __future__ import annotations

import ctypes

import torch

from . import _lib


def _ptr(t):
    return None if t is None else ctypes.c_void_p(t.data_ptr())


def _stream_handle(device):
    return ctypes.c_void_p(torch.cuda.current_stream(device).cuda_stream)


def _require_f32_cuda(t, name, device):
    if t.dtype != torch.float32 or not t.is_cuda or t.device != device:
        raise RuntimeError(f"dfwfm: {name} must be a float32 tensor on {device}, got {t.dtype} on {t.device}")
    if not t.is_contiguous():
        raise RuntimeError(f"dfwfm: {name} must be contiguous")


def _require_rows(t, name, dtype, device, width):
    if t.dtype != dtype or t.device != device:
        raise ValueError(f"dfwfm: {name} must be a {dtype} tensor on {device}, got {t.dtype} on {t.device}")
    if t.dim() < 1 or t.shape[0] == 0 or width == 0:
        return
    inner = 1
    for d in range(t.dim() - 1, 0, -1):
        if t.shape[d] != 1 and t.stride(d) != inner:
            raise ValueError(f"dfwfm: {name} rows must be contiguous (got strides {tuple(t.stride())}); "
                             "pass .contiguous()")
        inner *= t.shape[d]
    if inner < width:
        raise ValueError(f"dfwfm: {name} has {inner} entries per row, the model needs {width}")


class ForwardEngine:

    def __init__(self, cfg: dict, device: torch.device):
        self.device = device
        self.cfg = dict(cfg)
        c = _lib.dfwfm_config(**{k: int(v) for k, v in cfg.items()})
        h = ctypes.c_void_p()
        L = _lib.lib()
        with torch.cuda.device(device):
            _lib.check(L.dfwfm_model_create(ctypes.byref(c), ctypes.byref(h)), "dfwfm_model_create")
        self.handle = h
        self._tables_key = None
        self._dense_key = None
        self._keep = None
        self.small_rows = 0
        self.bf16 = False

    def close(self):
        if self.handle is not None and self.handle.value:
            _lib.lib().dfwfm_model_destroy(self.handle)
        self.handle = None

    def __del__(self):
        try:
            self.close()
        except Exception:
            pass

    def sync_tables(self, fields):
        names = ("emb2", "emb2_r", "emb1", "emb1_r")
        key = tuple(tuple(None if f[nm] is None else f[nm].data_ptr() for nm in names) for f in fields)
        if key == self._tables_key:
            return
        arr = (_lib.dfwfm_field_tables * len(fields))()
        for i, f in enumerate(fields):
            for nm in ("emb2", "emb2_r", "emb1", "emb1_r"):
                if f[nm] is not None:
                    _require_f32_cuda(f[nm], f"field {i} {nm}", self.device)
            arr[i] = _lib.dfwfm_field_tables(
                *[None if f[nm] is None else f[nm].data_ptr() for nm in names],
                int(f["n"]), int(f["c"]), int(f["op"]), 0)
        _lib.check(_lib.lib().dfwfm_model_set_tables(self.handle, arr, len(fields),
                                                     _stream_handle(self.device)), "dfwfm_model_set_tables")
        self._packed_key = None
        self._keep = arr
        self._tables_key = key

    def sync_dense(self, field_cov, fwfm_lin, fm_1st, bias, lin_w, lin_b, fc_w):
        tensors = [field_cov, fwfm_lin, fm_1st, bias, fc_w] + list(lin_w) + list(lin_b)
        key = tuple(None if t is None else (t.data_ptr(), t._version) for t in tensors)
        if key == self._dense_key:
            return
        for i, t in enumerate(tensors):
            if t is not None:
                _require_f32_cuda(t, f"dense parameter {i}", self.device)
        H = len(lin_w)
        W = (ctypes.c_void_p * max(H, 1))(*[t.data_ptr() for t in lin_w])
        B = (ctypes.c_void_p * max(H, 1))(*[t.data_ptr() for t in lin_b])
        self.__dict__.pop("_ws_cache", None)
        self.invalidate_derived()
        _lib.check(_lib.lib().dfwfm_model_set_dense(
            self.handle, _ptr(field_cov), _ptr(fwfm_lin), _ptr(fm_1st), _ptr(bias),
            W if H else None, B if H else None, _ptr(fc_w), _stream_handle(self.device)),
            "dfwfm_model_set_dense")
        self._dense_key = key

    def invalidate_derived(self):
        self._pairs_key = None
        self._sparse_key = None
        self._bf16_key = None

    def sync_packed(self, tables, enable: bool = True) -> bool:
        key = (bool(enable),) + tuple((t.data_ptr(), t._version) for pair in tables for t in pair if t is not None)
        if key == getattr(self, "_packed_key", None):
            return self._packed_on
        en = ctypes.c_int32(0)
        _lib.check(_lib.lib().dfwfm_model_pack_tables(self.handle, int(bool(enable)), ctypes.byref(en),
                                                      _stream_handle(self.device)), "dfwfm_model_pack_tables")
        self._packed_on = bool(en.value)
        self._packed_key = key
        return self._packed_on

    def sync_pairs(self, max_pairs: int) -> bool:
        key = (self._dense_key, int(max_pairs))
        if key == getattr(self, "_pairs_key", None):
            return self._pairs_on
        en = ctypes.c_int32(0)
        _lib.check(_lib.lib().dfwfm_model_build_fwfm_pairs(self.handle, int(max_pairs), ctypes.byref(en),
                                                           _stream_handle(self.device)),
                   "dfwfm_model_build_fwfm_pairs")
        self._pairs_on = bool(en.value)
        self._pairs_key = key
        return self._pairs_on

    def sync_sparse(self, max_density: float) -> bool:
        key = (self._dense_key, float(max_density))
        if key == getattr(self, "_sparse_key", None):
            return self._sparse_on
        en = ctypes.c_int32(0)
        _lib.check(_lib.lib().dfwfm_model_build_sparse_mlp(self.handle, float(max_density), ctypes.byref(en),
                                                           _stream_handle(self.device)),
                   "dfwfm_model_build_sparse_mlp")
        self._sparse_on = bool(en.value)
        self._sparse_key = key
        self.__dict__.pop("_ws_cache", None)
        return self._sparse_on

    def sync_bf16(self, enable: bool = True) -> bool:
        key = (self._dense_key, bool(enable))
        if key == getattr(self, "_bf16_key", None):
            return bool(enable)
        _lib.check(_lib.lib().dfwfm_model_pack_bf16(self.handle, int(bool(enable)), _stream_handle(self.device)),
                   "dfwfm_model_pack_bf16")
        self._bf16_key = key
        return bool(enable)

    def forward(self, xi: torch.Tensor, xv: torch.Tensor, out: torch.Tensor | None = None) -> torch.Tensor:
        B = xi.shape[0]
        if self.bf16 and B > 0:
            return self.forward_bf16(xi, xv, out)
        if 0 < B <= self.small_rows:
            return self.forward_small(xi, xv, out)
        ncat = self.cfg["field_size"] - self.cfg["numerical"]
        num = self.cfg["numerical"]
        _require_rows(xi, "Xi", torch.int64, self.device, ncat)
        _require_rows(xv, "Xv", torch.float32, self.device, num)
        if out is None:
            out = torch.empty(B, dtype=torch.float32, device=self.device)
        xs = xi.stride(0) if ncat > 0 else 0
        vs = xv.stride(0) if num > 0 else 0
        ws_bytes = self._ws_bytes(B)
        ws = torch.empty(ws_bytes, dtype=torch.uint8, device=self.device) if ws_bytes else None
        rc = _lib.lib().dfwfm_forward_ws(self.handle, ctypes.c_void_p(xi.data_ptr()), xs,
                                         ctypes.c_void_p(xv.data_ptr()), vs, B,
                                         ctypes.c_void_p(out.data_ptr()), _ptr(ws), ws_bytes,
                                         _stream_handle(self.device))
        _lib.check(rc, "dfwfm_forward")
        return out

    def forward_small(self, xi: torch.Tensor, xv: torch.Tensor, out: torch.Tensor | None = None) -> torch.Tensor:
        B = xi.shape[0]
        ncat = self.cfg["field_size"] - self.cfg["numerical"]
        num = self.cfg["numerical"]
        _require_rows(xi, "Xi", torch.int64, self.device, ncat)
        _require_rows(xv, "Xv", torch.float32, self.device, num)
        if out is None:
            out = torch.empty(B, dtype=torch.float32, device=self.device)
        xs = xi.stride(0) if ncat > 0 else 0
        vs = xv.stride(0) if num > 0 else 0
        ws_bytes = self._serve_ws_bytes(B)
        ws = torch.empty(ws_bytes, dtype=torch.uint8, device=self.device) if ws_bytes else None
        rc = _lib.lib().dfwfm_serve_forward(self.handle, ctypes.c_void_p(xi.data_ptr()), xs,
                                            ctypes.c_void_p(xv.data_ptr()), vs, B,
# ... 265 lines not shown
```

xsdeepfwfm_deprecated_amd/training.py:

```python
from __future__ import annotations

import ctypes
import logging
import math
import os
from time import time

import numpy as np
import torch
import torch.nn.functional as F

from . import _lib
from . import engine as _engine


def _grad_buffer(params, need, device):
    sizes = [p.numel() if n else 0 for p, n in zip(params, need)]
    flat = torch.zeros(sum(sizes), dtype=torch.float32, device=device)
    views, off = [], 0
    for p, n, sz in zip(params, need, sizes):
        views.append(flat[off:off + sz].view_as(p) if n else None)
        off += sz
    return flat, views

# ... 550 lines not shown
        if (not batches or not self.use_graph or self.dist is not None or self.steps < 1
                or any(int(xi.shape[0]) != self.B for xi, _, _ in batches) or any(d is None for d in direct)):
            for xi, xv, y in batches:
                loss = self.step(xi, xv, y)
            return self.loss_sum if not batches else loss
        if not self._attached:
            raise RuntimeError("FusedTrainStep.step_many after close()")
        self.drop = self.drop_train if self.model.training else 0.0
        denom = float(self.B)
        key = ("many", denom, self.drop, self.deterministic, self._ws_generation(),
               tuple((t.data_ptr(), tuple(t.stride())) for d in direct for t in d))
        hit = self._many_sets.pop(key, None)
        if hit is None:
            if len(self._many_sets) >= self.max_many_sets:
                self._many_sets.pop(next(iter(self._many_sets)))
            s = torch.cuda.Stream(self.dev)
            s.wait_stream(torch.cuda.current_stream(self.dev))
            g = torch.cuda.CUDAGraph()
            s1 = torch.cuda.Stream(self.dev)
            with torch.cuda.stream(s):
                with torch.cuda.graph(g, stream=s, capture_error_mode="thread_local"):
                    for d in direct:
                        self._in = d
                        self._one_process_step(denom, s, s1)
            torch.cuda.current_stream(self.dev).wait_stream(s)
            hit = ((g, None, None, None, None), direct)
        self._many_sets[key] = hit
        hit[0][0].replay()
        self.steps += len(batches)
        self.eng._dense_key = None
        self.eng._packed_key = None
        self.eng.invalidate_derived()
        return self.loss_sum

    _graph_key = None
    _attached = False


def binary_search_threshold(param, target_percent, total_no):
    lo, hi = 0.0, 1e2
    mid = (lo + hi) / 2
    for _ in range(101):
        if not lo < hi:
            break
        mid = (lo + hi) / 2
        rate = (param.abs() < mid).sum().item() * 1.0 / total_no
        if abs(rate - target_percent) < 0.0001:
            return mid
        if rate > target_percent:
            hi = mid
        else:
            lo = mid
    return mid


class DevicePruner:

    def __init__(self, device):
        self.device = device
        self.ws = torch.empty(0, dtype=torch.uint8, device=device)
        self.thr = torch.zeros(1, dtype=torch.float64, device=device)
        self.L = _lib.lib()

    def _stream(self):
        return ctypes.c_void_p(torch.cuda.current_stream(self.device).cuda_stream)

    def threshold(self, sources, target):
        arr = (_lib.dfwfm_prune_source * len(sources))()
        total = 0
        for i, (t, sym) in enumerate(sources):
            if t.dtype != torch.float32 or not t.is_cuda or not t.is_contiguous():
                raise RuntimeError("dfwfm pruning: sources must be contiguous float32 HIP tensors")
            arr[i] = _lib.dfwfm_prune_source(t.data_ptr(), t.numel(), int(sym), 0)
            total += t.numel()
        need = int(self.L.dfwfm_prune_workspace_bytes(total))
        if self.ws.numel() < need:
            self.ws = torch.empty(need, dtype=torch.uint8, device=self.device)
        thr = torch.empty(1, dtype=torch.float64, device=self.device)
        _lib.check(self.L.dfwfm_prune_threshold(arr, len(sources), float(target), ctypes.c_void_p(thr.data_ptr()),
                                                ctypes.c_void_p(self.ws.data_ptr()), self.ws.numel(), self._stream()),
                   "dfwfm_prune_threshold")
        return thr

    def apply(self, t, thr, sym_f=0):
        _lib.check(self.L.dfwfm_prune_apply(ctypes.c_void_p(t.data_ptr()), t.numel(), int(sym_f),
                                            ctypes.c_void_p(thr.data_ptr()), self._stream()), "dfwfm_prune_apply")
        torch.autograd.graph.increment_version(t)


def prune_step(model, adaptive_sparse, prune_fm, prune_r, prune_deep, emb_r, emb_corr):
    dev = model._device()
    if dev.type == "cpu":
        return _prune_step_host(model, adaptive_sparse, prune_fm, prune_r, prune_deep, emb_r, emb_corr)
    if dev.type != "cuda":
        raise _lib.DfwfmError(f"pruning runs on a HIP device or the CPU, not on {dev}")
    pr = getattr(model, "_pruner", None)
    if pr is None or pr.device != dev:
        pr = model._pruner = DevicePruner(dev)
    with torch.no_grad():
        named = list(model.named_parameters())
        if prune_fm != 0:
            embs = [p.data for n, p in named if "fm_2nd_embeddings" in n]
            thr = pr.threshold([(e, 0) for e in embs], adaptive_sparse * emb_r)
            for e in embs:
                pr.apply(e, thr)
        for name, param in named:
            if "linear" in name and "weight" in name and prune_deep != 0:
                pr.apply(param.data, pr.threshold([(param.data, 0)], adaptive_sparse))
            if name == "field_cov.weight" and prune_r != 0:
                F_ = param.shape[0]
                pr.apply(param.data, pr.threshold([(param.data, F_)], adaptive_sparse * emb_corr), F_)


def _prune_step_host(model, adaptive_sparse, prune_fm, prune_r, prune_deep, emb_r, emb_corr):
    with torch.no_grad():
        named = list(model.named_parameters())
        if prune_fm != 0:
            embs = [p.data for n, p in named if "fm_2nd_embeddings" in n]
            flat = torch.cat([e.reshape(-1) for e in embs])
            thr = binary_search_threshold(flat, adaptive_sparse * emb_r, flat.numel())
            for e in embs:
                e[e.abs() < thr] = 0
        for name, param in named:
            if "linear" in name and "weight" in name and prune_deep != 0:
                thr = binary_search_threshold(param.data, adaptive_sparse, param.numel())
                param.data[param.data.abs() < thr] = 0
            if name == "field_cov.weight" and prune_r != 0:
                sym = (param.data + param.data.t()) * 0.5
                thr = binary_search_threshold(sym, adaptive_sparse * emb_corr, param.numel())
                param.data[sym.abs() < thr] = 0


def _dist():
    import torch.distributed as dist
    if dist.is_available() and dist.is_initialized() and dist.get_world_size() > 1:
        return dist
    return None


def allreduce_grads(model):
    dist = _dist()
    if dist is None:
        return
    params = [p for p in model.parameters() if p.grad is not None]
    flat = getattr(model, "_grad_flat", None)
    if flat is not None and params:
        lo, hi = flat.data_ptr(), flat.data_ptr() + flat.numel() * 4
        if all(lo <= p.grad.data_ptr() < hi for p in params):
            dist.all_reduce(flat)
            return
    grads = [p.grad for p in params]
    buf = torch._utils._flatten_dense_tensors(grads)
    dist.all_reduce(buf)
    for g, r in zip(grads, torch._utils._unflatten_dense_tensors(buf, grads)):
        g.copy_(r)


def make_optimizer(model):
    if model.optimizer_type == "adam":
        if model._device().type == "cpu":
            return torch.optim.Adam(model.parameters(), lr=model.learning_rate, weight_decay=model.weight_decay)
        return Adam(model.parameters(), lr=model.learning_rate, weight_decay=model.weight_decay)
    if model.optimizer_type == "rmsp":
        return torch.optim.RMSprop(model.parameters(), lr=model.learning_rate, weight_decay=model.weight_decay)
    if model.optimizer_type == "adag":
        return torch.optim.Adagrad(model.parameters(), lr=model.learning_rate, weight_decay=model.weight_decay)
    return torch.optim.SGD(model.parameters(), lr=model.learning_rate, momentum=model.momentum,
                           weight_decay=model.weight_decay)


def _param_summary(model, log, nonzero=False):
    tot = e1 = e2 = dnn = 0
    nz_r = 0
    for name, p in model.named_parameters():
        c = int((p != 0).sum().item()) if nonzero else p.numel()
        tot += c
        if "1st_embeddings" in name:
            e1 += c
        if "2nd_embeddings" in name:
            e2 += c
        if "linear_" in name:
            dnn += c
        if name == "field_cov.weight":
            nz_r = int((0.5 * (p.data + p.data.t()) != 0).sum().item())
    return tot, e1, e2, dnn, nz_r


def fit(model, Xi_train, Xv_train, y_train, Xi_valid=None, Xv_valid=None, y_valid=None, early_stopping=False,
        refit=False, save_path=None, prune=0, prune_fm=0, prune_r=0, prune_deep=0, emb_r=1., emb_corr=1.,
        teacher_model=None):
    log = model.logger
    device = model._device()
    if device.type not in ("cuda", "cpu"):
        from ._lib import DfwfmError
# ... 169 lines not shown
```

Measured before the change: 135.2 million.

## Fold numerical-field embeddings into first MLP layer weights for inference

```diff
diff --git a/include/dfwfm_fold.h b/include/dfwfm_fold.h
--- /dev/null
+++ b/include/dfwfm_fold.h
@@ -0,0 +1,23 @@
+#ifndef DFWFM_FOLD_H
+#define DFWFM_FOLD_H
+
+#include <stddef.h>
+#include <stdint.h>
+
+#include "dfwfm.h"
+
+#ifdef __cplusplus
+extern "C" {
+#endif
+
+#define DFWFM_FOLD_ABI_VERSION 1
+
+int dfwfm_fold_abi_version(void);
+
+int dfwfm_model_fold_numerical(dfwfm_model* m, int32_t enable, int32_t* enabled, void* stream);
+
+#ifdef __cplusplus
+}
+#endif
+
+#endif
diff --git a/xsdeepfwfm_deprecated_amd/DeepFMs.py b/xsdeepfwfm_deprecated_amd/DeepFMs.py
--- a/xsdeepfwfm_deprecated_amd/DeepFMs.py
+++ b/xsdeepfwfm_deprecated_amd/DeepFMs.py
@@ -79,6 +79,7 @@
         self.sparse_mlp_max_density = 0.0
         self.fwfm_pair_max = 0
         self.pack_tables = True
+        self.fold_numerical = True
         self.small_batch_rows = 0
         self.mlp_dtype = "f32"
         self.deterministic = True
@@ -227,6 +228,9 @@
                 d = self._field_desc(None if second is None else second[f], None if first is None else first[f])
                 tabs.append((d["emb2"], d["emb1"]))
             eng.sync_packed(tabs, self.pack_tables)
+            if self.use_deep:
+                eng.sync_fold([second[f].weight.detach() for f in range(self.num)],
+                              bool(getattr(self, "fold_numerical", True)))
             eng.small_rows = max(int(getattr(self, "small_batch_rows", 0)), 0) if self.use_deep else 0
             eng.bf16 = eng.sync_bf16(self._mlp_bf16()) if self.use_deep else False
         return eng
diff --git a/xsdeepfwfm_deprecated_amd/_lib.py b/xsdeepfwfm_deprecated_amd/_lib.py
--- a/xsdeepfwfm_deprecated_amd/_lib.py
+++ b/xsdeepfwfm_deprecated_amd/_lib.py
@@ -24,7 +24,8 @@
         u += [(s, f"{os.path.splitext(s)[0]}_d{d}.o", [f"-DDFWFM_KD={d}"]) for d in EMB_SIZES]
     return u
 HEADERS = ["dfwfm_internal.h", "dfwfm_device.h", os.path.join("..", "..", "include", "dfwfm.h"),
-           os.path.join("..", "..", "include", "dfwfm_serve.h"), os.path.join("..", "..", "include", "dfwfm_bf16.h")]
+           os.path.join("..", "..", "include", "dfwfm_serve.h"), os.path.join("..", "..", "include", "dfwfm_bf16.h"),
+           os.path.join("..", "..", "include", "dfwfm_fold.h")]
 ARCH = os.environ.get("DFWFM_OFFLOAD_ARCH", "gfx950")
 CPU_PATH = os.path.join(PKG_DIR, "libdfwfm_cpu.so")
 CPU_SOURCES = ["dfwfm_cpu.cpp"]
@@ -154,6 +155,11 @@
                                           ctypes.c_size_t, _P]),
 }
 
+FOLD_SIGNATURES = {
+    "dfwfm_fold_abi_version": (ctypes.c_int, []),
+    "dfwfm_model_fold_numerical": (ctypes.c_int, [_P, ctypes.c_int32, ctypes.POINTER(ctypes.c_int32), _P]),
+}
+
 _lib = None
 _lock = threading.Lock()
 
@@ -351,6 +357,12 @@
             fn.argtypes = args
         if L.dfwfm_bf16_abi_version() != 1:
             raise DfwfmError("libdfwfm bf16 ABI mismatch")
+        for name, (res, args) in FOLD_SIGNATURES.items():
+            fn = getattr(L, name)
+            fn.restype = res
+            fn.argtypes = args
+        if L.dfwfm_fold_abi_version() != 1:
+            raise DfwfmError("libdfwfm fold ABI mismatch")
         _lib = L
     return _lib
 
diff --git a/xsdeepfwfm_deprecated_amd/csrc/dfwfm_capi.hip b/xsdeepfwfm_deprecated_amd/csrc/dfwfm_capi.hip
--- a/xsdeepfwfm_deprecated_amd/csrc/dfwfm_capi.hip
+++ b/xsdeepfwfm_deprecated_amd/csrc/dfwfm_capi.hip
@@ -13,6 +13,7 @@
 #include "dfwfm_internal.h"
 #include "../../include/dfwfm_serve.h"
 #include "../../include/dfwfm_bf16.h"
+#include "../../include/dfwfm_fold.h"
 
 using namespace dfwfm;
 
@@ -61,6 +62,11 @@
   float* d_bias;
   uint16_t* d_wbf16;
   bool bf16_on;
+  int foldNC;
+  int foldSX, foldW0;
+  int foldSh;
+  size_t fold_lds_inf, fold_lds_r32;
+  bool fold_on;
   uint64_t* d_stamps;
   size_t stamps_cap;
   size_t stamps_ring;
@@ -278,6 +284,28 @@
     free_model(m);
     return fail(DFWFM_ERR_UNSUPPORTED, "LDS tile of %zu bytes exceeds 160 KiB", m->lds_bytes);
   }
+  if (c.use_deep && m->num > 0) {
+    const int KC = (F - m->num) * D;
+    const int nc = (KC + m->num + 15) / 16;
+    const bool st = m->NC0 == 25 && NT == 25;
+    const int ncp = st ? (nc <= kFoldNS ? kFoldNS : 25) : nc;
+    const int sh = (4 - (m->num * D) % 4) % 4;
+    const int w0 = 4 * m->S * D > m->num * D + ncp * 16 ? 4 * m->S * D : m->num * D + ncp * 16;
+    int sx = r4(sh + w0 > NT * 16 ? sh + w0 : NT * 16);
+    if (!((sx >> 2) & 1)) sx += 4;
+    const size_t l_inf = sizeof(float) * (size_t)lds_layout(F, D, m->MT, m->S, sx, m->SY, m->TPWI > 0 ? m->TPWI : 1, 1,
+                                                            true, m->tailI != 0, m->NG).total;
+    const size_t l_r32 = m->r32 ? fwd32_lds_bytes(F, D, m->MT, m->S, sx) : 0;
+    const bool fits = l_inf <= 160 * 1024 && l_r32 <= 160 * 1024 && !(m->lds_r32 <= 80 * 1024 && l_r32 > 80 * 1024);
+    if (fits && sh % 2 == 0) {
+      m->foldNC = ncp;
+      m->foldSX = sx;
+      m->foldW0 = w0;
+      m->foldSh = sh;
+      m->fold_lds_inf = l_inf;
+      m->fold_lds_r32 = l_r32;
+    }
+  }
 
   int rc = DFWFM_OK;
   if ((rc = dev_alloc(&m->d_fields, F)) || (rc = dev_alloc(&m->d_upack, (size_t)m->MT * m->S * 64)) ||
@@ -293,14 +321,15 @@
   }
   if (c.use_deep) {
     m->wpack_elems = (size_t)NT * m->NC0 * 64 + (size_t)(H - 1) * NT * NT * 64;
-    if (m->wpack_elems * sizeof(float4) >= (size_t)1 << 31) {
+    if ((m->wpack_elems + (size_t)NT * m->foldNC * 64) * sizeof(float4) >= (size_t)1 << 31) {
       free_model(m);
       return fail(DFWFM_ERR_UNSUPPORTED, "packed MLP weights exceed the 2 GiB buffer-descriptor range");
     }
     m->wtpack_elems = m->wpack_elems;
     m->wt_off[1] = 0;
     for (int l = 2; l <= H; ++l) m->wt_off[l] = m->wt_off[l - 1] + (l == 2 ? m->NC0 : NT) * NT * 64;
-    if ((rc = dev_alloc(&m->d_wtpack, m->wtpack_elems)) || (rc = dev_alloc(&m->d_wpack, m->wpack_elems)) ||
+    if ((rc = dev_alloc(&m->d_wtpack, m->wtpack_elems)) ||
+        (rc = dev_alloc(&m->d_wpack, m->wpack_elems + (size_t)NT * m->foldNC * 64)) ||
         (rc = dev_alloc(&m->d_mlp_b, (size_t)H * NT * 16)) || (rc = dev_alloc(&m->d_fc, (size_t)NT * 16))) {
       free_model(m);
       return rc;
@@ -347,6 +376,7 @@
     if (host[f].c > 0) host[f].n = (host[f].n + host[f].c - 1) / host[f].c * host[f].c;
   memcpy(m->h_fields, host, sizeof(FieldDev) * n);
   m->pkw = 0;
+  m->fold_on = false;
   m->flags &= ~kHasQR;
   for (int f = 0; f < n; ++f)
     if (host[f].c > 0) m->flags |= kHasQR;
@@ -423,6 +453,7 @@
   m->dense_set = true;
   m->sp = 0;
   m->bf16_on = false;
+  m->fold_on = false;
   m->flags &= ~kPairs;
   for (int h = 0; h < m->H; ++h) m->lin_w[h] = lin_w ? lin_w[h] : nullptr;
   return DFWFM_OK;
@@ -503,6 +534,16 @@
   memcpy(a.fw_off8, m->fw_off8, sizeof a.fw_off8);
 }
 
+void apply_fold(const dfwfm_model* m, FwdArgs& a) {
+  if (!m->fold_on) return;
+  a.wfold_off = (int32_t)m->wpack_elems;
+  a.wpack_bytes = (int32_t)((m->wpack_elems + (size_t)m->NT * m->foldNC * 64) * sizeof(float4));
+  a.NC0f = m->foldNC;
+  a.xsh = m->foldSh;
+  a.SX = m->foldSX;
+  a.W0 = m->foldW0;
+}
+
 int dw_plan(const dfwfm_model* m, int64_t batch, int* per_split, int64_t* splits, int64_t* rows,
             int64_t* cap = nullptr) {
   const int edge = kDwEdge, quantum = kDwRows;
@@ -646,9 +687,11 @@
   a.flags |= kPrio | kPrioEpi | kDeferTail;
   if ((rc = diag_stamps_buffer(m, batch, 1, &a.stamps)) != DFWFM_OK) return rc;
   a.tail = m->tailI;
+  apply_fold(m, a);
   const bool r32 = (a.flags & kHasDeep) && use_fwd32(m, batch, stream);
-  hipError_t e = r32 ? launch_fwd32(a, m->D, m->lds_r32, (hipStream_t)stream)
-                     : launch_forward(a, m->D, m->TPWI > 0 ? m->TPWI : 1, m->KS, m->NG, m->lds_inf, (hipStream_t)stream);
+  hipError_t e = r32 ? launch_fwd32(a, m->D, m->fold_on ? m->fold_lds_r32 : m->lds_r32, (hipStream_t)stream)
+                     : launch_forward(a, m->D, m->TPWI > 0 ? m->TPWI : 1, m->KS, m->NG,
+                                      m->fold_on ? m->fold_lds_inf : m->lds_inf, (hipStream_t)stream);
   if (e != hipSuccess) return hip_fail(e, "forward launch");
   return DFWFM_OK;
 }
@@ -681,6 +724,7 @@
     fill_forward_args(m, a, xi[i0], xi_stride, xv[i0], xv_stride, batch, out[i0]);
     a.flags |= kPrio | kPrioEpi | kDeferTail;
     a.tail = m->tailI;
+    apply_fold(m, a);
     if (n > 1) {
       a.nb = n;
       a.tiles = (int32_t)((batch + rows - 1) / rows);
@@ -692,9 +736,9 @@
     }
     int rc = diag_stamps_buffer(m, (int64_t)n * a.tiles * rows, 1, &a.stamps);
     if (rc != DFWFM_OK) return rc;
-    const hipError_t e = r32 ? launch_fwd32(a, m->D, m->lds_r32, (hipStream_t)stream)
-                             : launch_forward(a, m->D, m->TPWI > 0 ? m->TPWI : 1, m->KS, m->NG, m->lds_inf,
-                                              (hipStream_t)stream);
+    const hipError_t e = r32 ? launch_fwd32(a, m->D, m->fold_on ? m->fold_lds_r32 : m->lds_r32, (hipStream_t)stream)
+                             : launch_forward(a, m->D, m->TPWI > 0 ? m->TPWI : 1, m->KS, m->NG,
+                                              m->fold_on ? m->fold_lds_inf : m->lds_inf, (hipStream_t)stream);
     if (e != hipSuccess) return hip_fail(e, "batch-set forward launch");
   }
   return DFWFM_OK;
@@ -913,6 +957,39 @@
   ba.NC0 = m->NC0;
   e = launch_bf16_mlp(ba, (hipStream_t)stream);
   if (e != hipSuccess) return hip_fail(e, "bf16 MLP launch");
+  return DFWFM_OK;
+}
+
+int dfwfm_fold_abi_version(void) { return DFWFM_FOLD_ABI_VERSION; }
+
+int dfwfm_model_fold_numerical(dfwfm_model* m, int32_t enable, int32_t* enabled, void* stream) {
+  if (!m || !enabled) return fail(DFWFM_ERR_INVALID_ARG, "null argument");
+  *enabled = 0;
+  if (!enable) {
+    m->fold_on = false;
+    return DFWFM_OK;
+  }
+  if (!m->tables_set || !m->dense_set)
+    return fail(DFWFM_ERR_STATE, "set_tables and set_dense must precede fold_numerical");
+  if (m->foldNC == 0 || !m->lin_w[0] || diag_opt("fold", 1) == 0) {
+    m->fold_on = false;
+    return DFWFM_OK;
+  }
+  FoldPackArgs fa;
+  memset(&fa, 0, sizeof fa);
+  fa.w1 = m->lin_w[0];
+  fa.fields = m->d_fields;
+  fa.dst = m->d_wpack + m->wpack_elems;
+  fa.N = m->N;
+  fa.F = m->F;
+  fa.D = m->D;
+  fa.num = m->num;
+  fa.NT = m->NT;
+  fa.NC = m->foldNC;
+  hipError_t e = launch_pack_fold(fa, (hipStream_t)stream);
+  if (e != hipSuccess) return hip_fail(e, "fold pack launch");
+  m->fold_on = true;
+  *enabled = 1;
   return DFWFM_OK;
 }
 
diff --git a/xsdeepfwfm_deprecated_amd/csrc/dfwfm_fwd32.hip b/xsdeepfwfm_deprecated_amd/csrc/dfwfm_fwd32.hip
--- a/xsdeepfwfm_deprecated_amd/csrc/dfwfm_fwd32.hip
+++ b/xsdeepfwfm_deprecated_amd/csrc/dfwfm_fwd32.hip
@@ -1,5 +1,7 @@
 #include <hip/hip_runtime.h>
 #include <stdint.h>
+
+#include <type_traits>
 
 #include "dfwfm_device.h"
 #include "dfwfm_internal.h"
@@ -13,6 +15,8 @@
 constexpr int kNG = 8;
 constexpr int kTPW = 3;
 constexpr int kNS = 25;
+constexpr int kNSF = kFoldNS;
+static_assert(kNSF == kNS - 7, "k_loop_rt's folded form jumps over seven of the kNS steps");
 constexpr int kNTH = 64 * kNG;
 
 struct Lds32 {
@@ -52,30 +56,48 @@
       }
 }
 
+template <int B, int E, class Fn>
+__device__ __forceinline__ void static_for(Fn&& f) {
+  if constexpr (B < E) {
+    f(std::integral_constant<int, B>{});
+    static_for<B + 1, E>(f);
+  }
+}
+
+constexpr int kSkipAt = 3, kSkipMid = 6;
 template <int TPW, int RT, int NG, int NS>
 __device__ __forceinline__ void k_loop_rt(f32x4 (&acc)[RT][TPW], const float* __restrict__ act, int SA,
                                           const LayerStream<TPW, 1, NG>& ls, f32x4 (&b0)[TPW], f32x4 (&b1)[TPW],
                                           f32x4 (&b2)[TPW], int lane, const TailStream<NG>& ts, f32x4 (&tp)[RT],
-                                          bool mid_barrier) {
+                                          bool mid_barrier, bool skip) {
+  static_assert(kSkipMid % 3 == 0 && kSkipAt >= 2 && kSkipAt + kSkipMid + 2 < NS, "skipped steps keep the rotation");
   const int voff = lane * 16;
   const float* arow = act + (lane & 15) * SA + 4 * (lane >> 4);
+  const int sk = skip ? kSkipMid : 0;
+  const float* arow_s = arow - 16 * sk;
+  const int c_pen = skip ? NS - 2 - kSkipMid : NS - 1;
   float4 a0[RT], a1[RT], a2[RT];
 #pragma unroll
   for (int rt = 0; rt < RT; ++rt) {
     a0[rt] = *reinterpret_cast<const float4*>(arow + rt * 16 * SA);
     a1[rt] = *reinterpret_cast<const float4*>(arow + rt * 16 * SA + 16);
   }
-#pragma unroll
-  for (int i = 0; i < NS; ++i) {
+  auto step = [&](auto i_) __attribute__((always_inline)) {
+    constexpr int i = decltype(i_)::value;
     f32x4 (&X)[TPW] = (i % 3 == 0) ? b0 : ((i % 3 == 1) ? b1 : b2);
     f32x4 (&Z)[TPW] = (i % 3 == 0) ? b2 : ((i % 3 == 1) ? b0 : b1);
     float4 (&AX)[RT] = (i % 3 == 0) ? a0 : ((i % 3 == 1) ? a1 : a2);
     float4 (&AZ)[RT] = (i % 3 == 0) ? a2 : ((i % 3 == 1) ? a0 : a1);
     if (i + 3 == NS && mid_barrier) __syncthreads();
-    if (i + 2 < NS) {
-#pragma unroll
-      for (int rt = 0; rt < RT; ++rt) AZ[rt] = *reinterpret_cast<const float4*>(arow + rt * 16 * SA + 16 * (i + 2));
-      ls.load(Z, ls.c0 + i + 2, voff);
+    if constexpr (i + 3 == NS) {
+#pragma unroll
+      for (int rt = 0; rt < RT; ++rt) AZ[rt] = *reinterpret_cast<const float4*>(arow + rt * 16 * SA + 16 * c_pen);
+      ls.load(Z, ls.c0 + c_pen, voff);
+    } else if constexpr (i + 2 < NS) {
+      const float* ar = i + 2 >= kSkipAt + kSkipMid ? arow_s : arow;
+#pragma unroll
+      for (int rt = 0; rt < RT; ++rt) AZ[rt] = *reinterpret_cast<const float4*>(ar + rt * 16 * SA + 16 * (i + 2));
+      ls.load(Z, ls.c0 + i + 2 - (i + 2 >= kSkipAt + kSkipMid ? sk : 0), voff);
     } else {
       ts.template load_set<TPW>(ls.rsrc, Z, i + 2 == NS ? 0 : TPW, voff);
     }
@@ -87,7 +109,11 @@
     }
     __builtin_amdgcn_sched_group_barrier(0x008, 2 * RT * TPW, 0);
     __builtin_amdgcn_sched_barrier(0);
-  }
+  };
+  static_for<0, kSkipAt>(step);
+  if (!skip) static_for<kSkipAt, kSkipAt + kSkipMid>(step);
+  static_for<kSkipAt + kSkipMid, NS - 1>(step);
+  if (!skip) step(std::integral_constant<int, NS - 1>{});
   f32x4 c0[RT], c1[RT];
 #pragma unroll
   for (int rt = 0; rt < RT; ++rt) c0[rt] = c1[rt] = f32x4{0.f, 0.f, 0.f, 0.f};
@@ -131,6 +157,9 @@
   const int Fp = r4(F);
   const Lds32 L = lds32_layout(F, D, p.MT, p.S, SX);
   float* buf = smem + L.buf;
+  const bool fold = p.wfold_off != 0;
+  float* ebuf = buf + (fold ? p.xsh : 0);
+  const int nc1 = fold ? p.NC0f : p.NC0;
   float* fs = smem + L.fs;
   float* dsum = smem + L.dsum;
   FieldDev* desc = reinterpret_cast<FieldDev*>(smem + L.desc);
@@ -321,7 +350,7 @@
         }
       }
     }
-    ls.init(wrsrc, 0, p.NC0, p.NT, g, 0);
+    ls.init(wrsrc, p.wfold_off, nc1, p.NT, g, 0);
     ls.preload(wb0, wb1, lane * 16);
 #pragma unroll
     for (int k = 0; k < kUpkPT; ++k) {
@@ -334,10 +363,11 @@
       if (i < n_fwlw) fwlw_s[i] = fw[k];
     }
     if ((flags & kFoLw) && tid < F) lw_s[tid] = lwv;
-    const int w = p.W0 - F * D;
+    const int zc = F * D + (fold ? num : 0);
+    const int w = p.W0 - zc;
     for (int i = tid; i < kRows * w; i += kNTH) {
       const int b = i / w;
-      buf[b * SX + F * D + (i - b * w)] = 0.f;
+      ebuf[b * SX + zc + (i - b * w)] = 0.f;
     }
 #pragma unroll
     for (int k = 0; k < RPT; ++k) {
@@ -349,7 +379,8 @@
           float e[D];
 #pragma unroll
           for (int d = 0; d < D; ++d) e[d] = live[k] ? combine(mode[k], va[k][d], QR ? vb[k][d] : 0.f, scale[k]) : 0.f;
-          store_row<D>(buf + b * SX + f * D, e);
+          store_row<D>(ebuf + b * SX + f * D, e);
+          if (fold && f < num) ebuf[b * SX + F * D + f] = live[k] ? scale[k] : 0.f;
         }
         fo[b * Fp + f] = live[k] ? combine(mode[k], fa[k], QR ? fb[k] : 0.f, scale[k]) : 0.f;
       }
@@ -362,7 +393,7 @@
     for (int r = tid; r < kRows * F; r += kNTH) {
       const int f = r >> 5;
       const int b = r & 31;
-      const float* e = buf + b * SX + f * D;
+      const float* e = ebuf + b * SX + f * D;
       const float* w = fwlw_s + f * D;
       float s = 0.f;
 #pragma unroll
@@ -381,7 +412,7 @@
       const int nt = pc - m * D;
       const int n = nt * 16 + (lane & 15);
       const int b = n / D;
-      const float* ecol0 = buf + b * SX + (n - b * D);
+      const float* ecol0 = ebuf + b * SX + (n - b * D);
       const float* ecol1 = ecol0 + 16 * SX;
       const float* ua = upk + m * S * 64 + lane;
       f32x4 acc0 = f32x4{0.f, 0.f, 0.f, 0.f}, acc1 = acc0;
@@ -477,13 +508,13 @@
   };
   f32x4 bq[kTPW];
   load_bias(bq, 0, 4 * (lane >> 4));
-  int layer_off = 0;
+  int layer_off = p.wfold_off;
   for (int h = 0; h < p.H; ++h) {
     int lv = lane;
     asm volatile("" : "+v"(lv));
     const int rowl = lv & 15;
     const int nq = 4 * (lv >> 4);
-    const int NC = h == 0 ? p.NC0 : p.NT;
+    const int NC = h == 0 ? nc1 : p.NT;
     const bool last = h == p.H - 1;
     const int boff = __builtin_amdgcn_readfirstlane((h * p.NT + TT) * 64 + (g & 3) * 4);
     const int ntail = TT * 16 + nq + (g & 3);
@@ -496,7 +527,8 @@
       for (int j = 0; j < kTPW; ++j) acc[rt][j] = bq[j];
     ts.init(layer_off, NC, TT, g);
     f32x4 tp[kRT];
-    k_loop_rt<kTPW, kRT, kNG, kNS>(acc, buf, SX, ls, wb0, wb1, wb2, lane, ts, tp, h > 0 && (flags & kDeferTail));
+    k_loop_rt<kTPW, kRT, kNG, kNS>(acc, h == 0 && fold ? ebuf + num * D : buf, SX, ls, wb0, wb1, wb2, lane, ts, tp,
+                                   h > 0 && (flags & kDeferTail), h == 0 && nc1 == kNSF);
     if (flags & kPrioEpi) __builtin_amdgcn_s_setprio(1);
     if (h == 0) stamp(p.stamps, 12, tid);
     __syncthreads();
@@ -532,7 +564,7 @@
         if (lane < 16) dsum[g * kRows + rt * 16 + rowl] = d;
       }
     }
-    layer_off += p.NT * NC * 64;
+    layer_off = h == 0 ? p.NT * p.NC0 * 64 : layer_off + p.NT * NC * 64;
     if (!last) {
       ls.init(wrsrc, layer_off, p.NT, p.NT, g, 0);
       ls.preload(wb0, wb1, lane * 16);
diff --git a/xsdeepfwfm_deprecated_amd/csrc/dfwfm_internal.h b/xsdeepfwfm_deprecated_amd/csrc/dfwfm_internal.h
--- a/xsdeepfwfm_deprecated_amd/csrc/dfwfm_internal.h
+++ b/xsdeepfwfm_deprecated_amd/csrc/dfwfm_internal.h
@@ -36,6 +36,7 @@
 constexpr int kFtDiagHwId = 1 << 23, kFtDiagNoMlp = 1 << 24;
 constexpr int kMaxH = 16;
 constexpr int kMaxSet = 32;
+constexpr int kFoldNS = 18;
 
 struct FieldDev {
   const float* emb2;
@@ -79,6 +80,9 @@
   int32_t tail;
   int32_t ns;
   int32_t flags;
+  int32_t wfold_off;
+  int32_t NC0f;
+  int32_t xsh;
   uint64_t* stamps;
   float* sv_e;
   float* sv_fo;
@@ -464,6 +468,13 @@
 hipError_t launch_pack_tables(const PackTabList& L, hipStream_t s);
 hipError_t launch_forward_gather(const FwdArgs& a, int D, size_t lds1, hipStream_t s);
 hipError_t launch_pack_list(const PackList& L, int total_blocks, hipStream_t s);
+struct FoldPackArgs {
+  const float* w1;
+  const FieldDev* fields;
+  float4* dst;
+  int32_t N, F, D, num, NT, NC;
+};
+hipError_t launch_pack_fold(const FoldPackArgs& a, hipStream_t s);
 bool fwd32_supported(int F, int D, int H, int NT, int NC0, int tailI, int NG);
 size_t fwd32_lds_bytes(int F, int D, int MT, int S, int SX);
 hipError_t launch_fwd32(const FwdArgs& a, int D, size_t lds, hipStream_t s);
diff --git a/xsdeepfwfm_deprecated_amd/csrc/dfwfm_kernels.hip b/xsdeepfwfm_deprecated_amd/csrc/dfwfm_kernels.hip
--- a/xsdeepfwfm_deprecated_amd/csrc/dfwfm_kernels.hip
+++ b/xsdeepfwfm_deprecated_amd/csrc/dfwfm_kernels.hip
@@ -59,6 +59,10 @@
   float* part2 = smem + L.part2;
   float* dsum = smem + L.dsum;
   float* fs = smem + L.fs;
+  const bool fold = PART == 0 && !TRAIN && p.wfold_off != 0;
+  const int off1 = fold ? p.wfold_off : 0;
+  float* bufE = bufX + (fold ? p.xsh : 0);
+  const int nc1 = fold ? p.NC0f : p.NC0;
 
   const TileRef tr = tile_ref<kBM>(p);
   const int64_t b0 = tr.b0;
@@ -276,7 +280,7 @@
       }
     }
     if (deep) {
-      ls.init(wrsrc, 0, p.NC0, p.NT, g, kh);
+      ls.init(wrsrc, off1, nc1, p.NT, g, kh);
       DFWFM_PRELOAD(ls);
     }
     if constexpr (!QR)
@@ -292,10 +296,11 @@
       if (i < n_fwlw) fwlw_s[i] = fw[k];
     }
     if ((flags & kFoLw) && tid < F) lw_s[tid] = lwv;
-    const int w = p.W0 - F * D;
+    const int zc = F * D + (fold ? num : 0);
+    const int w = p.W0 - zc;
     for (int i = tid; i < kBM * w; i += NTH) {
       const int b = i / w;
-      bufX[b * SX + F * D + (i - b * w)] = 0.f;
+      bufE[b * SX + zc + (i - b * w)] = 0.f;
     }
 #pragma unroll
     for (int k = 0; k < RPT; ++k) {
@@ -307,7 +312,8 @@
           float e[D];
 #pragma unroll
           for (int d = 0; d < D; ++d) e[d] = live[k] ? combine(mode[k], va[k][d], QR ? vb[k][d] : 0.f, scale[k]) : 0.f;
-          store_row<D>(bufX + b * SX + f * D, e);
+          store_row<D>(bufE + b * SX + f * D, e);
+          if (fold && f < num) bufE[b * SX + F * D + f] = live[k] ? scale[k] : 0.f;
         }
         fo[b * Fp + f] = live[k] ? combine(mode[k], fa[k], QR ? fb[k] : 0.f, scale[k]) : 0.f;
       }
@@ -327,7 +333,7 @@
     for (int r = tid; r < kBM * F; r += NTH) {
       const int f = r >> 4;
       const int b = r & 15;
-      const float* e = bufX + b * SX + f * D;
+      const float* e = bufE + b * SX + f * D;
       const float* w = fwlw_s + f * D;
       float s = 0.f;
 #pragma unroll
@@ -450,7 +456,7 @@
       const int nt = pc - m * D;
       const int n = nt * 16 + (lane & 15);
       const int b = n / D;
-      const float* ecol = bufX + b * SX + (n - b * D);
+      const float* ecol = bufE + b * SX + (n - b * D);
       const float* ua = upk + m * S * 64 + lane;
       f32x4 acc = f32x4{0.f, 0.f, 0.f, 0.f};
       auto group = [&](int s0, auto U_) {
@@ -485,7 +491,7 @@
   }
   if constexpr (NSK == 0) {
     if (deep && tail) {
-      ts.init(0, p.NC0, TT, g);
+      ts.init(off1, nc1, TT, g);
       ts.load(wrsrc, tw, lane * 16);
     }
   }
@@ -579,18 +585,18 @@
   };
   f32x4 bq[TPW];
   load_bias(bq, 0, 4 * (lane >> 4));
-  int layer_off = 0;
+  int layer_off = off1;
   for (int h = 0; h < p.H; ++h) {
     int lv = lane;
     asm volatile("" : "+v"(lv));
     const int rowl = lv & 15;
     const int nq = 4 * (lv >> 4);
     const bool even = (h & 1) == 0;
-    const float* in = even ? bufX : bufY;
+    const float* in = h == 0 ? bufE + (fold ? num * D : 0) : (even ? bufX : bufY);
     const int SA = even ? SX : SY;
     float* outa = even ? bufY : bufX;
     const int SO = even ? SY : SX;
-    const int NC = h == 0 ? p.NC0 : p.NT;
+    const int NC = h == 0 ? nc1 : p.NT;
     const bool last = h == p.H - 1;
     const int boff = __builtin_amdgcn_readfirstlane((h * p.NT + TT) * 64 + (g & 3) * 4);
     const int ntail = TT * 16 + nq + (g & 3);
@@ -604,7 +610,14 @@
       if (tail) ts.init(layer_off, NC, TT, g);
       else ts.cnt = 0;
       f32x4 tp;
-      mlp_k_loop_s<TPW, NG, NSK, true>(acc, in, SA, ls, wb0, wb1, wb2, lane, ts, tp);
+      bool folded1 = false;
+      if constexpr (PART == 0 && !TRAIN && NSK == 25) {
+        if (h == 0 && nc1 == kFoldNS) {
+          folded1 = true;
+          mlp_k_loop_s<TPW, NG, kFoldNS, true>(acc, in, SA, ls, wb0, wb1, wb2, lane, ts, tp);
+        }
+      }
+      if (!folded1) mlp_k_loop_s<TPW, NG, NSK, true>(acc, in, SA, ls, wb0, wb1, wb2, lane, ts, tp);
       if (tail) reinterpret_cast<f32x4*>(tailr)[g * 64 + lane] = tp;
     } else {
       if (tail) reinterpret_cast<f32x4*>(tailr)[g * 64 + lane] = ts.template mma<true>(in, SA, tw, lane);
@@ -661,7 +674,7 @@
       dpart += __shfl_xor(dpart, 32);
       if (lane < 16) dsum[g * kBM + rowl] = dpart;
     }
-    layer_off += p.NT * NC * 64;
+    layer_off = h == 0 ? p.NT * p.NC0 * 64 : layer_off + p.NT * NC * 64;
     if (!last) {
       ls.init(wrsrc, layer_off, p.NT, p.NT, g, kh);
       DFWFM_PRELOAD(ls);
@@ -933,6 +946,42 @@
   hipLaunchKernelGGL(pack_dense_kernel, dim3(total_blocks), dim3(256), 0, s, L);
   return hipGetLastError();
 }
+
+__global__ void __launch_bounds__(256) pack_fold_kernel(const FoldPackArgs a) {
+  const int64_t i = (int64_t)blockIdx.x * 256 + threadIdx.x;
+  if (i >= (int64_t)a.NT * a.NC * 64) return;
+  const int lane = (int)(i & 63);
+  const int64_t tc = i >> 6;
+  const int c = (int)(tc % a.NC);
+  const int t = (int)(tc / a.NC);
+  const int n = t * 16 + (lane & 15);
+  const int K = a.F * a.D;
+  const int KC = (a.F - a.num) * a.D;
+  float v[4];
+#pragma unroll
+  for (int s = 0; s < 4; ++s) {
+    const int k = 16 * c + 4 * (lane >> 4) + s;
+    v[s] = 0.f;
+    if (n < a.N && k < KC) {
+      v[s] = a.w1[(int64_t)n * K + a.num * a.D + k];
+    } else if (n < a.N && k < KC + a.num) {
+      const int f = k - KC;
+      const float* w = a.w1 + (int64_t)n * K + f * a.D;
+      const float* e = a.fields[f].emb2;
+      double acc = 0.0;
+      for (int d = 0; d < a.D; ++d) acc += (double)w[d] * (double)e[d];
+      v[s] = (float)acc;
+    }
+  }
+  a.dst[i] = make_float4(v[0], v[1], v[2], v[3]);
+}
+
+hipError_t launch_pack_fold(const FoldPackArgs& a, hipStream_t s) {
+  const int64_t total = (int64_t)a.NT * a.NC * 64;
+  if (total <= 0) return hipSuccess;
+  hipLaunchKernelGGL(pack_fold_kernel, dim3((unsigned)((total + 255) / 256)), dim3(256), 0, s, a);
+  return hipGetLastError();
+}
 #endif
 
 }
diff --git a/xsdeepfwfm_deprecated_amd/engine.py b/xsdeepfwfm_deprecated_amd/engine.py
--- a/xsdeepfwfm_deprecated_amd/engine.py
+++ b/xsdeepfwfm_deprecated_amd/engine.py
@@ -81,6 +81,7 @@
         _lib.check(_lib.lib().dfwfm_model_set_tables(self.handle, arr, len(fields),
                                                      _stream_handle(self.device)), "dfwfm_model_set_tables")
         self._packed_key = None
+        self._fold_key = None
         self._keep = arr
         self._tables_key = key
 
@@ -107,6 +108,18 @@
         self._pairs_key = None
         self._sparse_key = None
         self._bf16_key = None
+        self._fold_key = None
+
+    def sync_fold(self, tables, enable: bool = True) -> bool:
+        key = (self._dense_key, tuple((t.data_ptr(), t._version) for t in tables), bool(enable))
+        if key == getattr(self, "_fold_key", None):
+            return self._fold_on
+        en = ctypes.c_int32(0)
+        _lib.check(_lib.lib().dfwfm_model_fold_numerical(self.handle, int(bool(enable)), ctypes.byref(en),
+                                                         _stream_handle(self.device)), "dfwfm_model_fold_numerical")
+        self._fold_on = bool(en.value)
+        self._fold_key = key
+        return self._fold_on
 
     def sync_packed(self, tables, enable: bool = True) -> bool:
         key = (bool(enable),) + tuple((t.data_ptr(), t._version) for pair in tables for t in pair if t is not None)
diff --git a/xsdeepfwfm_deprecated_amd/training.py b/xsdeepfwfm_deprecated_amd/training.py
--- a/xsdeepfwfm_deprecated_amd/training.py
+++ b/xsdeepfwfm_deprecated_amd/training.py
@@ -656,10 +656,10 @@
                    "dfwfm_prune_threshold")
         return thr
 
-    def apply(self, t, thr, sym_f=0):
+    def apply(self, t, thr, sym_f=0, owner=None):
         _lib.check(self.L.dfwfm_prune_apply(ctypes.c_void_p(t.data_ptr()), t.numel(), int(sym_f),
                                             ctypes.c_void_p(thr.data_ptr()), self._stream()), "dfwfm_prune_apply")
-        torch.autograd.graph.increment_version(t)
+        torch.autograd.graph.increment_version(t if owner is None else owner)
 
 
 def prune_step(model, adaptive_sparse, prune_fm, prune_r, prune_deep, emb_r, emb_corr):
@@ -674,16 +674,16 @@
     with torch.no_grad():
         named = list(model.named_parameters())
         if prune_fm != 0:
-            embs = [p.data for n, p in named if "fm_2nd_embeddings" in n]
-            thr = pr.threshold([(e, 0) for e in embs], adaptive_sparse * emb_r)
+            embs = [p for n, p in named if "fm_2nd_embeddings" in n]
+            thr = pr.threshold([(e.data, 0) for e in embs], adaptive_sparse * emb_r)
             for e in embs:
-                pr.apply(e, thr)
+                pr.apply(e.data, thr, owner=e)
         for name, param in named:
             if "linear" in name and "weight" in name and prune_deep != 0:
-                pr.apply(param.data, pr.threshold([(param.data, 0)], adaptive_sparse))
+                pr.apply(param.data, pr.threshold([(param.data, 0)], adaptive_sparse), owner=param)
             if name == "field_cov.weight" and prune_r != 0:
                 F_ = param.shape[0]
-                pr.apply(param.data, pr.threshold([(param.data, F_)], adaptive_sparse * emb_corr), F_)
+                pr.apply(param.data, pr.threshold([(param.data, F_)], adaptive_sparse * emb_corr), F_, owner=param)
 
 
 def _prune_step_host(model, adaptive_sparse, prune_fm, prune_r, prune_deep, emb_r, emb_corr):
```

After: 146.2 million, median of 6. 1.08x the previous value.
